# ibrohimmn1994/GPU-implementation-of-signle-and-block-Lanczos

Measured on AMD Instinct MI355X. Metric: block-Lanczos iters/sec + SpMM achieved HBM GB/s vs peak, n=10M nnz=1e8 b=16, higher is better.
Workload: dtype f64; 1 GPU; C3 block Lanczos b=16 fp64, banded-random symmetric CSR n=10000000 per GPU, nnz~10/row, halfwidth 4096; config=C3, n_total=10000000, n_per_gpu=10000000, nnz_per_gpu=100000182, b=16, parallelism=single

## Files before the change

### gpu-implementation-of-signle-and-block-lanczos_amd/__init__.py

```python
from __future__ import annotations

import ctypes
import os
from dataclasses import dataclass
from typing import NamedTuple, Optional

import numpy as np

PKG_DIR = os.path.dirname(os.path.abspath(__file__))
LIB_DIR = os.path.join(PKG_DIR, "lib")
HIP_LIB = os.environ.get("LZ_HIP_LIB") or os.path.join(LIB_DIR, "liblz_hip.so")
HOST_LIB = os.path.join(LIB_DIR, "liblz_host.so")

LZ_F64, LZ_F32 = 0, 1
LZ_ROW_MAJOR, LZ_COL_MAJOR = 0, 1
(LZ_K_SEG768, LZ_K_SEG1536, LZ_K_SEG1024, LZ_K_FNZ, LZ_K_BUF, LZ_K_LDS, LZ_K_ANY_B, LZ_K_CM_DIRECT,
 LZ_K_SPMV) = range(1, 10)
LZ_K_WIN, LZ_K_YCM, LZ_K_EPI, LZ_K_AX3, LZ_K_DOT = 0x100, 0x200, 0x400, 0x800, 0x1000
LZ_K_AX4 = 0x2000
LZ_K_GRAM16, LZ_K_GRAM32F, LZ_K_GRAM_GEN, LZ_K_TSMM16, LZ_K_TSMM32F, LZ_K_TSMM_GEN = range(1, 7)
LZ_K_PGRAM16, LZ_K_PGRAM_GEN, LZ_K_PAPPLY16, LZ_K_PAPPLY_GEN = range(7, 11)
PANEL_GROUP_16, PANEL_GROUP_GEN = 16, 4
PANEL_MAX_BLOCKS = 64
LZ_K_PCOMP16, LZ_K_PCOMP_GEN = 11, 12
PANEL_MAX_KEEP = 16
TRANSPOSE_SHORT, TRANSPOSE_LDS, TRANSPOSE_SCAN_BLOCK = 16, 4096, 2048
CG_THREADS, CG_ROWS_128, CG_GRID_CAP, CG_CHECK_EVERY = 256, 32, 2048, 8
CG_MET, CG_SPENT, CG_NOT_PD = 0, 1, 2
BCG_THREADS, BCG_ROWS_16, BCG_ROWS_32, BCG_ROWS_GEN, BCG_GRID_CAP, BCG_MAX_B = 256, 64, 128, 16, 1024, 32
LZ_K_BCG16, LZ_K_BCG32F, LZ_K_BCG_GEN = 13, 14, 15
BCG_NONE, BCG_CONVERGED, BCG_SPENT, BCG_RANK, BCG_NOT_PD = 0, 1, 2, 3, 4


def bcg_guard(b: int, eps: float) -> float:
    return max(1e-10, 64.0 * b * eps)


_c_i64, _c_i32, _c_int, _c_dbl, _c_vp = ctypes.c_int64, ctypes.c_int32, ctypes.c_int, ctypes.c_double, ctypes.c_void_p
_c_u32, _c_u64 = ctypes.c_uint32, ctypes.c_uint64


class LanczosError(RuntimeError):
    """Raised for a non-zero status from liblz_hip.so / liblz_host.so."""


_hip = None
_host = None

HIP_SYMBOLS = [
    ("lz_init", _c_int, [_c_int, ctypes.POINTER(_c_vp)]),
    ("lz_finalize", _c_int, [_c_vp]),
    ("lz_set_stream", _c_int, [_c_vp, _c_vp]),
    ("lz_set_final_state", _c_int, [_c_vp, _c_int]),
    ("lz_last_error", ctypes.c_char_p, []),
    ("lz_version", ctypes.c_char_p, []),
    ("lz_device_ok", _c_int, [_c_int]),
    ("lz_device_error", _c_int, [_c_vp, ctypes.POINTER(_c_int)]),
    ("lz_debug_poison_lds", _c_int, [_c_vp, ctypes.c_uint32]),
    ("lz_debug_set_device_error", _c_int, [_c_vp, _c_int]),
    ("lz_debug_fail_next_setup", _c_int, [_c_vp, _c_int]),
    ("lz_prof_enable", _c_int, [_c_vp, _c_int]),
    ("lz_prof_enable_mask", _c_int, [_c_vp, ctypes.c_uint]),
    ("lz_prof_read", _c_int, [_c_vp, _c_int, ctypes.POINTER(_c_dbl), ctypes.POINTER(_c_int)]),
    ("lz_csr_spmm", _c_int, [_c_vp, _c_i64, _c_i64, _c_i64, _c_vp, _c_vp, _c_vp, _c_int, _c_int,
                             _c_vp, _c_i64, _c_int, _c_vp, _c_i64]),
    ("lz_to_row_major", _c_int, [_c_vp, _c_i64, _c_int, _c_int, _c_vp, _c_i64, _c_vp]),
    ("lz_to_col_major", _c_int, [_c_vp, _c_i64, _c_int, _c_int, _c_vp, _c_vp, _c_i64]),
    ("lz_csr_spmv", _c_int, [_c_vp, _c_i64, _c_i64, _c_i64, _c_vp, _c_vp, _c_vp, _c_int, _c_vp, _c_vp]),
    ("lz_gram", _c_int, [_c_vp, _c_i64, _c_int, _c_int, _c_vp, _c_i64, _c_vp]),
    ("lz_sym_cross_gram", _c_int, [_c_vp, _c_i64, _c_int, _c_int, _c_vp, _c_vp, _c_i64, _c_vp]),
    ("lz_tsmm", _c_int, [_c_vp, _c_i64, _c_int, _c_int, _c_dbl, _c_dbl, _c_vp, _c_vp, _c_vp, _c_i64]),
    ("lz_sqrtm_pair", _c_int, [_c_vp, _c_int, _c_int, _c_vp, _c_vp, _c_vp, _c_vp]),
    ("lz_copy_row", _c_int, [_c_vp, _c_int, _c_int, _c_vp, _c_i64, _c_int, _c_i64, _c_vp, _c_i64]),
    ("lz_block_lanczos", _c_int, [_c_vp, _c_i64, _c_i64, _c_vp, _c_vp, _c_vp, _c_int, _c_int, _c_int,
                                  _c_i64, _c_vp, _c_vp, _c_vp, _c_vp, _c_vp, _c_vp, _c_vp]),
    ("lz_block_lanczos_unfused", _c_int, [_c_vp, _c_i64, _c_i64, _c_vp, _c_vp, _c_vp, _c_int, _c_int,
                                          _c_int, _c_i64, _c_vp, _c_vp, _c_vp, _c_vp, _c_vp, _c_vp, _c_vp]),
    ("lz_panel_gram", _c_int, [_c_vp, _c_i64, _c_int, _c_int, _c_int, _c_vp, _c_i64, _c_vp, _c_vp]),
    ("lz_panel_apply", _c_int, [_c_vp, _c_i64, _c_int, _c_int, _c_int, _c_dbl, _c_dbl, _c_vp, _c_i64, _c_vp, _c_vp]),
    ("lz_block_lanczos_reorth", _c_int, [_c_vp, _c_i64, _c_i64, _c_vp, _c_vp, _c_vp, _c_int, _c_int, _c_int,
                                         _c_i64, _c_vp, _c_vp, _c_vp, _c_vp, _c_vp, _c_i64, _c_vp, _c_int]),
    ("lz_panel_compress", _c_int, [_c_vp, _c_i64, _c_int, _c_int, _c_int, _c_int, _c_vp, _c_i64, _c_vp]),
    ("lz_block_lanczos_reorth_resume", _c_int, [_c_vp, _c_i64, _c_i64, _c_vp, _c_vp, _c_vp, _c_int, _c_int, _c_int,
                                                _c_int, _c_i64, _c_vp, _c_vp, _c_vp, _c_vp, _c_vp, _c_i64, _c_vp,
                                                _c_int]),
    ("lz_csr_spmm_axpby", _c_int, [_c_vp, _c_i64, _c_i64, _c_vp, _c_vp, _c_vp, _c_int, _c_int, _c_dbl, _c_vp,
                                   _c_dbl, _c_dbl, _c_vp, _c_vp]),
    ("lz_cheb_apply", _c_int, [_c_vp, _c_i64, _c_i64, _c_vp, _c_vp, _c_vp, _c_int, _c_int, _c_vp, _c_vp, _c_vp,
                               _c_vp]),
    ("lz_col_dots", _c_int, [_c_vp, _c_i64, _c_int, _c_int, _c_vp, _c_vp, _c_vp]),
    ("lz_csr_spmm_axpby_dots", _c_int, [_c_vp, _c_i64, _c_i64, _c_vp, _c_vp, _c_vp, _c_int, _c_int, _c_dbl, _c_vp,
                                        _c_dbl, _c_dbl, _c_vp, _c_vp, _c_vp]),
    ("lz_cheb_moments", _c_int, [_c_vp, _c_i64, _c_i64, _c_vp, _c_vp, _c_vp, _c_int, _c_int, _c_dbl, _c_dbl, _c_int,
                                 _c_vp, _c_vp, _c_vp]),
    ("lz_cg_update", _c_int, [_c_vp, _c_i64, _c_int, _c_int, _c_vp, _c_vp, _c_vp, _c_vp, _c_vp, _c_vp, _c_vp]),
    ("lz_cg_solve", _c_int, [_c_vp, _c_i64, _c_i64, _c_vp, _c_vp, _c_vp, _c_int, _c_int, _c_dbl, _c_vp, _c_vp, _c_vp,
                             _c_vp, _c_vp, _c_vp, _c_vp, _c_vp, _c_vp]),
    ("lz_bcg_update", _c_int, [_c_vp, _c_i64, _c_int, _c_int, _c_vp, _c_vp, _c_vp, _c_vp, _c_vp, _c_vp, _c_vp]),
    ("lz_bcg_direction", _c_int, [_c_vp, _c_i64, _c_int, _c_int, _c_vp, _c_vp, _c_vp, _c_vp]),
    ("lz_bcg_solve", _c_int, [_c_vp, _c_i64, _c_i64, _c_vp, _c_vp, _c_vp, _c_int, _c_int, _c_dbl, _c_vp, _c_vp, _c_vp,
                              _c_vp, _c_vp, _c_vp, _c_vp, _c_vp, _c_vp]),
    ("lz_block_lanczos_reorth_cheb", _c_int, [_c_vp, _c_i64, _c_i64, _c_vp, _c_vp, _c_vp, _c_int, _c_int, _c_int,
                                              _c_i64, _c_vp, _c_vp, _c_vp, _c_vp, _c_vp, _c_i64, _c_vp, _c_int,
                                              _c_vp, _c_vp]),
    ("lz_block_lanczos_reorth_resume_cheb", _c_int, [_c_vp, _c_i64, _c_i64, _c_vp, _c_vp, _c_vp, _c_int, _c_int,
                                                     _c_int, _c_int, _c_i64, _c_vp, _c_vp, _c_vp, _c_vp, _c_vp,
                                                     _c_i64, _c_vp, _c_int, _c_vp, _c_vp]),
    ("lz_csr_spmm_axpby4", _c_int, [_c_vp, _c_i64, _c_i64, _c_vp, _c_vp, _c_vp, _c_int, _c_int, _c_dbl, _c_vp,
                                    _c_dbl, _c_dbl, _c_vp, _c_dbl, _c_vp, _c_vp]),
    ("lz_cheb_series_apply", _c_int, [_c_vp, _c_i64, _c_i64, _c_vp, _c_vp, _c_vp, _c_int, _c_int, _c_int, _c_dbl,
                                      _c_dbl, _c_vp, _c_vp, _c_vp, _c_vp]),
    ("lz_block_lanczos_reorth_series", _c_int, [_c_vp, _c_i64, _c_i64, _c_vp, _c_vp, _c_vp, _c_int, _c_int, _c_int,
                                                _c_i64, _c_vp, _c_vp, _c_vp, _c_vp, _c_vp, _c_i64, _c_vp, _c_int,
                                                _c_int, _c_dbl, _c_dbl, _c_vp, _c_vp]),
    ("lz_block_lanczos_reorth_resume_series", _c_int, [_c_vp, _c_i64, _c_i64, _c_vp, _c_vp, _c_vp, _c_int, _c_int,
                                                       _c_int, _c_int, _c_i64, _c_vp, _c_vp, _c_vp, _c_vp, _c_vp,
                                                       _c_i64, _c_vp, _c_int, _c_int, _c_dbl, _c_dbl, _c_vp, _c_vp]),
    ("lz_csr_transpose", _c_int, [_c_vp, _c_i64, _c_i64, _c_i64, _c_vp, _c_vp, _c_vp, _c_int, _c_vp, _c_vp, _c_vp]),
    ("lz_normal_apply", _c_int, [_c_vp, _c_i64, _c_i64, _c_i64, _c_vp, _c_vp, _c_vp, _c_vp, _c_vp, _c_vp, _c_int,
                                 _c_int, _c_vp, _c_vp, _c_vp]),
    ("lz_block_lanczos_reorth_normal", _c_int, [_c_vp, _c_i64, _c_i64, _c_i64, _c_vp, _c_vp, _c_vp, _c_vp, _c_vp,
                                                _c_vp, _c_int, _c_int, _c_int, _c_i64, _c_vp, _c_vp, _c_vp, _c_vp,
                                                _c_vp, _c_i64, _c_vp, _c_int, _c_vp]),
    ("lz_block_lanczos_reorth_resume_normal", _c_int, [_c_vp, _c_i64, _c_i64, _c_i64, _c_vp, _c_vp, _c_vp, _c_vp,
                                                       _c_vp, _c_vp, _c_int, _c_int, _c_int, _c_int, _c_i64, _c_vp,
                                                       _c_vp, _c_vp, _c_vp, _c_vp, _c_i64, _c_vp, _c_int, _c_vp]),
    ("lz_vector_lanczos", _c_int, [_c_vp, _c_i64, _c_i64, _c_vp, _c_vp, _c_vp, _c_int, _c_int, _c_i64,
                                   _c_vp, _c_vp, _c_vp, _c_vp, _c_vp, _c_vp, _c_vp]),
    ("lz_fdtd_block", _c_int, [_c_vp, _c_i64, _c_i64, _c_vp, _c_vp, _c_vp, _c_int, _c_int, _c_vp,
                               _c_i64, _c_dbl, _c_i64, _c_vp, _c_vp, _c_vp]),
    ("lz_comm_unique_id", _c_int, [_c_vp]),
    ("lz_comm_init", _c_int, [_c_vp, _c_int, _c_int, _c_vp]),
    ("lz_halo_init", _c_int, [_c_vp, _c_i64, _c_i64, _c_vp, _c_vp]),
    ("lz_halo_sizes", _c_int, [_c_vp, _c_vp, _c_vp]),
    ("lz_halo_exchange", _c_int, [_c_vp, _c_int, _c_int, _c_vp]),
    ("lz_block_lanczos_halo", _c_int, [_c_vp, _c_i64, _c_i64, _c_vp, _c_vp, _c_vp, _c_int, _c_int, _c_int,
                                       _c_i64, _c_int, _c_vp, _c_vp, _c_vp, _c_vp, _c_vp, _c_vp]),
    ("lz_comm_destroy", _c_int, [_c_vp]),
    ("lz_local_group_create", _c_int, [_c_int, _c_int, ctypes.POINTER(_c_vp)]),
    ("lz_local_group_destroy", _c_int, [_c_vp]),
    ("lz_local_group_abort", _c_int, [_c_vp]),
    ("lz_comm_init_local", _c_int, [_c_vp, _c_vp, _c_int]),
    ("lz_comm_abort", _c_int, [_c_vp]),
    ("lz_debug_last_split", _c_int, [_c_vp, _c_vp]),
    ("lz_debug_last_wf", _c_int, [_c_vp, ctypes.POINTER(_c_int)]),
    ("lz_debug_last_kernel", _c_int, [_c_vp, ctypes.POINTER(_c_int)]),
    ("lz_debug_wf_plan", _c_int, [_c_vp, _c_i64, _c_i64, _c_vp, _c_vp, _c_i64, _c_i64, _c_vp, _c_vp,
                                  ctypes.POINTER(_c_int)]),
    ("lz_block_lanczos_dist", _c_int, [_c_vp, _c_i64, _c_i64, _c_i64, _c_i64, _c_vp, _c_vp, _c_vp,
                                       _c_int, _c_int, _c_int, _c_i64, _c_int, _c_vp, _c_vp, _c_vp,
                                       _c_vp, _c_vp, _c_vp, _c_vp, _c_vp]),
]

HOST_SYMBOLS = [
    ("lzh_gen_banded_count", _c_i64, [_c_i64, _c_dbl, _c_i64, _c_u64, _c_vp]),
    ("lzh_gen_banded_fill", _c_int, [_c_i64, _c_dbl, _c_i64, _c_u64, _c_vp, _c_vp, _c_vp, _c_vp]),
    ("lzh_gen_banded_local_count", _c_i64, [_c_i64, _c_dbl, _c_i64, _c_u64, _c_i64, _c_i64, _c_vp]),
    ("lzh_gen_banded_local_fill", _c_int, [_c_i64, _c_dbl, _c_i64, _c_u64, _c_i64, _c_i64, _c_vp, _c_vp,
                                           _c_vp, _c_vp]),
    ("lzh_gen_powerlaw_count", _c_i64, [_c_i64, _c_dbl, _c_dbl, _c_i64, _c_u64, _c_vp]),
    ("lzh_gen_powerlaw_fill", _c_int, [_c_i64, _c_dbl, _c_dbl, _c_i64, _c_u64, _c_vp, _c_vp, _c_vp, _c_vp]),
    ("lzh_matrix_a_shape", _c_int, [_c_int, _c_vp, _c_vp]),
    ("lzh_matrix_a_ell", _c_int, [_c_int, _c_int, _c_vp, _c_vp]),
    ("lzh_ell_to_csr_count", _c_i64, [_c_i64, _c_i64, _c_vp, _c_vp, _c_int, _c_vp]),
    ("lzh_ell_to_csr_fill", _c_int, [_c_i64, _c_i64, _c_vp, _c_vp, _c_int, _c_vp, _c_vp, _c_vp]),
    ("lzh_rand_B", _c_int, [_c_i64, _c_int, _c_u32, _c_i64, _c_int, _c_vp]),
    ("lzh_rand_lc", _c_i64, [_c_u32]),
    ("lzh_uniform_B", _c_int, [_c_i64, _c_int, _c_u64, _c_vp, _c_vp]),
    ("lzh_uniform_B_rows", _c_int, [_c_i64, _c_i64, _c_int, _c_u64, _c_vp, _c_vp]),
    ("lzh_sym_eig", _c_int, [_c_int, _c_vp, _c_vp, _c_vp]),
    ("lzh_assemble_T", _c_int, [_c_int, _c_int, _c_vp, _c_vp, _c_vp]),
    ("lzh_ritz_values", _c_int, [_c_int, _c_int, _c_vp, _c_vp, _c_vp]),
    ("lzh_ritz_pairs", _c_int, [_c_int, _c_int, _c_vp, _c_vp, _c_int, _c_int, _c_vp, _c_vp, _c_vp]),
    ("lzh_ritz_pairs_dense", _c_int, [_c_int, _c_int, _c_vp, _c_vp, _c_int, _c_int, _c_vp, _c_vp, _c_vp]),
    ("lzh_restart_coeffs", _c_int, [_c_int, _c_int, _c_int, _c_vp, _c_vp, _c_int, _c_vp, _c_vp, _c_vp, _c_vp]),
    ("lzh_restart_fill", _c_int, [_c_int, _c_int, _c_int, _c_vp, _c_vp, _c_vp]),
    ("lzh_gershgorin", _c_int, [_c_i64, _c_vp, _c_vp, _c_vp, _c_vp]),
    ("lzh_cg_start", _c_int, [_c_int, _c_int, _c_int, _c_vp, _c_vp, _c_vp, _c_vp, _c_vp, _c_vp, _c_vp, _c_vp, _c_vp,
                              _c_vp]),
    ("lzh_cg_scalars", _c_int, [_c_int, _c_int, _c_int, _c_vp, _c_vp, _c_vp, _c_vp, _c_vp, _c_vp, _c_vp, _c_vp, _c_vp,
                                _c_vp, _c_vp]),
    ("lzh_bcg_start", _c_int, [_c_int, _c_int, _c_vp, _c_vp, _c_vp, _c_vp, _c_vp, _c_vp]),
    ("lzh_bcg_start_finish", _c_int, [_c_int, _c_dbl, _c_vp, _c_vp, _c_vp, _c_vp, _c_vp, _c_vp, _c_vp]),
    ("lzh_bcg_mid", _c_int, [_c_int, _c_vp, _c_vp, _c_vp, _c_vp, _c_vp, _c_vp]),
    ("lzh_bcg_end", _c_int, [_c_int, _c_int, _c_dbl, _c_vp, _c_vp, _c_vp, _c_vp, _c_vp, _c_vp, _c_vp]),
    ("lzh_bcg_guard", _c_dbl, [_c_int, _c_dbl]),
    ("lzh_kpm_moments", _c_int, [_c_int, _c_int, _c_vp, _c_vp]),
    ("lzh_jackson", _c_int, [_c_int, _c_vp]),
    ("lzh_kpm_count", _c_int, [_c_int, _c_vp, _c_vp, _c_dbl, _c_dbl, _c_dbl, _c_dbl, _c_vp]),
    ("lzh_cheb_window", _c_int, [_c_int, _c_dbl, _c_dbl, _c_dbl, _c_dbl, _c_vp, _c_vp]),
    ("lzh_kpm_density", _c_int, [_c_int, _c_vp, _c_vp, _c_dbl, _c_dbl, _c_int, _c_vp, _c_vp]),
    ("lzh_block_solution", _c_int, [_c_int, _c_int, _c_dbl, _c_vp, _c_vp, _c_vp, _c_vp]),
    ("lzh_partition_rows", _c_int, [_c_i64, _c_vp, _c_int, _c_vp]),
    ("lzh_remap_cols_padded", _c_int, [_c_i64, _c_vp, _c_int, _c_vp, _c_i64, _c_vp]),
    ("lzh_halo_plan", _c_i64, [_c_i64, _c_vp, _c_int, _c_vp, _c_int, _c_vp, _c_vp, _c_vp]),
    ("lzh_csr_write", _c_int, [ctypes.c_char_p, _c_i64, _c_i64, _c_i64, _c_vp, _c_vp, _c_vp, _c_int]),
    ("lzh_csr_read_header", _c_int, [ctypes.c_char_p, _c_vp, _c_vp, _c_vp, _c_vp]),
    ("lzh_csr_read", _c_int, [ctypes.c_char_p, _c_vp, _c_vp, _c_vp]),
    ("lzh_num_threads", _c_int, []),
]


def _bind(lib, symbols, strict=True):
    for name, res, args in symbols:
        if not strict and not hasattr(lib, name):
            continue
        fn = getattr(lib, name)
        fn.restype = res
        fn.argtypes = args
    return lib


def build(verbose: bool = False) -> None:
    import subprocess
    jobs = str(min(16, os.cpu_count() or 4))
    out = subprocess.run(["make", "-C", PKG_DIR, "-j", jobs], capture_output=not verbose, text=True)
    if out.returncode != 0:
        raise LanczosError("build failed:\n" + (out.stdout or "") + (out.stderr or ""))


def host_lib():
    global _host
    if _host is None:
        if not os.path.exists(HOST_LIB):
            raise LanczosError(f"{HOST_LIB} missing: run make in {PKG_DIR}")
        _host = _bind(ctypes.CDLL(HOST_LIB), HOST_SYMBOLS)
    return _host


def hip_lib():
    global _hip
    if _hip is None:
        if not os.path.exists(HIP_LIB):
            raise LanczosError(f"{HIP_LIB} missing: run make in {PKG_DIR}")
        try:
            import torch
        except ImportError:
            pass
        _hip = _bind(ctypes.CDLL(HIP_LIB), HIP_SYMBOLS, strict=not os.environ.get("LZ_HIP_LIB"))
    return _hip


def _check(rc: int, what: str) -> None:
    if rc != 0:
        msg = hip_lib().lz_last_error().decode(errors="replace") if _hip is not None else ""
        raise LanczosError(f"{what} failed with status {rc}: {msg}")


def _p(a: np.ndarray):
    return a.ctypes.data_as(_c_vp)


@dataclass
class CsrHost:
    n: int
    row_ptr: np.ndarray
    col: np.ndarray
    val: np.ndarray

    @property
    def nnz(self) -> int:
        return int(self.row_ptr[-1])


def gen_banded(n: int, nnz_per_row: float = 10.0, halfwidth: int = 4096, seed: int = 20261015,
               dtype=np.float64) -> CsrHost:
    L = host_lib()
    rp = np.empty(n + 1, np.int64)
    nnz = L.lzh_gen_banded_count(n, nnz_per_row, halfwidth, seed, _p(rp))
    if nnz < 0:
        raise LanczosError("lzh_gen_banded_count failed")
    col = np.empty(nnz, np.int32)
    val = np.empty(nnz, dtype)
    v64 = _p(val) if dtype == np.float64 else None
    v32 = _p(val) if dtype == np.float32 else None
    if L.lzh_gen_banded_fill(n, nnz_per_row, halfwidth, seed, _p(rp), _p(col), v64, v32):
        raise LanczosError("lzh_gen_banded_fill failed")
    return CsrHost(n, rp, col, val)


def gen_banded_local(n: int, r0: int, r1: int, nnz_per_row: float = 10.0, halfwidth: int = 4096,
                     seed: int = 20261015, dtype=np.float64) -> CsrHost:
    L = host_lib()
    nl = r1 - r0
    rp = np.empty(nl + 1, np.int64)
    nnz = L.lzh_gen_banded_local_count(n, nnz_per_row, halfwidth, seed, r0, r1, _p(rp))
    if nnz < 0:
        raise LanczosError("lzh_gen_banded_local_count failed")
    col = np.empty(nnz, np.int32)
    val = np.empty(nnz, dtype)
    v64 = _p(val) if dtype == np.float64 else None
    v32 = _p(val) if dtype == np.float32 else None
    if L.lzh_gen_banded_local_fill(n, nnz_per_row, halfwidth, seed, r0, r1, _p(rp), _p(col), v64, v32):
        raise LanczosError("lzh_gen_banded_local_fill failed")
    return CsrHost(nl, rp, col, val)


def gen_powerlaw(n: int, nnz_per_row: float = 10.0, a: float = 2.1, cap: int = 100000,
                 seed: int = 20261015, dtype=np.float32) -> CsrHost:
    L = host_lib()
    rp = np.empty(n + 1, np.int64)
# ... 1035 lines not shown
                    scale=scale, cols=sel, filter=filt, n_steps=d.steps)

    def eigsh_interval(self, A: CsrDevice, a: float, b: float, /, block: int = 16, m: Optional[int] = None,
                       keep: Optional[int] = None, degree: Optional[int] = None, bounds=None, pad: float = 0.01,
                       tol: float = 1e-10, max_cycles: int = 100, B=None, lc: int = 0, passes: int = 2):
        torch = _torch()
        a, b = float(a), float(b)
        if not a < b:
            raise LanczosError(f"eigsh_interval: the window [{a}, {b}] needs a < b")
        lo, hi = gershgorin(A) if bounds is None else (float(bounds[0]), float(bounds[1]))
        if not (np.isfinite(lo) and np.isfinite(hi) and lo < hi and pad >= 0):
            raise LanczosError(f"eigsh_interval: bounds ({lo}, {hi}) must be finite with lo < hi, pad >= 0")
        lo, hi = lo - pad * (hi - lo), hi + pad * (hi - lo)
        if not (lo <= a and b <= hi):
            raise LanczosError(f"eigsh_interval: the window [{a}, {b}] is not inside the enclosure [{lo}, {hi}]")
        if degree is None:
            degree = min(65536, max(16, int(np.ceil(np.pi * (hi - lo) / (b - a)))))
        if not 1 <= int(degree) <= 65536:
            raise LanczosError("eigsh_interval: 1 <= degree <= 65536")
        degree = int(degree)
        if keep is None:
            keep = 4 if m is None else max(1, min(4, m - 1))
        m, r = _restart_sizes("eigsh_interval", "(keep - 1) * block", max((keep - 1) * block, 1), block, m, keep)
        n, bs = A.n, block
        scale = max(abs(lo), abs(hi))
        gamma = cheb_window(degree, lo, hi, a, b)
        work = torch.empty(2 * n * bs, dtype=A.val.dtype, device=A.val.device)
        d = _Restart(self, A, n, bs, m, r, lc, passes, A.val, series=(degree, lo, hi, gamma), work=work)
        V, vstride, kw = d.V, d.vstride, d.kw
        U, X = work[:n * bs].view(n, bs), work[n * bs:].view(n, bs)
        C = torch.empty(r, bs, bs, **kw)
        G, Dm = torch.empty(bs, bs, **kw), torch.empty(bs, bs, **kw)
        rb = r * bs

        def check():
            H = np.empty((rb, rb))
            for i in range(r):
                self.spmm(A, V[i * vstride:i * vstride + n * bs].view(n, bs), U)
                self.panel_gram(V, vstride, r, U, C)
                H[:, i * bs:(i + 1) * bs] = _f64(C).reshape(rb, bs)
            lam, Cm = np.linalg.eigh(0.5 * (H + H.T))
            Sd = torch.from_numpy(_pack_chunks(Cm, r, bs)).to(**kw)
            res = np.empty(rb)
            for c in range(r):
                self.panel_apply(0.0, 1.0, V, vstride, r, Sd[c], X)
                self.spmm(A, X, U)
                Dm.copy_(torch.from_numpy(np.diag(lam[c * bs:(c + 1) * bs])).to(**kw))
                self.mm_ts(1.0, -1.0, X, Dm, U)
                self.mm_tt(U, G)
                res[c * bs:(c + 1) * bs] = np.sqrt(np.maximum(np.diag(_f64(G)), 0.0))
            return lam, res, Cm

        d.first(d.start_block(B))
        history = []
        while True:
            d.compress("largest")
            lam, res, Cm = check()
            meets = (lam + res >= a) & (lam - res <= b)
            inside = (lam >= a) & (lam <= b)
            full = bool(inside.sum() == rb)
            history.append(float(res[meets].max()) if meets.any() else 0.0)
            converged = bool(not full and (res[meets] <= tol * scale).all())
            if converged or full or d.cycles >= max_cycles:
                break
            d.resume()
        sel = np.flatnonzero(inside)
        if sel.size:
            Zx = _pack_chunks(Cm[:, sel], r, bs)
            self.panel_compress(V, vstride, r, len(Zx), d._dev(Zx), n=n)
        return dict(theta=lam[sel], resid=res[sel], count=int(sel.size), V=V, vstride=vstride, cycles=d.cycles,
                    n_steps=d.steps, n_spmm=degree * d.steps + 2 * r * d.cycles, converged=converged, full=full,
                    history=history, scale=scale, filter=(degree, lo, hi))

    def set_final_state(self, on: bool) -> None:
        _check(self.L.lz_set_final_state(self.ptr, 1 if on else 0), "lz_set_final_state")

    def vector_lanczos(self, A: CsrDevice, bvec, m: int, lc: int, q, alpha, beta, q0, q1, w):
        n = bvec.shape[0]
        for t in (bvec, q, alpha, beta, q0, q1, w):
            if t.element_size() != (8 if A.dtype == LZ_F64 else 4):
                raise ValueError("vector_lanczos: every vector must have A's element type")
        _check(self.L.lz_vector_lanczos(self.ptr, n, A.nnz, _ptr(A.row_ptr), _ptr(A.col), _ptr(A.val), A.dtype,
                                        m, lc, _ptr(bvec), _ptr(q), _ptr(alpha), _ptr(beta), _ptr(q0),
                                        _ptr(q1), _ptr(w)), "lz_vector_lanczos")

    def ftdt_block(self, A: CsrDevice, U0, steps: int, T_end: float, lc: int, U, D, out):
        n, b = U0.shape
        _check(self.L.lz_fdtd_block(self.ptr, n, A.nnz, _ptr(A.row_ptr), _ptr(A.col), _ptr(A.val), A.dtype, b,
                                    _ptr(U0), steps, T_end, lc, _ptr(U), _ptr(D), _ptr(out)), "lz_fdtd_block")
        return out

    PROF_SPMM_PASS, PROF_UPDATE_PASS, PROF_SMALL, PROF_GRAM, PROF_TSMM, PROF_SPMM = range(6)

    def device_error(self) -> int:
        c = _c_int()
        _check(self.L.lz_device_error(self._h, ctypes.byref(c)), "lz_device_error")
        return c.value

    def debug_set_device_error(self, code: int):
        _check(self.L.lz_debug_set_device_error(self.ptr, code), "lz_debug_set_device_error")

    def debug_fail_next_setup(self, code: int = 5):
        _check(self.L.lz_debug_fail_next_setup(self._h, code), "lz_debug_fail_next_setup")

    def debug_poison_lds(self, pattern: int = 0xFFFFFFFF):
        _check(self.L.lz_debug_poison_lds(self._h, pattern), "lz_debug_poison_lds")

    def prof_enable(self, on: bool = True, classes=None):
        if classes is None:
            _check(self.L.lz_prof_enable(self._h, int(on)), "lz_prof_enable")
        else:
            mask = 0
            for c in classes:
                mask |= 1 << int(c)
            _check(self.L.lz_prof_enable_mask(self._h, mask if on else 0), "lz_prof_enable_mask")

    def prof_read(self, cls: int):
        ms, cnt = _c_dbl(), _c_int()
        _check(self.L.lz_prof_read(self._h, cls, ctypes.byref(ms), ctypes.byref(cnt)), "lz_prof_read")
        return ms.value, cnt.value

    def comm_init(self, nranks: int, rank: int, uid: bytes):
        buf = ctypes.create_string_buffer(uid, 128)
        _check(self.L.lz_comm_init(self._h, nranks, rank, buf), "lz_comm_init")

    def comm_init_local(self, group: "LocalGroup", rank: int):
        _check(self.L.lz_comm_init_local(self.ptr, group.ptr, rank), "lz_comm_init_local")
        group._keep.append(self)

    def last_wf(self):
        v = (_c_int * 2)()
        _check(self.L.lz_debug_last_wf(self._h, v), "lz_debug_last_wf")
        return bool(v[0]), bool(v[1])

    def last_kernel(self):
        v = (_c_int * 2)()
        _check(self.L.lz_debug_last_kernel(self._h, v), "lz_debug_last_kernel")
        return int(v[0]), int(v[1])

    def wf_plan(self, A, nx=None, xoff=0):
        import torch
        T_max = A.n // 16 + 2
        deps = torch.zeros(T_max * 2, dtype=torch.int32, device=A.row_ptr.device)
        c16 = torch.zeros(max(A.nnz, 1), dtype=torch.int16, device=A.row_ptr.device)
        info = (_c_int * 8)()
        _check(self.L.lz_debug_wf_plan(self.ptr, A.n, A.nnz, A.row_ptr.data_ptr(), A.col.data_ptr(),
                                       A.n if nx is None else nx, xoff, deps.data_ptr(), c16.data_ptr(), info),
               "lz_debug_wf_plan")
        T = int(info[2])
        d = {"ok": bool(info[0]), "col16": bool(info[1]), "T": T, "tr": int(info[3]),
             "spans": [int(info[4 + i]) for i in range(4)]}
        return d, deps[: 2 * T].view(T, 2), c16[: A.nnz]

    def last_split(self):
        v = (_c_i64 * 2)()
        _check(self.L.lz_debug_last_split(self._h, v), "lz_debug_last_split")
        return None if v[0] < 0 else (int(v[0]), int(v[1]))

    def comm_abort(self):
        _check(self.L.lz_comm_abort(self._h), "lz_comm_abort")

    def comm_destroy(self):
        _check(self.L.lz_comm_destroy(self._h), "lz_comm_destroy")

    def block_lanczos_dist(self, A_local: CsrDevice, n_pad: int, n_global: int, B_local, m: int,
                           lc_local: int, lc_rank: int, q, alpha, beta, Q0, W, X_full):
        n_local, b = A_local.n, B_local.shape[1]
        _check(self.L.lz_block_lanczos_dist(self.ptr, n_local, n_pad, n_global, A_local.nnz,
                                            _ptr(A_local.row_ptr), _ptr(A_local.col), _ptr(A_local.val),
                                            A_local.dtype, b, m, lc_local, lc_rank, _ptr(B_local), _ptr(q),
                                            _ptr(alpha), _ptr(beta), _ptr(Q0), None, _ptr(W), _ptr(X_full)),
               "lz_block_lanczos_dist")


    def halo_init(self, row0: int, n_local: int, recv_counts: np.ndarray, halo_rows: np.ndarray):
        rc = np.ascontiguousarray(recv_counts, np.int64)
        hr = np.ascontiguousarray(halo_rows, np.int32)
        _check(self.L.lz_halo_init(self.ptr, row0, n_local, _p(rc), _p(hr) if hr.size else None),
               "lz_halo_init")

    def halo_sizes(self):
        nh, ns = _c_i64(), _c_i64()
        _check(self.L.lz_halo_sizes(self.ptr, ctypes.byref(nh), ctypes.byref(ns)), "lz_halo_sizes")
        return nh.value, ns.value

    def halo_exchange(self, X):
        _check(self.L.lz_halo_exchange(self.ptr, _dt(X), X.shape[1], _ptr(X)), "lz_halo_exchange")

    def block_lanczos_halo(self, A_local: CsrDevice, B_local, m: int, lc_local: int, lc_rank: int,
                           q, alpha, beta, X0, X1):
        n_local, b = A_local.n, B_local.shape[1]
        _check(self.L.lz_block_lanczos_halo(self.ptr, n_local, A_local.nnz, _ptr(A_local.row_ptr),
                                            _ptr(A_local.col), _ptr(A_local.val), A_local.dtype, b, m,
                                            lc_local, lc_rank, _ptr(B_local), _ptr(q), _ptr(alpha),
                                            _ptr(beta), _ptr(X0), _ptr(X1)),
               "lz_block_lanczos_halo")


class LocalGroup:

    def __init__(self, nranks: int, device: int = 0):
        L = hip_lib()
        g = _c_vp()
        _check(L.lz_local_group_create(device, nranks, ctypes.byref(g)), "lz_local_group_create")
        self.ptr, self.nranks, self.device, self.L = g, nranks, device, L
        self._keep = []

    def abort(self):
        if self.ptr:
            self.L.lz_local_group_abort(self.ptr)

    def close(self):
        if self.ptr:
            self.L.lz_local_group_destroy(self.ptr)
            self.ptr = None

    def __del__(self):
        try:
            self.close()
        except Exception:
            pass


def run_virtual_ranks(nranks: int, fn, device: int = 0, timeout: float = 600.0):
    import threading
    torch = _torch()
    torch.cuda.synchronize(device)
    group = LocalGroup(nranks, device)
    handles = [Handle(device) for _ in range(nranks)]
    streams = [torch.cuda.Stream(device) for _ in range(nranks)]
    out, errs = [None] * nranks, [None] * nranks

    def body(r):
        try:
            with torch.cuda.device(device), torch.cuda.stream(streams[r]):
                handles[r].comm_init_local(group, r)
                out[r] = fn(r, handles[r])
                torch.cuda.current_stream(device).synchronize()
        except BaseException as e:
            errs[r] = e
            group.abort()

    threads = [threading.Thread(target=body, args=(r,), daemon=True) for r in range(nranks)]
    try:
        for t in threads:
            t.start()
        for t in threads:
            t.join(timeout)
        if any(t.is_alive() for t in threads):
            group.abort()
            for t in threads:
                t.join(30)
        if any(t.is_alive() for t in threads):
            raise LanczosError("virtual ranks did not finish")
    finally:
        if not any(t.is_alive() for t in threads):
            torch.cuda.synchronize(device)
            for h in handles:
                h.close()
            group.close()
            group._keep.clear()
            del streams[:]
    for r, e in enumerate(errs):
        if e is not None:
            raise LanczosError(f"virtual rank {r}: {e}") from e
    return out


def comm_unique_id() -> bytes:
    buf = ctypes.create_string_buffer(128)
    _check(hip_lib().lz_comm_unique_id(buf), "lz_comm_unique_id")
    return buf.raw


def run_block_lanczos(h: Handle, A: CsrDevice, B, m: int, lc: int, fused: bool = True):
    torch = _torch()
    n, b = B.shape
    kw = dict(dtype=B.dtype, device=B.device)
    q = torch.zeros(m * b, **kw)
    alpha = torch.zeros(m, b, b, **kw)
    beta = torch.zeros(m + 1, b, b, **kw)
    Q0, Q1, W = (torch.empty(n, b, **kw) for _ in range(3))
    h.block_lanczos_blas(A, B, m, lc, q, alpha, beta, Q0, Q1, W, fused=fused)
    return q, alpha, beta
```

### gpu-implementation-of-signle-and-block-lanczos_amd/csrc/lz_api.hip

```cpp
#include <cmath>
#include <cstdarg>
#include <cstdlib>
#include <cstring>
#include <algorithm>
#include <utility>
#include <vector>

#include <type_traits>
#include "lz_comm.hpp"
#include "lz_common.hpp"
#include "lz_internal.hpp"
#include "lz_kernels.hpp"

namespace lz {

static thread_local char g_err[1024] = "";

int prof_begin(lz_handle *h, int cls)
{
    if (!h->prof || !((h->prof_mask >> cls) & 1u) || h->ev_used + 2 > h->ev_cap) return -1;
    const int idx = h->ev_used;
    if (hipEventRecord(h->ev_pool[idx], h->stream) != hipSuccess) return -1;
    h->ev_class[idx / 2] = cls;
    h->ev_used += 2;
// ... 340 lines not shown
        LZ_ARG_CHECK(std::isfinite(sr.lo) && std::isfinite(sr.hi) && sr.lo < sr.hi, "Chebyshev series: lo < hi, finite");
        LZ_ARG_CHECK(sr.gamma != nullptr, "Chebyshev series: gamma is NULL");
        break;
    case OpSpec::Normal:
        LZ_ARG_CHECK(op.p >= 1, "normal operator: p >= 1");
        LZ_ARG_CHECK(op.t_rp != nullptr, "normal operator: the transpose's row_ptr is NULL");
        LZ_ARG_CHECK(op.t_col != nullptr && op.t_val != nullptr, "normal operator: the transpose's col/val NULL");
        break;
    }
    LZ_ARG_CHECK(op.work != nullptr, "work is NULL");
    LZ_ARG_CHECK(!work16 || reinterpret_cast<uintptr_t>(op.work) % 16 == 0, "work must be on 16 bytes");
    LZ_ARG_CHECK(apart(span_of(op.work, op.work_elems(n, b), dtype), others), apart_msg);
    return LZ_OK;
}

template <typename T>
static int reorth_op(lz_handle *h, int64_t n, int b, const OpSpec &op, const T *Q, T *W)
{
    const T *val = (const T *)op.val;
    T *work = (T *)op.work;
    switch (op.form) {
    case OpSpec::Filter:
        return cheb_apply<T>(h, n, op.nnz, op.rp, op.col, val, b, op.f, Q, W, work);
    case OpSpec::Series:
        return cheb_series_apply<T>(h, n, op.nnz, op.rp, op.col, val, b, op.sr, Q, W, work);
    case OpSpec::Normal:
        LZ_TRY(spmm_rm<T>(h, op.p, op.nnz, op.rp, op.col, val, b, Q, b, n, work, b));
        return spmm_rm<T>(h, n, op.nnz, op.t_rp, op.t_col, (const T *)op.t_val, b, work, b, op.p, W, b);
    case OpSpec::Plain:
        break;
    }
    return spmm_rm<T>(h, n, op.nnz, op.rp, op.col, val, b, Q, b, n, W, b);
}

template <typename T>
static int reorth_steps(lz_handle *h, int64_t n, const OpSpec &op, int b, int j0, int m, int64_t lc, T *q,
                        T *alpha, T *beta, T *V, int64_t vstride, T *W, int passes)
{
    const int64_t bb = (int64_t)b * b;
    T *binv = ScratchT<T>(h, b).binv[0];
    int P = 0;
    for (int j = j0; j < m; ++j) {
        T *bj = beta + j * bb, *aj = alpha + j * bb;
        T *Qp = V + (int64_t)(j - 1) * vstride, *Qj = V + (int64_t)j * vstride;
        LZ_TRY(gram_partials<T>(h, n, b, W, W, b, &P));
        LZ_TRY(sqrtm_pair<T>(h, b, nullptr, P, bj, binv, nullptr));
        LZ_TRY(tsmm<T>(h, n, b, T(0), T(1), W, binv, Qj, b));
        LZ_TRY(reorth_op<T>(h, n, b, op, Qj, W));
        LZ_TRY(tsmm<T>(h, n, b, T(1), T(-1), Qp, bj, W, b));
        LZ_TRY(gram_partials<T>(h, n, b, W, Qj, b, &P));
        LZ_TRY(gram_finish<T>(h, b, P, 1, aj));
        LZ_TRY(tsmm<T>(h, n, b, T(1), T(-1), Qj, aj, W, b));
        LZ_TRY(reorth_rounds<T>(h, n, b, j + 1, V, vstride, W, passes));
        LZ_TRY(copy_row<T>(h, b, Qj, b, 0, lc, q + (int64_t)j * b));
    }
    LZ_TRY(gram_partials<T>(h, n, b, W, W, b, &P));
    LZ_TRY(sqrtm_pair<T>(h, b, nullptr, P, beta + m * bb, binv, nullptr));
    return LZ_OK;
}

template <typename T>
static int reorth_cycle(lz_handle *h, int64_t n, const OpSpec &op, int b, int r, int m, int64_t lc, const T *B,
                        const T *sigma, T *q, T *alpha, T *beta, T *V, int64_t vstride, T *W, int passes)
{
    const int64_t bb = (int64_t)b * b;
    const bool first = r == 0;
    T *binv = ScratchT<T>(h, b).binv[0];
    LZ_TRY(reorth_reserve<T>(h, n, b, m, passes));
    int P = 0;
    const T *R = first ? B : W;
    T *br = beta + r * bb, *ar = alpha + r * bb, *Qr = V + (int64_t)r * vstride;
    LZ_TRY(gram_partials<T>(h, n, b, R, R, b, &P));
    LZ_TRY(sqrtm_pair<T>(h, b, nullptr, P, br, binv, nullptr));
    LZ_TRY(tsmm<T>(h, n, b, T(0), T(1), R, binv, Qr, b));
    if (first) LZ_TRY(copy_row<T>(h, b, Qr, b, 0, lc, q));
    LZ_TRY(reorth_op<T>(h, n, b, op, Qr, W));
    if (!first) LZ_TRY(panel_apply<T>(h, n, b, r, 1.0, -1.0, V, vstride, sigma, W));
    LZ_TRY(gram_partials<T>(h, n, b, W, Qr, b, &P));
    LZ_TRY(gram_finish<T>(h, b, P, 1, ar));
    LZ_TRY(tsmm<T>(h, n, b, T(1), T(-1), Qr, ar, W, b));
    LZ_TRY(reorth_rounds<T>(h, n, b, r + 1, V, vstride, W, passes));
    if (!first) LZ_TRY(copy_row<T>(h, b, Qr, b, 0, lc, q + (int64_t)r * b));
    return reorth_steps<T>(h, n, op, b, r + 1, m, lc, q, alpha, beta, V, vstride, W, passes);
}

struct Pass1Plan {
    const uint64_t *pairs = nullptr;
    int win = 0;
    const int16_t *col16 = nullptr;
};
static int pass1_plan(lz_handle *h, int64_t n, int64_t nnz, const int64_t *rp, const int32_t *col, int64_t nx,
                      int64_t row_off, Pass1Plan *pl)
{
    LZ_TRY(strip_pairs(h, n, rp, &pl->pairs));
    if (nx >= (1 << 24)) {
        bool ok = false;
        LZ_TRY(gather_window_ok(h, n, rp, col, nx, row_off, &ok));
        pl->win = ok ? 1 : 0;
    }
    if (nx < (1 << 24) || pl->win) LZ_TRY(col16_plan(h, n, nnz, rp, col, row_off, &pl->col16));
    return LZ_OK;
}

template <typename T>
struct ResidualRing {
    const T *in, *prev = nullptr;
    T *r0, *r1;
    ResidualRing(const T *B, int m, T *W, T *Q1) : in(B), r0((m & 1) ? W : Q1), r1((m & 1) ? Q1 : W) {}
    T *out(int j) const { return j == 0 ? r0 : j == 1 ? r1 : const_cast<T *>(prev); }
    void advance(T *out) { prev = in, in = out; }
};

template <typename T>
static int store_beta_m(lz_handle *h, T *beta, int m, int64_t bb, T *const binv[2])
{
    LZ_HIP_TRY(hipMemcpyAsync(beta + m * bb, binv[(m - 1) & 1], sizeof(T) * bb, hipMemcpyDeviceToDevice, h->stream));
    return LZ_OK;
}

struct WfTail {
    lz_handle *h;
    double *slab;
    double *const *binv;
    double *P1, *P2, *alpha, *beta, *q;
    int64_t lc;
    Comm *cm = nullptr;
    int operator()(int j, const WfSlabs &sl, const double *V) const
    {
        constexpr int64_t bb = 256;
        LZ_TRY(wf_fold16(h, sl, slab));
        if (cm) LZ_TRY(cm->allreduce_sum(slab, 3 * bb, h->stream));
        const WfAlpha wa{slab, 1, alpha + j * bb, P2, V, lc, q + j * 16};
        return sqrtm_pair<double>(h, 16, nullptr, 1, beta + j * bb, binv[j & 1], nullptr, slab + 2 * bb,
                                  j ? binv[(j - 1) & 1] : nullptr, j ? P1 : nullptr, &wa);
    }
};

static WfSlabs wf_one_set(const double *part, int P)
{
    WfSlabs sl;
    sl.add(part, P);
    return sl;
}

static int gram_beside(lz_handle *h, int64_t n, const double *B, int *P)
{
    LZ_TRY(stream_fork(h, h->ev_fork, h->side));
    StreamScope on_side(h, h->side);
    LZ_TRY(gram_partials<double>(h, n, 16, B, B, 16, P));
    LZ_HIP_TRY(hipEventRecord(h->ev_join, h->side));
    return LZ_OK;
}

static int block_lanczos_wf16(lz_handle *h, int64_t n, int64_t nnz, const int64_t *rp, const int32_t *col,
                              const double *val, int m, int64_t lc, const double *B, double *q, double *alpha,
                              double *beta, double *Q0, double *Q1, double *W, const Pass1Plan &pl,
                              const WfPlan &wp, int Pg)
{
    constexpr int64_t bb = 256;
    (void)nnz;
    const Scratch16 sc(h);
    double *const *binv = sc.binv;
    double *P1 = sc.P1, *P2 = sc.P2, *slab = sc.slab;
    const int64_t lcl = (lc >= 0 && lc < n) ? lc : -1;
    int P = 0;
    const bool g0 = Pg < 0;
    if (!g0) LZ_TRY(sqrtm_pair<double>(h, 16, nullptr, Pg, beta, binv[0], nullptr));
    LZ_TRY(wf_reset16(h, n, wp));
    const WfSolve ws{n, rp, col, val, pl.pairs, wp, n};
    const WfTail tail{h, slab, binv, P1, P2, alpha, beta, q, lcl};
    double *part = h->partials2;
    LZ_TRY(wf_step16(h, ws, ws.first(B, Q0, g0), part, &P));
    if (g0) LZ_TRY(tail(0, wf_one_set(part, P), B));
    else LZ_TRY(alpha_wf16(h, part, P, binv[0], nullptr, alpha, P2, B, lc, n, q));
    const double *Vm1 = nullptr, *V0 = B;
    auto pass2 = [&](int j, double *Vn) { return WfPass2{Q0, Vm1, V0, Vn, binv[j & 1], j ? P1 : nullptr, P2}; };
    for (int j = 0; j + 1 < m; ++j) {
        double *Vn = j == 0 ? W : j == 1 ? Q1 : const_cast<double *>(Vm1);
        LZ_TRY(wf_step16(h, ws, ws.step(pass2(j, Vn), ws.all(), {Vn, Q0, ws.all()}, j + 1), part, &P));
        LZ_TRY(tail(j + 1, wf_one_set(part, P), Vn));
        Vm1 = V0;
        V0 = Vn;
    }
    LZ_TRY(store_beta_m<double>(h, beta, m, bb, binv));
    if (h->final_state) {
        const WfPass2 p2 = pass2(m - 1, W);
        if (wp.var == 111)
            LZ_TRY(wf_step16(h, ws, ws.post_call(p2, m, Q0, m >= 2 ? Q1 : nullptr), part, &P));
        else
            LZ_TRY(final_state<double>(h, n, 16, p2.Yj, p2.Vprev, p2.Vj, nullptr, p2.binv, p2.P1, p2.P2, W, Q0,
                                       m >= 2 ? Q1 : nullptr));
    }
    return LZ_OK;
}

static int block_lanczos_fused16(lz_handle *h, int64_t n, int64_t nnz, const int64_t *rp, const int32_t *col,
                                 const double *val, int m, int64_t lc, const double *B, double *q,
                                 double *alpha, double *beta, double *Q0, double *Q1, double *W)
{
    constexpr int64_t bb = 256;
    (void)Q0;
    const Scratch16 qb(h);
    double *const qP = qb.P1;
    int P = 0;
    Pass1Plan pl;
    const bool g0 = wf_first_gram(n, nnz);
    if (!g0) LZ_TRY(gram_beside(h, n, B, &P));
    JoinSide join_side{h};
    {
        WfPlan wp;
        LZ_TRY(wf_plan16(h, n, nnz, rp, col, &wp));
        if (wp.ok) {
            LZ_TRY(strip_pairs(h, n, rp, &pl.pairs));
            pl.col16 = wp.col16;
            if (!g0) LZ_HIP_TRY(hipStreamWaitEvent(h->stream, h->ev_join, 0));
            else if (wp.var != 111) LZ_TRY(gram_partials<double>(h, n, 16, B, B, 16, &P));
            const bool first = g0 && wp.var == 111;
            return block_lanczos_wf16(h, n, nnz, rp, col, val, m, lc, B, q, alpha, beta, Q0, Q1, W, pl, wp,
                                      first ? -1 : P);
        }
    }
    if (g0) LZ_TRY(gram_partials<double>(h, n, 16, B, B, 16, &P));
    LZ_TRY(pass1_plan(h, n, nnz, rp, col, n, 0, &pl));
    LZ_HIP_TRY(hipStreamWaitEvent(h->stream, h->ev_join, 0));
    LZ_TRY(sqrtm_pair<double>(h, 16, nullptr, P, beta, qb.binv[0], nullptr));
    ResidualRing<double> r(B, m, W, Q1);
    for (int j = 0; j < m; ++j) {
        double *out = r.out(j);
        const double *bi = qb.binv[j & 1];
        LZ_TRY(fused_spmm16(h, n, rp, col, val, r.in, n, r.in, r.prev, out, bi, j ? qP : nullptr, lc, q + j * 16, &P,
                            pl.pairs, nnz, 0, pl.win, 0, pl.col16));
        LZ_TRY(gram_finish<double>(h, 16, P, 1, alpha + j * bb, h->partials2, bi, qP));
        LZ_TRY(fused_update16(h, n, out, r.in, qP, &P));
        if (j + 1 < m)
            LZ_TRY(sqrtm_pair<double>(h, 16, nullptr, P, beta + (j + 1) * bb, qb.binv[(j + 1) & 1], nullptr,
                                      nullptr, bi, qP));
        r.advance(out);
    }
    LZ_TRY(store_beta_m<double>(h, beta, m, bb, qb.binv));
    if (h->final_state)
        LZ_TRY(final_state<double>(h, n, 16, nullptr, nullptr, r.prev, r.in, qb.binv[(m - 1) & 1], nullptr, nullptr,
                                   W, Q0, m >= 2 ? Q1 : nullptr));
    return LZ_OK;
}

static int block_lanczos_b2_32(lz_handle *h, int64_t n, int64_t nnz, const int64_t *rp, const int32_t *col,
                               const float *val, int m, int64_t lc, const float *B, float *q, float *alpha,
                               float *beta, float *Q0, float *Q1, float *W)
{
    constexpr int b = 32;
    const int64_t bb = (int64_t)b * b;
    const ScratchT<float> sc(h, b);
    float *const *binv = sc.binv;
    float *P2 = sc.P, *M = sc.P3;
    float *U = Q0;
    JoinSide join_side{h};
    int np = 0, cap = 768, lslot = -1;
    LZ_TRY(spmm_b2_stage(h, n, rp, &cap));
#ifndef LZ_B2_STEP0_QUEUES
    LZ_TRY(spmm_b2_plan(h, n, rp, cap, &lslot));
#endif
    LZ_TRY(gram_partials<float>(h, n, b, B, B, b, &np));
    LZ_TRY(sqrtm_pair<float>(h, b, nullptr, np, beta, binv[0], nullptr));
    ResidualRing<float> r(B, m, W, Q1);
    for (int j = 0; j < m; ++j) {
        float *out = r.out(j);
        const float *bi = binv[j & 1];
        const float *in = r.in, *prev = r.prev;
#ifndef LZ_B2_STEP0_QUEUES
        LZ_TRY(spmm_rm_b2(h, n, nnz, rp, col, val, in, n, U, prev, j ? M : nullptr, lslot, nullptr, cap));
#else
        LZ_TRY(spmm_rm_b2(h, n, nnz, rp, col, val, in, n, U, prev, j ? M : nullptr, j ? lslot : -1,
                          j ? nullptr : &lslot, cap));
#endif
        if (j > 0) LZ_HIP_TRY(hipStreamWaitEvent(h->stream, h->ev_join, 0));
        LZ_TRY(fused_el32(h, n, in, U, &np));
        const int nf = fold_slabs_g(h, h->partials, np, (int)bb, 32);
        LZ_TRY(alpha_b2(h, h->partials2, nf, bi, alpha + j * bb, P2, in, lc, n, q + (int64_t)j * b));
        const bool qlast = j + 1 == m && h->final_state;
        LZ_TRY(fused_ub32(h, n, U, in, bi, P2, out, &np, qlast ? Q0 : nullptr, qlast && m >= 2 ? Q1 : nullptr));
        if (j + 1 < m) {
            const int ng = fold_slabs_g(h, h->partials, np, (int)bb, 32);
            LZ_TRY(m_b2(h, h->partials2, ng, bi, M));
            LZ_TRY(stream_fork(h, h->ev_fork, h->side));
            StreamScope on_side(h, h->side);
            LZ_TRY(sqrtm_pair<float>(h, b, nullptr, ng, beta + (j + 1) * bb, binv[(j + 1) & 1], nullptr,
                                     h->partials2));
            LZ_HIP_TRY(hipEventRecord(h->ev_join, h->side));
        }
        r.advance(out);
    }
    LZ_TRY(store_beta_m<float>(h, beta, m, bb, binv));
    return LZ_OK;
}

template <typename T>
static int block_lanczos_sep(lz_handle *h, int64_t n, int64_t nnz, const int64_t *rp, const int32_t *col,
                             const T *val, int b, int m, int64_t lc, const T *B, T *q, T *alpha, T *beta, T *Q0,
                             T *Q1, T *W)
{
    if constexpr (std::is_same<T, float>::value) {
        const char *e = getenv("LZ_C5_B2");
        if (b == 32 && !(e && atoi(e) == 0) && spmm_b2_ok(n, nnz, n))
            return block_lanczos_b2_32(h, n, nnz, rp, col, val, m, lc, B, q, alpha, beta, Q0, Q1, W);
    }
    const int64_t bb = (int64_t)b * b;
    const ScratchT<T> sc(h, b);
    T *const *binv = sc.binv;
    T *P = sc.P;
    T *Y = Q0;
    int np = 0;
    LZ_TRY(gram_partials<T>(h, n, b, B, B, b, &np));
    LZ_TRY(sqrtm_pair<T>(h, b, nullptr, np, beta, binv[0], nullptr));
    ResidualRing<T> r(B, m, W, Q1);
    for (int j = 0; j < m; ++j) {
        T *out = r.out(j);
        const T *bi = binv[j & 1];
        const T *in = r.in, *prev = r.prev;
        LZ_TRY(spmm_rm<T>(h, n, nnz, rp, col, val, b, in, b, n, Y, b));
        if (j > 0) LZ_HIP_TRY(hipStreamWaitEvent(h->stream, h->ev_join, 0));
        LZ_TRY(fused_e_sep<T>(h, n, b, Y, in, prev, out, bi, j ? P : nullptr, lc, q + (int64_t)j * b, &np));
        LZ_TRY(gram_finish<T>(h, b, np, 1, alpha + j * bb, h->partials, bi, P));
        LZ_TRY(fused_u_sep<T>(h, n, b, out, in, P, &np));
        if (j + 1 < m) {
            LZ_TRY(stream_fork(h, h->ev_fork, h->side));
            StreamScope on_side(h, h->side);
            LZ_TRY(sqrtm_pair<T>(h, b, nullptr, np, beta + (j + 1) * bb, binv[(j + 1) & 1], nullptr, nullptr, bi, P));
            LZ_HIP_TRY(hipEventRecord(h->ev_join, h->side));
        }
        r.advance(out);
    }
    LZ_TRY(store_beta_m<T>(h, beta, m, bb, binv));
    if (h->final_state)
        LZ_TRY(final_state<T>(h, n, b, nullptr, nullptr, r.prev, r.in, binv[(m - 1) & 1], nullptr, nullptr, W, Q0,
                              m >= 2 ? Q1 : nullptr));
    return LZ_OK;
}

constexpr int64_t kFdtdGraph = 256;
constexpr int64_t kFdtdFusedRows = 1 << 18;

template <typename T>
static int fdtd_block(lz_handle *h, int64_t n, int64_t nnz, const int64_t *rp, const int32_t *col, const T *val,
                      int b, const T *U0, int64_t steps, double T_end, int64_t lc, T *U, T *D,
                      T *out)
{
    const T dt = (T)(T_end / (double)steps);
    LZ_HIP_TRY(hipMemcpyAsync(U, U0, sizeof(T) * n * b, hipMemcpyDeviceToDevice, h->stream));
    const bool fused = n <= kFdtdFusedRows;
    T *cur = U;
    auto step = [&]() -> int {
        if (fused) {
            T *nxt = cur == U ? D : U;
            const int64_t nb = n * b;
            hipLaunchKernelGGL((k_fdtd_step<T>), dim3((unsigned)ceil_div(nb, 256)), dim3(256), 0, h->stream,
                               nb, b, rp, col, val, dt, (const T *)cur, nxt);
            LZ_LAUNCH_CHECK();
            cur = nxt;
            return LZ_OK;
        }
        LZ_TRY(spmm_rm<T>(h, n, nnz, rp, col, val, b, U, b, n, D, b));
        return axpy<T>(h, n * b, dt, D, U);
    };
    const char *graph_env = getenv("LZ_FDTD_GRAPH");
    const bool use_graph = !(graph_env && graph_env[0] == '0');
    int64_t s = 0;
    LZ_TRY(step());
    ++s;
    if (use_graph && steps - s >= 2 * kFdtdGraph) {
        hipStream_t cap = nullptr;
        LZ_HIP_TRY(hipStreamCreateWithFlags(&cap, hipStreamNonBlocking));
        int rc = LZ_OK;
// ... 453 lines not shown
    LZ_TRY(wf_reset16(h, n, wp));
    const WfSolve ws{n, rp, col, val, pairs, wp, nx};
    const WfTail tail{h, slab, binv, P1, P2, alpha, beta, q, lcl, cx.reduce ? cm : nullptr};
    const double *Vm1 = nullptr, *V0 = ag ? slot : X0;
    int G = 0;
    LZ_TRY(wf_step16(h, ws, ws.first(X0, Y, g0), h->partials2, &G));
    if (g0) {
        LZ_TRY(tail(0, wf_one_set(h->partials2, G), V0));
    } else {
        LZ_TRY(wf_fold16(h, wf_one_set(h->partials2, G), slab));
        LZ_TRY(cx.allreduce(3 * bb));
        LZ_TRY(alpha_wf16(h, slab, 1, binv[0], nullptr, alpha, P2, V0, lcl, n, q));
    }
    const bool sw = ag && h->nranks > 1;
    for (int j = 0; j + 1 < m; ++j) {
        double *Vn = sw ? slot : ((j & 1) ? X0 : X1);
        double *Vg = sw ? X0 : Vn;
        const double *Vprev = sw ? (j ? X1 : nullptr) : Vm1;
        const WfPass2 p2{Y, Vprev, V0, Vn, binv[j & 1], j ? P1 : nullptr, P2, sw ? X1 : nullptr};
        WfSlabs sl;
        double *part = h->partials2;
        auto launch = [&](const WfLaunch &L) -> int {
            int g = 0;
            LZ_TRY(wf_step16(h, ws, L, part, &g));
            sl.add(part, g);
            part += 3 * (int64_t)g * 256;
            return LZ_OK;
        };
        if (pre) {
            LZ_TRY(launch(ws.pass2(p2, {0, sh}, {st, T}, j + 1)));
            LZ_TRY(stream_fork(h, h->ev_cx, h->xstream));
            LZ_TRY(cx.exchange(Vg, h->xstream));
            LZ_HIP_TRY(hipEventRecord(h->ev_xd, h->xstream));
        }
        LZ_TRY(launch(ws.step(p2, pre ? WfTiles{sh, st} : ws.all(), {Vg, Y, {t0, t1}}, j + 1)));
        if (exch) {
            if (pre) LZ_HIP_TRY(hipStreamWaitEvent(h->stream, h->ev_xd, 0));
            else LZ_TRY(cx.exchange(Vg, h->stream));
            const bool two = t0 > 0 && t1 < T;
            if (two) LZ_TRY(stream_fork(h, h->ev_cx, h->xstream));
            LZ_TRY(launch(ws.boundary(Vg, Y, {0, t0})));
            {
                StreamScope on_x(h, two ? h->xstream : h->stream);
                LZ_TRY(launch(ws.boundary(Vg, Y, {t1, T})));
            }
            if (two) LZ_TRY(stream_join(h, h->ev_bd, h->xstream));
        }
        LZ_TRY(tail(j + 1, sl, Vn));
        Vm1 = V0;
        V0 = Vn;
    }
    LZ_TRY(store_beta_m<double>(h, beta, m, bb, binv));
    if (cm) LZ_TRY(cm->fence(h->stream));
    return LZ_OK;
}

template <typename T>
static int dist_solve(lz_handle *h, int form, HaloPlan *hp, int64_t n, int64_t n_pad, int64_t nnz, const int64_t *rp,
                      const int32_t *col, const T *val, int b, int m, int64_t lc, const T *B, T *q, T *alpha, T *beta,
                      T *X0, T *X1)
{
    LZ_TRY(solve_begin(h));
    int rc = dist_solve_impl<T>(h, form, hp, n, n_pad, nnz, rp, col, val, b, m, lc, B, q, alpha, beta, X0, X1);
    if (rc == LZ_OK) rc = solve_status(h);
    return rc;
}

}

using namespace lz;

static int dist_fail(lz_handle *h, int rc, uint64_t issued0)
{
    if (rc != LZ_OK && rc != LZ_E_DEVICE && h && h->comm &&
        (h->comm->abort_wakes_peers() || h->comm->issued != issued0))
        h->comm->abort();
    return rc;
}

static uint64_t comm_issued(const lz_handle *h) { return h && h->comm ? h->comm->issued : 0; }

#define LZ_HANDLE_CHECK(h)                                                          \
    do {                                                                            \
        if (!(h)) {                                                                 \
            set_error("handle is NULL");                                           \
            return LZ_E_STATE;                                                      \
        }                                                                           \
        LZ_HIP_TRY(hipSetDevice((h)->device));                                      \
    } while (0)

static int shape_args(lz_dtype dtype, int64_t n, int64_t n_min, int b, int b_max, const char *msg = nullptr)
{
    char text[64];
    if (!msg) snprintf(text, sizeof(text), "n >= %lld, b in [1,%d]", (long long)n_min, b_max), msg = text;
    LZ_ARG_CHECK(dtype == LZ_F64 || dtype == LZ_F32, "dtype");
    LZ_ARG_CHECK(n >= n_min && b >= 1 && b <= b_max, msg);
    return LZ_OK;
}

template <typename Solve>
static int krylov_entry(lz_handle *h, int64_t n, int64_t nnz, const int64_t *rp, const int32_t *col, const void *val,
                        lz_dtype dtype, int b, int b_max, double shift, const void *B, void *X, void *work,
                        const lz_cg_opts *opts, int *iters, int *status, double *resid, double *est, int *info,
                        Solve solve)
{
    LZ_HANDLE_CHECK(h);
    LZ_TRY(check_csr(n, nnz, rp, col, val));
    LZ_TRY(shape_args(dtype, n, 1, b, b_max));
    LZ_ARG_CHECK(B && X && work && opts && iters && status && resid && est && info, "NULL argument");
    LZ_ARG_CHECK(opts->tol > 0.0 && std::isfinite(opts->tol) && std::isfinite(shift), "tol > 0, tol and shift finite");
    LZ_ARG_CHECK(opts->max_iter >= 0 && opts->max_restarts >= 0, "max_iter, max_restarts >= 0");
    const int64_t nb = n * b;
    LZ_ARG_CHECK(pairwise_apart({span_of(B, nb, dtype), span_of(X, nb, dtype), span_of(work, 4 * nb, dtype)}),
                 "B, X and work must be pairwise distinct");
    return by_dtype(dtype, [&](auto t) {
        using T = decltype(t);
        return solve(h, n, nnz, rp, col, (const T *)val, b, shift, (const T *)B, (T *)X, (T *)work, *opts, iters, status,
                     resid, est, info);
    });
}

extern "C" {

const char *lz_last_error(void) { return g_err; }
const char *lz_version(void) { return "lz_hip 0.1 gfx950"; }

int lz_device_ok(int device)
{
    int count = 0;
    if (hipGetDeviceCount(&count) != hipSuccess || device < 0 || device >= count) return 0;
    hipDeviceProp_t prop;
    if (hipGetDeviceProperties(&prop, device) != hipSuccess) return 0;
    return std::strncmp(prop.gcnArchName, "gfx950", 6) == 0 ? 1 : 0;
}

static int init_handle(lz_handle *h, int device)
{
    h->device = device;
    hipDeviceProp_t prop;
    LZ_HIP_TRY(hipGetDeviceProperties(&prop, device));
    if (std::strncmp(prop.gcnArchName, "gfx950", 6) != 0) {
        set_error("device %d is %s, liblz_hip.so is built for gfx950 only", device, prop.gcnArchName);
        return LZ_E_HIP;
    }
    h->n_cu = prop.multiProcessorCount;
    LZ_TRY(ensure_partials(h, (size_t)kMaxPartials * kMaxB * kMaxB));
    LZ_HIP_TRY(hipMalloc(&h->partials2, sizeof(double) * kPartials2Doubles));
    LZ_HIP_TRY(hipMalloc(&h->scratch, sizeof(double) * kScratchDoubles));
    LZ_HIP_TRY(hipMalloc(&h->err_flag, sizeof(int) * kFlagWords));
    LZ_HIP_TRY(hipMemsetAsync(h->err_flag, 0, sizeof(int) * kFlagWords, h->stream));
    LZ_HIP_TRY(hipStreamCreateWithFlags(&h->side, hipStreamNonBlocking));
    LZ_HIP_TRY(hipEventCreateWithFlags(&h->ev_fork, hipEventDisableTiming));
    LZ_HIP_TRY(hipEventCreateWithFlags(&h->ev_join, hipEventDisableTiming));
    if (const char *pz = getenv("LZ_POISON"); pz && pz[0] == '1') {
        LZ_HIP_TRY(hipMemsetAsync(h->partials, 0xFF, h->partials_cap, h->stream));
        LZ_HIP_TRY(hipMemsetAsync(h->partials2, 0xFF, sizeof(double) * kPartials2Doubles, h->stream));
        LZ_HIP_TRY(hipMemsetAsync(h->scratch, 0xFF, sizeof(double) * kScratchDoubles, h->stream));
    }
    LZ_HIP_TRY(hipStreamSynchronize(h->stream));
    return LZ_OK;
}

int lz_init(int device, lz_handle **out)
{
    LZ_ARG_CHECK(out != nullptr, "out handle pointer is NULL");
    *out = nullptr;
    int count = 0;
    LZ_HIP_TRY(hipGetDeviceCount(&count));
    LZ_ARG_CHECK(device >= 0 && device < count, "device index");
    LZ_HIP_TRY(hipSetDevice(device));
    lz_handle *h = new lz_handle();
    const int rc = init_handle(h, device);
    if (rc != LZ_OK) {
        lz_finalize(h);
        return rc;
    }
    *out = h;
    return LZ_OK;
}

int lz_finalize(lz_handle *h)
{
    if (!h) return LZ_OK;
    (void)hipSetDevice(h->device);
    detach_comm(h);
    (void)hipFree(h->pairs);
    (void)hipFree(h->longq);
    (void)hipFree(h->cm_buf);
    (void)hipFree(h->dots_ws);
    (void)hipFree(h->cg_ws);
    (void)hipFree(h->bcg_ws);
    (void)hipFree(h->ybuf);
    (void)hipFree(h->coef);
    (void)hipFree(h->tr_ws);
    (void)hipFree(h->c16buf);
    (void)hipFree(h->wf_deps);
    (void)hipFree(h->wf_flags);
    (void)hipFree(h->fnz_colf);
    (void)hipFree(h->fnz_trow);
    if (h->ev_pool) {
        for (int i = 0; i < h->ev_cap; ++i) (void)hipEventDestroy(h->ev_pool[i]);
        delete[] h->ev_pool;
    }
    (void)hipFree(h->partials);
    (void)hipFree(h->partials2);
    (void)hipFree(h->scratch);
    (void)hipFree(h->err_flag);
    if (h->ev_fork) (void)hipEventDestroy(h->ev_fork);
    if (h->ev_join) (void)hipEventDestroy(h->ev_join);
    if (h->ev_lfork) (void)hipEventDestroy(h->ev_lfork);
    if (h->ev_ljoin) (void)hipEventDestroy(h->ev_ljoin);
    if (h->lstream) (void)hipStreamDestroy(h->lstream);
    if (h->side) (void)hipStreamDestroy(h->side);
    for (hipStream_t s : {h->pf_sg, h->pf_sp})
        if (s) {
            (void)hipStreamSynchronize(s);
            (void)hipStreamDestroy(s);
        }
    for (hipEvent_t e : {h->ev_pff, h->ev_pfg, h->ev_pfp})
        if (e) (void)hipEventDestroy(e);
    (void)hipFree(h->pf_ctl);
    delete h;
    return LZ_OK;
}

int lz_device_error(lz_handle *h, int *code)
{
    LZ_ARG_CHECK(h && code, "null argument");
    int c = 0;
    LZ_HIP_TRY(hipMemcpyAsync(&c, h->err_flag, sizeof(int), hipMemcpyDeviceToHost, h->stream));
    LZ_HIP_TRY(hipMemsetAsync(h->err_flag, 0, sizeof(int), h->stream));
    LZ_HIP_TRY(hipStreamSynchronize(h->stream));
    *code = c;
    return LZ_OK;
}

int lz_debug_set_device_error(lz_handle *h, int code)
{
    LZ_HANDLE_CHECK(h);
    LZ_HIP_TRY(hipMemsetD32Async(reinterpret_cast<hipDeviceptr_t>(h->err_flag), code, 1, h->stream));
    return LZ_OK;
}

int lz_debug_fail_next_setup(lz_handle *h, int code)
{
    LZ_HANDLE_CHECK(h);
    h->dbg_setup_fail = code;
    return LZ_OK;
}

__global__ __launch_bounds__(1024) void k_poison_lds(uint32_t pattern)
{
    constexpr int kWords = 160 * 1024 / 4;
    __shared__ uint32_t lds[kWords];
    volatile uint32_t *v = lds;
    for (int i = threadIdx.x; i < kWords; i += blockDim.x) v[i] = pattern;
}

int lz_debug_poison_lds(lz_handle *h, uint32_t pattern)
{
    LZ_HANDLE_CHECK(h);
    hipLaunchKernelGGL(k_poison_lds, dim3(h->n_cu * 4), dim3(1024), 0, h->stream, pattern);
    LZ_LAUNCH_CHECK();
    const int byte = (int)(pattern & 0xFF);
    LZ_HIP_TRY(hipMemsetAsync(h->partials, byte, h->partials_cap, h->stream));
    LZ_HIP_TRY(hipMemsetAsync(h->partials2, byte, sizeof(double) * kPartials2Doubles, h->stream));
    LZ_HIP_TRY(hipMemsetAsync(h->scratch, byte, sizeof(double) * kScratchDoubles, h->stream));
    if (h->dots_ws) LZ_HIP_TRY(hipMemsetAsync(h->dots_ws, byte, h->dots_cap, h->stream));
    if (h->cg_ws) LZ_HIP_TRY(hipMemsetAsync(h->cg_ws, byte, h->cg_cap, h->stream));
    if (h->bcg_ws) LZ_HIP_TRY(hipMemsetAsync(h->bcg_ws, byte, h->bcg_cap, h->stream));
    return LZ_OK;
}

int lz_prof_enable_mask(lz_handle *h, unsigned class_mask)
{
    LZ_HANDLE_CHECK(h);
    if (class_mask && !h->ev_pool) {
        h->ev_cap = 8192;
        h->ev_pool = new hipEvent_t[h->ev_cap];
        for (int i = 0; i < h->ev_cap; ++i) LZ_HIP_TRY(hipEventCreate(&h->ev_pool[i]));
    }
    h->prof = class_mask != 0;
    h->prof_mask = class_mask;
    h->ev_used = 0;
    return LZ_OK;
}

int lz_prof_enable(lz_handle *h, int on) { return lz_prof_enable_mask(h, on ? ~0u : 0u); }

int lz_prof_read(lz_handle *h, int cls, double *ms_total, int *count)
{
    LZ_HANDLE_CHECK(h);
    LZ_ARG_CHECK(ms_total && count, "NULL outputs");
    *ms_total = 0.0;
    *count = 0;
    if (!h->ev_pool || h->ev_used == 0) return LZ_OK;
    LZ_HIP_TRY(hipEventSynchronize(h->ev_pool[h->ev_used - 1]));
    for (int i = 0; i < h->ev_used; i += 2) {
        if (h->ev_class[i / 2] != cls) continue;
        float ms = 0.f;
        LZ_HIP_TRY(hipEventElapsedTime(&ms, h->ev_pool[i], h->ev_pool[i + 1]));
        *ms_total += ms;
        *count += 1;
    }
    return LZ_OK;
}

int lz_set_final_state(lz_handle *h, int on)
{
    LZ_HANDLE_CHECK(h);
    h->final_state = on ? 1 : 0;
    return LZ_OK;
}

int lz_set_stream(lz_handle *h, void *stream)
{
    LZ_HANDLE_CHECK(h);
    h->stream = reinterpret_cast<hipStream_t>(stream);
    return LZ_OK;
}

int lz_csr_spmm(lz_handle *h, int64_t n_rows, int64_t n_cols, int64_t nnz, const int64_t *rp,
                const int32_t *col, const void *val, lz_dtype dtype, int b, const void *X,
                int64_t ldx, lz_layout layout, void *Y, int64_t ldy)
{
    LZ_HANDLE_CHECK(h);
    LZ_TRY(check_csr(n_rows, nnz, rp, col, val));
    LZ_ARG_CHECK(b >= 1 && b <= kMaxB, "b in [1,64]");
    LZ_ARG_CHECK(X && Y, "X/Y NULL");
    if (layout == LZ_ROW_MAJOR) {
        LZ_ARG_CHECK(ldx >= b && ldy >= b, "row-major ld >= b");
    } else {
        LZ_ARG_CHECK(ldx >= n_cols && ldy >= n_rows, "column-major ld >= rows");
    }
    return by_dtype(dtype, [&](auto t) {
        using T = decltype(t);
        const T *v = (const T *)val, *x = (const T *)X;
        if (layout == LZ_ROW_MAJOR) return spmm_rm<T>(h, n_rows, nnz, rp, col, v, b, x, ldx, n_cols, (T *)Y, ldy);
        return spmm_cm<T>(h, n_rows, nnz, rp, col, v, b, x, ldx, n_cols, (T *)Y, ldy);
    });
}

int lz_to_row_major(lz_handle *h, int64_t rows, int b, lz_dtype dtype, const void *X, int64_t ldx, void *Y)
{
    LZ_HANDLE_CHECK(h);
    LZ_ARG_CHECK(X && Y && X != Y, "to_row_major: X, Y distinct, not NULL");
    return by_dtype(dtype, [&](auto t) {
        using T = decltype(t);
        return to_row_major<T>(h, rows, b, (const T *)X, ldx, (T *)Y);
    });
}

int lz_to_col_major(lz_handle *h, int64_t rows, int b, lz_dtype dtype, const void *X, void *Y, int64_t ldy)
{
    LZ_HANDLE_CHECK(h);
    LZ_ARG_CHECK(X && Y && X != Y, "to_col_major: X, Y distinct, not NULL");
    return by_dtype(dtype, [&](auto t) {
        using T = decltype(t);
        return to_col_major<T>(h, rows, b, (const T *)X, ldy, (T *)Y);
    });
}

// ... 381 lines not shown
int lz_block_lanczos_reorth_normal(lz_handle *h, int64_t n, int64_t p, int64_t nnz, const int64_t *rp,
                                   const int32_t *col, const void *val, const int64_t *t_rp, const int32_t *t_col,
                                   const void *t_val, lz_dtype dtype, int b, int m, int64_t lc, const void *B, void *q,
                                   void *alpha, void *beta, void *V, int64_t vstride, void *W, int passes, void *work)
{
    return cycle_entry(h, n, OpSpec::normal(p, nnz, rp, col, val, t_rp, t_col, t_val, work), dtype, b, 0, m, lc, B,
                       nullptr, q, alpha, beta, V, vstride, W, passes);
}

int lz_panel_compress(lz_handle *h, int64_t n, int b, int k, int r, lz_dtype dtype, void *V, int64_t vstride,
                      const void *Z)
{
    LZ_HANDLE_CHECK(h);
    LZ_TRY(panel_args(n, b, k, dtype, V, vstride));
    LZ_ARG_CHECK(r >= 1 && r <= k, "panel_compress keeps 1 <= r <= k blocks");
    LZ_ARG_CHECK(r <= kPanelMaxKeep, "panel_compress keeps at most LZ_PANEL_MAX_KEEP = 16 blocks");
    LZ_ARG_CHECK(Z != nullptr, "Z is NULL");
    return by_dtype(dtype, [&](auto t) {
        using T = decltype(t);
        return panel_compress<T>(h, n, b, k, r, (T *)V, vstride, (const T *)Z);
    });
}

int lz_block_lanczos_reorth_resume(lz_handle *h, int64_t n, int64_t nnz, const int64_t *rp, const int32_t *col,
                                   const void *val, lz_dtype dtype, int b, int r, int m, int64_t lc,
                                   const void *sigma, void *q, void *alpha, void *beta, void *V, int64_t vstride,
                                   void *W, int passes)
{
    return lz_block_lanczos_reorth_resume_cheb(h, n, nnz, rp, col, val, dtype, b, r, m, lc, sigma, q, alpha, beta, V,
                                               vstride, W, passes, nullptr, nullptr);
}

int lz_block_lanczos_reorth_resume_cheb(lz_handle *h, int64_t n, int64_t nnz, const int64_t *rp, const int32_t *col,
                                        const void *val, lz_dtype dtype, int b, int r, int m, int64_t lc,
                                        const void *sigma, void *q, void *alpha, void *beta, void *V, int64_t vstride,
                                        void *W, int passes, const lz_cheb *f, void *work)
{
    return cycle_entry(h, n, OpSpec::filter(nnz, rp, col, val, f, work), dtype, b, r, m, lc, nullptr, sigma, q, alpha,
                       beta, V, vstride, W, passes);
}

int lz_block_lanczos_reorth_resume_normal(lz_handle *h, int64_t n, int64_t p, int64_t nnz, const int64_t *rp,
                                          const int32_t *col, const void *val, const int64_t *t_rp,
                                          const int32_t *t_col, const void *t_val, lz_dtype dtype, int b, int r, int m,
                                          int64_t lc, const void *sigma, void *q, void *alpha, void *beta, void *V,
                                          int64_t vstride, void *W, int passes, void *work)
{
    return cycle_entry(h, n, OpSpec::normal(p, nnz, rp, col, val, t_rp, t_col, t_val, work), dtype, b, r, m, lc, nullptr,
                       sigma, q, alpha, beta, V, vstride, W, passes);
}

int lz_csr_spmm_axpby4(lz_handle *h, int64_t n, int64_t nnz, const int64_t *rp, const int32_t *col, const void *val,
                       lz_dtype dtype, int b, double a, const void *X, double c, double d, const void *Z, double e,
                       const void *U, void *Y)
{
    return terms_entry(h, n, false, nnz, rp, col, val, dtype, b, a, X, c, d, Z, e, U, true, Y, nullptr);
}

int lz_cheb_series_apply(lz_handle *h, int64_t n, int64_t nnz, const int64_t *rp, const int32_t *col, const void *val,
                         lz_dtype dtype, int b, int degree, double lo, double hi, const double *gamma, const void *X,
                         void *Y, void *work)
{
    LZ_HANDLE_CHECK(h);
    LZ_TRY(check_csr(n, nnz, rp, col, val));
    LZ_TRY(shape_args(dtype, n, 1, b, kMaxB));
    LZ_ARG_CHECK(X && Y && work, "X/Y/work NULL");
    return apply_entry(h, n, OpSpec::series(nnz, rp, col, val, degree, lo, hi, gamma, work), dtype, b, X, Y);
}

int lz_block_lanczos_reorth_series(lz_handle *h, int64_t n, int64_t nnz, const int64_t *rp, const int32_t *col,
                                   const void *val, lz_dtype dtype, int b, int m, int64_t lc, const void *B, void *q,
                                   void *alpha, void *beta, void *V, int64_t vstride, void *W, int passes, int degree,
                                   double lo, double hi, const double *gamma, void *work)
{
    return cycle_entry(h, n, OpSpec::series(nnz, rp, col, val, degree, lo, hi, gamma, work), dtype, b, 0, m, lc, B,
                       nullptr, q, alpha, beta, V, vstride, W, passes);
}

int lz_block_lanczos_reorth_resume_series(lz_handle *h, int64_t n, int64_t nnz, const int64_t *rp, const int32_t *col,
                                          const void *val, lz_dtype dtype, int b, int r, int m, int64_t lc,
                                          const void *sigma, void *q, void *alpha, void *beta, void *V,
                                          int64_t vstride, void *W, int passes, int degree, double lo, double hi,
                                          const double *gamma, void *work)
{
    return cycle_entry(h, n, OpSpec::series(nnz, rp, col, val, degree, lo, hi, gamma, work), dtype, b, r, m, lc, nullptr,
                       sigma, q, alpha, beta, V, vstride, W, passes);
}

int lz_vector_lanczos(lz_handle *h, int64_t n, int64_t nnz, const int64_t *rp, const int32_t *col,
                      const void *val, lz_dtype dtype, int m, int64_t lc, const void *bvec,
                      void *q, void *alpha, void *beta, void *q0, void *q1, void *w)
{
    LZ_HANDLE_CHECK(h);
    LZ_TRY(check_csr(n, nnz, rp, col, val));
    LZ_ARG_CHECK(n >= 1 && m >= 1 && lc >= 0 && lc < n, "vector Lanczos sizes");
    LZ_ARG_CHECK(bvec && q && alpha && beta && q0 && q1 && w, "NULL buffer");
    LZ_ARG_CHECK(bvec != q0 && bvec != q1 && bvec != w && q0 != q1 && q0 != w && q1 != w,
                 "b, q0, q1, w must be distinct buffers");
    return by_dtype(dtype, [&](auto t) {
        using T = decltype(t);
        return vector_lanczos_dev<T>(h, n, nnz, rp, col, (const T *)val, m, lc, (const T *)bvec, (T *)q, (T *)alpha,
                                     (T *)beta, (T *)q0, (T *)q1, (T *)w);
    });
}

int lz_fdtd_block(lz_handle *h, int64_t n, int64_t nnz, const int64_t *rp, const int32_t *col,
                  const void *val, lz_dtype dtype, int b, const void *U0, int64_t steps,
                  double T_end, int64_t lc, void *U, void *D, void *out)
{
    LZ_HANDLE_CHECK(h);
    LZ_TRY(check_csr(n, nnz, rp, col, val));
    LZ_ARG_CHECK(steps >= 1 && lc >= 0 && lc < n && U0 && U && D && out, "fdtd args");
    return by_dtype(dtype, [&](auto t) {
        using T = decltype(t);
        return fdtd_block<T>(h, n, nnz, rp, col, (const T *)val, b, (const T *)U0, steps, T_end, lc, (T *)U, (T *)D,
                             (T *)out);
    });
}

int lz_comm_init(lz_handle *h, int nranks, int rank, const unsigned char id[128])
{
    LZ_HANDLE_CHECK(h);
    LZ_ARG_CHECK(nranks >= 1 && rank >= 0 && rank < nranks && id, "comm args");
    LZ_ARG_CHECK(h->comm == nullptr, "handle already has a communicator (lz_comm_destroy first)");
    Comm *c = nullptr;
    LZ_TRY(make_rccl_comm(nranks, rank, id, &c));
    return attach_comm(h, c);
}

int lz_debug_last_split(lz_handle *h, int64_t out[2])
{
    LZ_ARG_CHECK(h && out, "NULL argument");
    out[0] = h->last_split[0];
    out[1] = h->last_split[1];
    return LZ_OK;
}

int lz_debug_last_wf(lz_handle *h, int out[2])
{
    LZ_ARG_CHECK(h && out, "NULL argument");
    out[0] = h->last_wf;
    out[1] = h->last_wf_pre;
    return LZ_OK;
}

int lz_debug_last_kernel(lz_handle *h, int out[2])
{
    LZ_HANDLE_CHECK(h);
    out[0] = h->last_kernel[0];
    out[1] = h->last_kernel[1];
    return LZ_OK;
}

int lz_debug_wf_plan(lz_handle *h, int64_t n, int64_t nnz, const int64_t *row_ptr, const int32_t *col_idx,
                     int64_t nx, int64_t xoff, int32_t *deps_out, int16_t *col16_out, int32_t info[8])
{
    LZ_HANDLE_CHECK(h);
    LZ_ARG_CHECK(row_ptr && col_idx && deps_out && col16_out && info, "NULL argument");
    lz::WfPlan wp;
    LZ_TRY(lz::wf_plan16(h, n, nnz, row_ptr, col_idx, &wp, nx, xoff));
    const int64_t T = wp.tr > 0 ? lz::ceil_div(n, (int64_t)wp.tr) : 0;
    int sp[4] = {0, 0, 0, 0};
    if (wp.planned && T > 0) {
        LZ_HIP_TRY(hipMemcpyAsync(deps_out, h->wf_deps, sizeof(int32_t) * 2 * (size_t)T, hipMemcpyDeviceToDevice,
                                  h->stream));
        LZ_HIP_TRY(hipMemcpyAsync(sp, flag_word(h, kFlagPlanStats), sizeof(sp), hipMemcpyDeviceToHost, h->stream));
    } else if (T > 0) {
        LZ_HIP_TRY(hipMemsetAsync(deps_out, 0, sizeof(int32_t) * 2 * (size_t)T, h->stream));
    }
    if (nnz > 0) {
        if (wp.col16)
            LZ_HIP_TRY(hipMemcpyAsync(col16_out, wp.col16, sizeof(int16_t) * (size_t)nnz, hipMemcpyDeviceToDevice,
                                      h->stream));
        else
            LZ_HIP_TRY(hipMemsetAsync(col16_out, 0, sizeof(int16_t) * (size_t)nnz, h->stream));
    }
    LZ_HIP_TRY(hipStreamSynchronize(h->stream));
    info[0] = wp.ok ? 1 : 0;
    info[1] = wp.col16 ? 1 : 0;
    info[2] = (int32_t)T;
    info[3] = wp.tr;
    for (int i = 0; i < 4; ++i) info[4 + i] = sp[i];
    return LZ_OK;
}

int lz_comm_destroy(lz_handle *h)
{
    LZ_HANDLE_CHECK(h);
    detach_comm(h);
    return LZ_OK;
}

static int dist_args(lz_handle *h, lz_dtype dtype, int b, int m)
{
    LZ_ARG_CHECK(dtype == LZ_F64 || dtype == LZ_F32, "dtype");
    LZ_ARG_CHECK(b >= 1 && b <= 32, "distributed block Lanczos: 1 <= b <= 32");
    LZ_ARG_CHECK(m >= 1, "m >= 1");
    (void)h;
    return LZ_OK;
}

static int lz_block_lanczos_dist_impl(lz_handle *h, int64_t n_local, int64_t n_pad, int64_t n_global,
                          int64_t nnz_local, const int64_t *rp, const int32_t *col,
                          const void *val, lz_dtype dtype, int b, int m, int64_t lc_local,
                          int lc_rank, const void *B_local, void *q, void *alpha, void *beta,
                          void *Q0, void *Q1, void *W, void *X_full)
{
    LZ_HANDLE_CHECK(h);
    LZ_ARG_CHECK(h->comm != nullptr, "lz_comm_init first");
    LZ_TRY(check_csr(n_local, nnz_local, rp, col, val));
    LZ_TRY(dist_args(h, dtype, b, m));
    LZ_ARG_CHECK(n_local >= 1 && n_pad >= n_local && n_pad * h->nranks == n_global,
                 "dist sizes: n_pad >= n_local >= 1 and n_global == n_pad * nranks (padded numbering)");
    LZ_ARG_CHECK(B_local && q && alpha && beta && W && X_full, "NULL buffer");
    LZ_ARG_CHECK(W != X_full && B_local != X_full && B_local != W, "B_local, W, X_full must be distinct");
    (void)Q0;
    (void)Q1;
    const int64_t lc = (lc_rank == h->rank) ? lc_local : -1;
    return by_dtype(dtype, [&](auto t) {
        using T = decltype(t);
        return dist_solve<T>(h, kFormAllgather, nullptr, n_local, n_pad, nnz_local, rp, col, (const T *)val, b, m, lc,
                             (const T *)B_local, (T *)q, (T *)alpha, (T *)beta, (T *)X_full, (T *)W);
    });
}

int lz_block_lanczos_dist(lz_handle *h, int64_t n_local, int64_t n_pad, int64_t n_global,
                          int64_t nnz_local, const int64_t *rp, const int32_t *col,
                          const void *val, lz_dtype dtype, int b, int m, int64_t lc_local,
                          int lc_rank, const void *B_local, void *q, void *alpha, void *beta,
                          void *Q0, void *Q1, void *W, void *X_full)
{
    const uint64_t issued0 = comm_issued(h);
    const int rc = lz_block_lanczos_dist_impl(h, n_local, n_pad, n_global, nnz_local, rp, col, val, dtype, b, m,
                                              lc_local, lc_rank, B_local, q, alpha, beta, Q0, Q1, W, X_full);
    return dist_fail(h, rc, issued0);
}

static int halo_init_impl(lz_handle *h, int64_t row0, int64_t n_local, const int64_t *recv_counts,
                          const int32_t *halo_rows)
{
    LZ_ARG_CHECK(n_local >= 0 && row0 >= 0 && recv_counts, "halo args");
    const int nr = h->nranks;
    LZ_ARG_CHECK(nr == 1 || h->comm != nullptr, "lz_comm_init first");
    LZ_ARG_CHECK(recv_counts[h->rank] == 0, "recv_counts[rank] must be 0 (own rows are not halo)");
    halo_free(h);
    HaloPlan *hp = new HaloPlan();
    h->halo = hp;
    hp->n_local = n_local;
    hp->roff.assign(nr + 1, 0);
    hp->soff.assign(nr + 1, 0);
    for (int p = 0; p < nr; ++p) {
        LZ_ARG_CHECK(recv_counts[p] >= 0, "negative recv count");
        hp->roff[p + 1] = hp->roff[p] + recv_counts[p];
    }
    hp->n_halo = hp->roff[nr];
    LZ_ARG_CHECK(hp->n_halo == 0 || halo_rows, "halo_rows is NULL");
    LZ_ARG_CHECK(n_local + hp->n_halo < (1LL << 31), "n_local + n_halo must fit int32 columns");
    if (nr == 1) return LZ_OK;
    Comm *cm = h->comm;
    int64_t *dcnt = nullptr;
    LZ_HIP_TRY(hipMalloc(&dcnt, sizeof(int64_t) * 2 * nr));
    std::vector<int64_t> scnt(nr, 0);
    int rc = LZ_OK;
    do {
        if (hipMemcpyAsync(dcnt, recv_counts, sizeof(int64_t) * nr, hipMemcpyHostToDevice, h->stream) != hipSuccess ||
            hipMemsetAsync(dcnt + nr, 0, sizeof(int64_t) * nr, h->stream) != hipSuccess ||
            hipStreamSynchronize(h->stream) != hipSuccess) {
            set_error("lz_halo_init: staging counts failed");
            rc = LZ_E_HIP;
            break;
        }
        std::vector<P2POp> ops;
        for (int p = 0; p < nr; ++p)
            if (p != h->rank) ops.push_back(P2POp{p, dcnt + p, sizeof(int64_t), dcnt + nr + p, sizeof(int64_t)});
        rc = cm->exchange(ops.data(), (int)ops.size(), h->stream);
        if (rc != LZ_OK) break;
        if (hipStreamSynchronize(h->stream) != hipSuccess ||
            hipMemcpyAsync(scnt.data(), dcnt + nr, sizeof(int64_t) * nr, hipMemcpyDeviceToHost, h->stream) !=
                hipSuccess ||
            hipStreamSynchronize(h->stream) != hipSuccess) {
            set_error("lz_halo_init: reading counts failed");
            rc = LZ_E_HIP;
        }
    } while (0);
    if (rc == LZ_OK) rc = cm->fence(h->stream);
    (void)hipStreamSynchronize(h->stream);
    (void)hipFree(dcnt);
    if (rc != LZ_OK) return rc;
    for (int p = 0; p < nr; ++p) {
        LZ_ARG_CHECK(scnt[p] >= 0 && scnt[p] <= n_local, "peer requested more rows than this rank owns");
        hp->soff[p + 1] = hp->soff[p] + scnt[p];
    }
    hp->n_send = hp->soff[nr];
    int32_t *dreq = nullptr;
    LZ_HIP_TRY(hipMalloc(&dreq, sizeof(int32_t) * std::max<int64_t>(1, hp->n_halo)));
    LZ_HIP_TRY(hipMalloc(&hp->send_idx, sizeof(int32_t) * std::max<int64_t>(1, hp->n_send)));
    std::vector<int32_t> sidx(hp->n_send);
    do {
        if (hp->n_halo &&
            (hipMemcpyAsync(dreq, halo_rows, sizeof(int32_t) * hp->n_halo, hipMemcpyHostToDevice, h->stream) !=
                 hipSuccess ||
             hipStreamSynchronize(h->stream) != hipSuccess)) {
            set_error("lz_halo_init: staging requests failed");
            rc = LZ_E_HIP;
            break;
        }
        std::vector<P2POp> ops;
        for (int p = 0; p < nr; ++p) {
            if (p == h->rank) continue;
            const int64_t sc = hp->soff[p + 1] - hp->soff[p], rcv = hp->roff[p + 1] - hp->roff[p];
            if (sc || rcv)
                ops.push_back(P2POp{p, dreq + hp->roff[p], sizeof(int32_t) * (size_t)rcv, hp->send_idx + hp->soff[p],
                                    sizeof(int32_t) * (size_t)sc});
        }
        rc = cm->exchange(ops.data(), (int)ops.size(), h->stream);
        if (rc != LZ_OK) break;
        if (hipStreamSynchronize(h->stream) != hipSuccess ||
            (hp->n_send && (hipMemcpyAsync(sidx.data(), hp->send_idx, sizeof(int32_t) * hp->n_send,
                                           hipMemcpyDeviceToHost, h->stream) != hipSuccess ||
                            hipStreamSynchronize(h->stream) != hipSuccess))) {
            set_error("lz_halo_init: reading requests failed");
            rc = LZ_E_HIP;
        }
    } while (0);
    if (rc == LZ_OK) rc = cm->fence(h->stream);
    (void)hipStreamSynchronize(h->stream);
    (void)hipFree(dreq);
    if (rc != LZ_OK) return rc;
    hp->send_head = 0;
    hp->send_tail = n_local;
    for (int64_t i = 0; i < hp->n_send; ++i) {
        const int64_t g = (int64_t)sidx[i] - row0;
        LZ_ARG_CHECK(g >= 0 && g < n_local, "a peer requested a row this rank does not own");
        sidx[i] = (int32_t)g;
        if (2 * g < n_local) hp->send_head = std::max(hp->send_head, g + 1);
        else hp->send_tail = std::min(hp->send_tail, g);
// ... 74 lines not shown
```

### gpu-implementation-of-signle-and-block-lanczos_amd/csrc/lz_common.hpp

```cpp
#pragma once
#include <hip/hip_runtime.h>

#include <cstdint>
#include <cstdio>
#include <string>

#include "lz_hip.h"

namespace lz {

class Comm;

void set_error(const char *fmt, ...);

#define LZ_HIP_TRY(expr)                                                          \
    do {                                                                          \
        hipError_t e_ = (expr);                                                   \
        if (e_ != hipSuccess) {                                                   \
            ::lz::set_error("%s:%d %s -> %s", __FILE__, __LINE__, #expr,          \
                            hipGetErrorString(e_));                               \
            return LZ_E_HIP;                                                      \
        }                                                                         \
    } while (0)

#define LZ_ARG_CHECK(cond, msg)                                                   \
    do {                                                                          \
        if (!(cond)) {                                                            \
            ::lz::set_error("argument error: %s (%s)", msg, #cond);             \
            return LZ_E_ARG;                                                      \
        }                                                                         \
    } while (0)

#define LZ_LAUNCH_CHECK()                                                         \
    do {                                                                          \
        hipError_t e_ = hipGetLastError();                                        \
        if (e_ != hipSuccess) {                                                   \
            ::lz::set_error("%s:%d kernel launch -> %s", __FILE__, __LINE__,      \
                            hipGetErrorString(e_));                               \
            return LZ_E_HIP;                                                      \
        }                                                                         \
    } while (0)

#define LZ_TRY(expr)                                                              \
    do {                                                                          \
        int rc_ = (expr);                                                         \
        if (rc_ != LZ_OK) return rc_;                                             \
    } while (0)

constexpr int kWave = 64;
constexpr int kMaxPartials = 2048;
constexpr int kMaxB = 64;
constexpr int kMaxSolveB = 32;
constexpr size_t kScratchDoubles = 8 * kMaxB * kMaxB;
constexpr size_t kPartials2Doubles = 256 * kMaxB * kMaxB + 4096 * 256;

__host__ __device__ inline int64_t ceil_div(int64_t a, int64_t b) { return (a + b - 1) / b; }

}

struct lz_handle {
    int device = 0;
    hipStream_t stream = nullptr;
    hipStream_t side = nullptr;
    hipEvent_t ev_fork = nullptr, ev_join = nullptr;
    int n_cu = 256;
    int grid_cap = 0;
    double *partials = nullptr;
    size_t partials_cap = 0;
    double *partials2 = nullptr;
    double *scratch = nullptr;
    int *err_flag = nullptr;
    lz::Comm *comm = nullptr;
    int nranks = 1, rank = 0;
    hipStream_t xstream = nullptr;
    hipEvent_t ev_cx = nullptr, ev_xd = nullptr;
    hipEvent_t ev_bd = nullptr;
    int64_t last_split[2] = {-1, -1};
    int last_wf = 0, last_wf_pre = 0;
    int last_kernel[2] = {0, 0};
    int final_state = 1;
    int dbg_setup_fail = 0;
    void *c16buf = nullptr;
    size_t c16_cap = 0;
    int32_t *fnz_colf = nullptr, *fnz_trow = nullptr;
    int64_t fnz_key[4] = {0, 0, 0, 0};
    bool fnz_ok = false;
    void *wf_deps = nullptr;
    int *wf_flags = nullptr;
    size_t wf_deps_cap = 0, wf_flags_cap = 0;
    void *ybuf = nullptr;
    size_t ybuf_cap = 0;
    void *coef = nullptr;
    size_t coef_cap = 0;
    void *tr_ws = nullptr;
    size_t tr_cap = 0;
    void *halo = nullptr;
    uint64_t *pairs = nullptr;
    int *longq = nullptr;
    size_t longq_cap = 0;
    int longq_parity = 0;
    hipStream_t lstream = nullptr;
    hipEvent_t ev_lfork = nullptr, ev_ljoin = nullptr;
    hipStream_t pf_sg = nullptr, pf_sp = nullptr;
    hipEvent_t ev_pff = nullptr, ev_pfg = nullptr, ev_pfp = nullptr;
    int *pf_ctl = nullptr;
    int pf_key = -1;
    int pf_band = 0;
    int64_t pf_band_key[3] = {0, 0, -1};
    size_t pairs_cap = 0;
    void *cm_buf = nullptr;
    size_t cm_cap = 0;
    double *dots_ws = nullptr;
    size_t dots_cap = 0;
    void *cg_ws = nullptr;
    size_t cg_cap = 0;
    void *bcg_ws = nullptr;
    size_t bcg_cap = 0;
    bool prof = false;
    unsigned prof_mask = ~0u;
    hipEvent_t *ev_pool = nullptr;
    int ev_cap = 0, ev_used = 0;
    int ev_class[4096];
};

namespace lz {
enum ProfClass { PROF_SPMM_PASS = 0, PROF_UPDATE_PASS = 1, PROF_SMALL = 2, PROF_GRAM = 3,
                 PROF_TSMM = 4, PROF_SPMM = 5, PROF_NCLASS = 6 };
int prof_begin(lz_handle *h, int cls);
void prof_end(lz_handle *h, int idx);

int grow_ws(lz_handle *h, void **buf, size_t *cap_bytes, size_t bytes);
template <typename P>
inline int grow_ws(lz_handle *h, P **buf, size_t *cap_bytes, size_t bytes)
{
    return grow_ws(h, reinterpret_cast<void **>(buf), cap_bytes, bytes);
}
int grow_ws_poisoned(lz_handle *h, void **buf, size_t *cap_bytes, size_t bytes);
template <typename P>
inline int grow_ws_poisoned(lz_handle *h, P **buf, size_t *cap_bytes, size_t bytes)
{
    return grow_ws_poisoned(h, reinterpret_cast<void **>(buf), cap_bytes, bytes);
}
int ensure_partials(lz_handle *h, size_t doubles);
inline int c16_reserve(lz_handle *h, int64_t nnz)
{
    return grow_ws(h, &h->c16buf, &h->c16_cap, (size_t)nnz * 2 + 16);
}

enum FlagWord {
    kFlagErr = 0,
    kFlagLongTiles = 4,
    kFlagWindow = 8,
    kFlagCol16 = 9,
    kFlagTrCol = 10,
    kFlagPlanStats = 12,
    kFlagWords = 16
};
inline int *flag_word(lz_handle *h, FlagWord w) { return h->err_flag + w; }

struct Scratch16 {
    static constexpr size_t kBegin = 4 * 256, kEnd = kBegin + 4 * 256 + 3 * 256;
    double *binv[2], *P1, *P2, *slab;
    explicit Scratch16(lz_handle *h)
    {
        double *sc = h->scratch + kBegin;
        binv[0] = sc;
        binv[1] = sc + 256;
        P1 = sc + 2 * 256;
        P2 = sc + 3 * 256;
        slab = sc + 4 * 256;
    }
};
template <typename T>
struct ScratchT {
    static constexpr size_t kSlabEnd = kMaxSolveB * kMaxSolveB;
    static constexpr size_t kBegin = 4 * kMaxB * kMaxB, kEnd = kBegin + 4 * kMaxSolveB * kMaxSolveB;
    double *slab;
    T *binv[2], *P, *P3;
    ScratchT(lz_handle *h, int b) : slab(h->scratch)
    {
        T *sc = reinterpret_cast<T *>(h->scratch + kBegin);
        const int64_t bb = (int64_t)b * b;
        binv[0] = sc;
        binv[1] = sc + bb;
        P = sc + 2 * bb;
        P3 = sc + 3 * bb;
    }
};
struct ScratchSplit {
    static constexpr size_t kBegin = 7 * kMaxB * kMaxB, kEnd = kBegin + 2;
    unsigned long long *words;
    explicit ScratchSplit(lz_handle *h) : words(reinterpret_cast<unsigned long long *>(h->scratch + kBegin)) {}
};
static_assert(sizeof(unsigned long long) == sizeof(double), "split words are scratch doubles");
static_assert(Scratch16::kEnd <= kScratchDoubles && ScratchT<double>::kEnd <= kScratchDoubles &&
                  ScratchSplit::kEnd <= kScratchDoubles,
              "every view fits h->scratch");
static_assert(3 * 256 <= ScratchT<double>::kSlabEnd && ScratchT<double>::kSlabEnd <= Scratch16::kBegin &&
                  Scratch16::kEnd <= ScratchT<double>::kBegin && ScratchT<double>::kEnd <= ScratchSplit::kBegin,
              "scratch views do not overlap");
}
```

### gpu-implementation-of-signle-and-block-lanczos_amd/csrc/lz_internal.hpp

```cpp
#pragma once
#include "lz_common.hpp"

namespace lz {

template <typename T>
int spmm_rm(lz_handle *h, int64_t n, int64_t nnz, const int64_t *rp, const int32_t *col, const T *val, int b,
            const T *X, int64_t ldx, int64_t nx, T *Y, int64_t ldy,
            bool ycm = false);
template <typename T>
struct SpmmTerms {
    T a;
    const T *X;
    T c, d;
    const T *Z;
    T e = T(0);
    const T *U = nullptr;
    bool four = false;
};
template <typename T>
int spmm_terms(lz_handle *h, int64_t n, int64_t nnz, const int64_t *rp, const int32_t *col, const T *val, int b,
               SpmmTerms<T> t, T *Y, double *dots = nullptr, bool fused = true, bool fused_dot = true);
template <typename T>
int spmm_cm(lz_handle *h, int64_t n, int64_t nnz, const int64_t *rp, const int32_t *col, const T *val, int b,
            const T *X, int64_t ldx, int64_t nx, T *Y, int64_t ldy);

int dots_reserve(lz_handle *h, int64_t n, int b, int64_t min_slabs = 0);
template <typename T>
int col_dots(lz_handle *h, int64_t n, int b, const T *Y, const T *X, double *dots, bool zero_cross = false);
int dots_fold(lz_handle *h, int64_t P, int b, double *dots, bool zero_cross = false);
int slabs_fold(lz_handle *h, int64_t P, int bb, double *out, int zero_from = -1);

constexpr int kCgThreads = 256, kCgRows128 = 32, kCgGridCap = 2048, kCgCheckEvery = 8;
template <typename T>
int cg_update(lz_handle *h, int64_t n, int b, const double *coef, T *R, const T *W, T *P, T *S, T *X, double *rr);
template <typename T>
int cg_solve(lz_handle *h, int64_t n, int64_t nnz, const int64_t *rp, const int32_t *col, const T *val, int b,
             double shift, const T *B, T *X, T *work, const lz_cg_opts &o, int *iters, int *status, double *resid,
             double *est, int *info);
constexpr int kBcgThreads = 256, kBcgRows16 = 64, kBcgRows32 = 128, kBcgRowsGen = 16, kBcgGridCap = 1024, kBcgRuleThreads = 256;
template <typename T>
int bcg_update(lz_handle *h, int64_t n, int b, const double *xi, const double *E, const T *S, const T *W, T *Q, T *X,
               double *G);
template <typename T>
int bcg_direction(lz_handle *h, int64_t n, int b, const double *z, const double *zinv, T *Q, T *S);
template <typename T>
int bcg_solve(lz_handle *h, int64_t n, int64_t nnz, const int64_t *rp, const int32_t *col, const T *val, int b,
              double shift, const T *B, T *X, T *work, const lz_cg_opts &o, int *iters, int *status, double *resid,
              double *est, int *info);
template <typename T>
int cheb_moments(lz_handle *h, int64_t n, int64_t nnz, const int64_t *rp, const int32_t *col, const T *val, int b,
                 double lo, double hi, int K, const T *X0, T *work, double *dots, bool fused, bool fused_dot);
template <typename T>
int to_row_major(lz_handle *h, int64_t rows, int b, const T *src, int64_t ld, T *dst);
template <typename T>
int spmv(lz_handle *h, int64_t n, const int64_t *rp, const int32_t *col, const T *val, const T *x,
         T *y, int64_t nnz_hint);

constexpr int kTrShort = 16;
constexpr int kTrLds = 4096;
constexpr int kTrScanThreads = 256, kTrScanPer = 8, kTrScanBlock = kTrScanThreads * kTrScanPer;
constexpr int kTrSortThreads = 1024;
static_assert((kTrLds & (kTrLds - 1)) == 0 && (kTrScanThreads & (kTrScanThreads - 1)) == 0, "powers of two");
template <typename T>
int csr_transpose(lz_handle *h, int64_t n_rows, int64_t n_cols, int64_t nnz, const int64_t *rp, const int32_t *col,
                  const T *val, int64_t *t_rp, int32_t *t_col, T *t_val);

template <typename T>
int gram_partials(lz_handle *h, int64_t n, int b, const T *X, const T *Y, int64_t ld, int *nparts);
template <typename T>
int gram_finish(lz_handle *h, int b, int nparts, int mode, T *R, const double *slabs = nullptr,
                const T *L = nullptr, T *LR = nullptr);
struct WfAlpha {
    const double *part = nullptr;
    int P = 0;
    double *alpha = nullptr, *P2 = nullptr;
    const double *V = nullptr;
    int64_t lc = -1;
    double *qrow = nullptr;
};
template <typename T>
int sqrtm_pair(lz_handle *h, int b, const T *G, int nparts, T *beta, T *beta_inv, T *eig,
               const double *slabs = nullptr, const T *L = nullptr, T *LB = nullptr,
               const WfAlpha *wa = nullptr);
template <typename T>
int tsmm(lz_handle *h, int64_t n, int b, T sw, T sq, const T *Q, const T *S, T *W, int64_t ld);
template <typename T>
int copy_row(lz_handle *h, int b, const T *Q, int64_t ld, int col_major, int64_t lc, T *q);
template <typename T>
int final_state(lz_handle *h, int64_t n, int b, const T *Y, const T *Vp, const T *Vq, const T *Wm, const T *binv,
                const T *P1, const T *P2, T *Wout, T *Q0, T *Q1);
template <typename T>
int to_col_major(lz_handle *h, int64_t rows, int b, const T *src, int64_t ld, T *dst);

constexpr int kPanelMaxK = 64;
constexpr int kPanelG16 = 16;
constexpr int kPanelGGen = 4;
template <typename T>
int panel_gram(lz_handle *h, int64_t n, int b, int k, const T *V, int64_t vstride, const T *W, T *C);
int panel_gram_reserve(lz_handle *h, int64_t n, int b, int kmax, bool f64);
template <typename T>
int panel_apply(lz_handle *h, int64_t n, int b, int k, double sw, double sq, const T *V, int64_t vstride, const T *S,
                T *W);
constexpr int kPanelMaxKeep = 16;
template <typename T>
int panel_compress(lz_handle *h, int64_t n, int b, int k, int r, T *V, int64_t vstride, const T *Z);

int fused_spmm16(lz_handle *h, int64_t n, const int64_t *rp, const int32_t *col,
                 const double *val, const double *Wg, int64_t nx, const double *Wown, const double *Wprev,
                 double *Wn, const double *binv, const double *P1, int64_t lc, double *qrow, int *nparts,
                 const uint64_t *pairs, int64_t nnz, int64_t row_off, int win, int slab_off = 0,
                 const int16_t *col16 = nullptr);
int col16_plan(lz_handle *h, int64_t n, int64_t nnz, const int64_t *rp, const int32_t *col, int64_t row_off,
               const int16_t **out);
bool fused16_direct(int64_t nx, int win);
int gather_window_ok(lz_handle *h, int64_t n, const int64_t *rp, const int32_t *col, int64_t nx, int64_t row_off,
                     bool *ok);
int strip_pairs(lz_handle *h, int64_t n, const int64_t *rp, const uint64_t **out);
int fused_update16(lz_handle *h, int64_t n, double *Wn, const double *Wcur, const double *P2,
                   int *nparts);
int fused_update16_swap(lz_handle *h, int64_t n, double *Wn, double *Xown, const double *alpha, int *nparts);
int mm16(lz_handle *h, const double *A, const double *B, double *C);

struct WfPlan {
    bool ok = false;
    int hback = 0, hfwd = 0;
    int nc = 12, tr = 192;
    int var = 0;
    const int16_t *col16 = nullptr;
    int64_t xoff = 0;
    bool planned = false;
};
bool wf_first_gram(int64_t n, int64_t nnz);
int wf_plan16(lz_handle *h, int64_t n, int64_t nnz, const int64_t *rp, const int32_t *col, WfPlan *pl,
              int64_t nx = -1, int64_t xoff = 0);
int wf_reset16(lz_handle *h, int64_t n, const WfPlan &pl);
struct WfTiles {
    int64_t a, b;
};
struct WfPass2 {
    const double *Yj, *Vprev, *Vj;
    double *Vout;
    const double *binv, *P1, *P2;
    double *Vsave = nullptr;
};
struct WfPass1 {
    const double *Vg;
    double *Yo;
    WfTiles t;
    bool gram = false;
};
struct WfLaunch {
    enum Role { kFirst, kBoundary, kStep, kPass2, kPostCall } role;
    WfPass1 p1;
    WfPass2 p2;
    WfTiles q, q2;
    int epoch = 0;
    double *Q0 = nullptr, *Q1 = nullptr;
};
struct WfSolve {
    int64_t n;
    const int64_t *rp;
    const int32_t *col;
    const double *val;
    const uint64_t *pairs;
    const WfPlan &pl;
    int64_t nx;
    int64_t T() const { return (n + pl.tr - 1) / pl.tr; }
    WfTiles all() const { return {0, T()}; }
    WfTiles none() const { return {T(), T()}; }
    WfLaunch first(const double *Vg, double *Yo, bool gram) const
    {
        return {WfLaunch::kFirst, {Vg, Yo, all(), gram}, {}, all(), none()};
    }
    WfLaunch boundary(const double *Vg, double *Yo, WfTiles t) const
    {
        return {WfLaunch::kBoundary, {Vg, Yo, t}, {}, all(), none()};
    }
    WfLaunch step(const WfPass2 &p2, WfTiles q, const WfPass1 &p1, int epoch) const
    {
        return {WfLaunch::kStep, p1, p2, q, none(), epoch};
    }
    WfLaunch pass2(const WfPass2 &p2, WfTiles qa, WfTiles qb, int epoch) const
    {
        return {WfLaunch::kPass2, {p2.Vout - 16 * pl.xoff, const_cast<double *>(p2.Yj), {0, 0}}, p2, qa, qb, epoch};
    }
    WfLaunch post_call(const WfPass2 &p2, int epoch, double *Q0, double *Q1) const
    {
        return {WfLaunch::kPostCall, {p2.Vout, nullptr, {0, 0}}, p2, all(), none(), epoch, Q0, Q1};
    }
};
int wf_step16(lz_handle *h, const WfSolve &ws, const WfLaunch &L, double *part, int *nparts);
struct WfSlabs {
    static constexpr int kMax = 6;
    const double *p[kMax] = {};
    int g[kMax] = {};
    int k = 0;
    void add(const double *ptr, int nslab)
    {
        p[k] = ptr;
        g[k] = nslab;
        ++k;
    }
};
int wf_fold16(lz_handle *h, const WfSlabs &sl, double *out);
int alpha_wf16(lz_handle *h, const double *part, int P, const double *binv, const double *P1, double *alpha,
               double *P2, const double *V, int64_t lc, int64_t n, double *qrow);

int fused_e32(lz_handle *h, int64_t n, const float *Y, const float *Wj, const float *Wprev, float *Wn,
              const float *binv, const float *P1, int64_t lc, float *qrow, int *nparts);
int fused_u32(lz_handle *h, int64_t n, float *Wn, const float *Wj, const float *P2, int *nparts);
int fused_el32(lz_handle *h, int64_t n, const float *Wj, const float *U, int *nparts);
int fused_ub32(lz_handle *h, int64_t n, const float *U, const float *Wj, const float *binv, const float *P2,
               float *Wn, int *nparts, float *Qa = nullptr,
               float *Qb = nullptr);
int alpha_b2(lz_handle *h, const double *part, int P, const float *binv, float *alpha, float *P2, const float *Wj,
             int64_t lc, int64_t n, float *qrow);
int m_b2(lz_handle *h, const double *part, int P, const float *binv, float *M);
bool spmm_b2_ok(int64_t n, int64_t nnz, int64_t nx);
int fold_slabs_g(lz_handle *h, const double *part, int64_t P, int bb, int G);
int spmm_rm_b2(lz_handle *h, int64_t n, int64_t nnz, const int64_t *rp, const int32_t *col, const float *val,
               const float *X, int64_t nx, float *Y, const float *Wp, const float *Mm, int plan_slot = -1,
               int *slot_out = nullptr, int cap = 768);
int spmm_b2_stage(lz_handle *h, int64_t n, const int64_t *rp, int *cap);
int spmm_b2_plan(lz_handle *h, int64_t n, const int64_t *rp, int cap, int *slot);
template <typename T>
int fused_e_sep(lz_handle *h, int64_t n, int b, const T *Y, const T *Wj, const T *Wprev, T *Wn, const T *binv,
                const T *P1, int64_t lc, T *qrow, int *nparts);
template <typename T>
int fused_u_sep(lz_handle *h, int64_t n, int b, T *Wn, const T *Wj, const T *P2, int *nparts);
template <typename T>
int fused_u_swap_sep(lz_handle *h, int64_t n, int b, T *Wn, T *Xown, const T *P2, int *nparts);

template <typename T>
int vector_lanczos_dev(lz_handle *h, int64_t n, int64_t nnz, const int64_t *rp, const int32_t *col,
                       const T *val, int m, int64_t lc, const T *b, T *q, T *alpha, T *beta, T *q0,
                       T *q1, T *w);

}
```

### gpu-implementation-of-signle-and-block-lanczos_amd/csrc/lz_wf.hip

```cpp
#include <climits>
#include <mutex>
#include <unordered_map>

#include "lz_internal.hpp"
#include "lz_kernels.hpp"

namespace lz {

constexpr int kWfK = 3, kWfNL = 2;
constexpr int kWfCapPerRow = 11;
constexpr int kWfWideCap = 4400;
constexpr double kWfWideRow = 27.0;
constexpr int kWfMaxSpan = 1024;
constexpr int kWfAux = 16;
constexpr long kWfSpin = 1L << 21;

__global__ __launch_bounds__(256) void k_wf_deps(int64_t n, int TR, const int64_t *__restrict__ rp,
                                                 const int32_t *__restrict__ col, int2 *__restrict__ deps,
                                                 int16_t *__restrict__ col16, int *__restrict__ spans, int64_t xoff,
                                                 int win)
{
    __shared__ int smin[4], smax[4];
    const int64_t T = ceil_div(n, (int64_t)TR);
    const int lane = threadIdx.x & 63, w = threadIdx.x >> 6;
    const int ns = TR / 16;
    int sb = 0, sf = 0, sw = 0, bad = 0, far = 0;
    for (int64_t t = blockIdx.x; t < T; t += gridDim.x) {
        int mn = INT_MAX, mx = -1;
        for (int s = w; s < ns; s += 4) {
            const int64_t s0 = t * TR + 16 * s;
            if (s0 >= n) break;
            const int64_t s1 = s0 + 16 < n ? s0 + 16 : n;
            for (int64_t k = rp[s0] + lane, e = rp[s1]; k < e; k += 64) {
                const int64_t c = (int64_t)col[k] - xoff;
                if (c >= 0 && c < n) {
                    mn = c < mn ? (int)c : mn;
                    mx = c > mx ? (int)c : mx;
                }
                const int64_t d = c - s0;
                if (win) far |= (d < -(kWinRows / 2) + 32) | (d > kWinRows / 2 - 32);
                if (col16) {
                    bad |= (d < -32768) | (d > 32767);
                    col16[k] = (int16_t)d;
                }
            }
        }
#pragma unroll
        for (int o = 32; o > 0; o >>= 1) {
            const int a = __shfl_xor(mn, o, 64), b = __shfl_xor(mx, o, 64);
            mn = a < mn ? a : mn;
            mx = b > mx ? b : mx;
        }
        if (lane == 0) {
            smin[w] = mn;
            smax[w] = mx;
        }
        __syncthreads();
        if (threadIdx.x == 0) {
            for (int i = 1; i < 4; ++i) {
                mn = smin[i] < mn ? smin[i] : mn;
                mx = smax[i] > mx ? smax[i] : mx;
            }
            int lo = (int)t, hi = (int)t;
            if (mx >= 0) {
                const int a = (int)(mn / TR), b = (int)(mx / TR);
                lo = a < lo ? a : lo;
                hi = b > hi ? b : hi;
            }
            deps[t] = make_int2(lo, hi);
            sb = (int)t - lo > sb ? (int)t - lo : sb;
            sf = hi - (int)t > sf ? hi - (int)t : sf;
            sw = hi - lo + 1 > sw ? hi - lo + 1 : sw;
        }
        __syncthreads();
    }
    if (__ballot(bad) != 0 && lane == 0) atomicOr(&spans[3], 1);
    if (__ballot(far) != 0 && lane == 0) atomicOr(&spans[3], 2);
    if (threadIdx.x == 0) {
        atomicMax(&spans[0], sb);
        atomicMax(&spans[1], sf);
        atomicMax(&spans[2], sw);
    }
}

typedef unsigned v4u32_t __attribute__((ext_vector_type(4)));
typedef double d2_t __attribute__((ext_vector_type(2)));

__device__ __forceinline__ double dpp_swap1(double x)
{
    int2 v;
    __builtin_memcpy(&v, &x, 8);
    v.x = __builtin_amdgcn_mov_dpp(v.x, 0xB1, 0xF, 0xF, false);
    v.y = __builtin_amdgcn_mov_dpp(v.y, 0xB1, 0xF, 0xF, false);
    double r;
    __builtin_memcpy(&r, &v, 8);
    return r;
}

template <int NC, int CAP, int K, int NL, int NU, int DU, bool C16, bool SW = false, bool GEN = true, int XO = 0>
__global__ __launch_bounds__(64 * (NC + NL + NU)) void k_wf16(
    int64_t n, const int64_t *__restrict__ rp, const int32_t *__restrict__ col, const int16_t *__restrict__ col16,
    const double *__restrict__ val, const uint64_t *__restrict__ pairs, const double *Yj, const double *Vprev,
    const double *Vj, double *Vout, const double *__restrict__ binv, const double *__restrict__ P1,
    const double *__restrict__ P2, const double *Vg, double *Yo, const int2 *__restrict__ deps, int *flags, int epoch,
    int64_t hback, int lead, double *__restrict__ part, int *__restrict__ err, int dbg, int64_t nx, int64_t p1a,
    int64_t p1b, int64_t Th, int cpol, int64_t xoff, int64_t q0, int64_t q1, int64_t q2, int64_t q3, double *Vsave)
{
    using CT = typename std::conditional<C16, int16_t, int32_t>::type;
    using C = FwCfg<NC, CAP, true, true, CT>;
    constexpr int TR = C::TR;
    constexpr int GA = kWfAux, SA = kWfAux;
    static_assert(NC > 3 && NC <= kPairPad, "strips per tile");
    __shared__ typename C::Stage st[K];
    __shared__ double scr[NC][256];
    __shared__ double ust[NU][DU + 1][3][256];
    __shared__ int ready[K], done[K], cons_in, upd_in;
    __shared__ int p1pub;
    const int lane = threadIdx.x & 63, w = __builtin_amdgcn_readfirstlane(threadIdx.x >> 6);
    const bool has_p2 = P2 != nullptr, has_prev = P1 != nullptr;
    constexpr bool kG0 = XO == 1 && DU >= 1 && NU * DU * 3 >= NC;
    constexpr bool QO = XO == 2;
    const bool g0 = kG0 && !has_p2 && Vj != nullptr;
    if (threadIdx.x < K) {
        ready[threadIdx.x] = -1;
        done[threadIdx.x] = 0;
    }
    if (threadIdx.x == 0) {
        cons_in = 0;
        p1pub = 0;
        upd_in = 0;
    }
    __syncthreads();
    const int64_t T = ceil_div(n, (int64_t)TR);
    static_assert(GEN || !SW, "SW stores are a distributed form");
    static_assert(!(SW && XO == 2), "Vsave carries either V_j (SW) or Q (XO 2)");
    if constexpr (!GEN) {
        xoff = 0;
        q0 = 0;
        q1 = q2 = q3 = T;
        nx = n;
    }
    if (T != Th || blockDim.x != 64 * (NC + NL + NU) || (kG0 != (!has_p2 && Vj != nullptr))) {
        if (threadIdx.x == 0) *err = 7;
        return;
    }
    const int64_t G = gridDim.x, bid = blockIdx.x;
    int64_t begin, end, kb, KB, pbeg, pend;
    const int64_t NP1 = p1b - p1a, nq1 = q1 - q0, NQ = nq1 + (q3 - q2);
    auto ptile = [&](int64_t v) {
        if constexpr (!GEN) return v;
        return v < nq1 ? q0 + v : q2 + (v - nq1);
    };
    auto clampq = [&](int64_t v) { return v < 0 ? (int64_t)0 : (v > NQ ? NQ : v); };
    if (G < 8) {
        begin = p1a; end = p1b; kb = bid; KB = G; pbeg = 0; pend = NQ;
    } else {
        const int64_t x = bid & 7;
        begin = p1a + NP1 * x / 8;
        end = p1a + NP1 * (x + 1) / 8;
        kb = bid >> 3;
        KB = (G - x + 7) >> 3;
        if (NP1 > 0) {
            pbeg = x == 0 ? 0 : clampq(begin - hback - q0);
            pend = x == 7 ? NQ : clampq(end - hback - q0);
        } else {
            pbeg = NQ * x / 8;
            pend = NQ * (x + 1) / 8;
        }
    }
    int64_t nt = (end - begin - kb + KB - 1) / KB > 0 ? (end - begin - kb + KB - 1) / KB : 0;
    if (dbg & 4) nt = 0;
    auto tile_of = [&](int64_t i) { return begin + kb + i * KB; };
    if (w < NL) {
        __builtin_amdgcn_s_setprio(3);
        const int64_t nnz = rp[n];
        for (int64_t i = w; i < nt; i += NL) {
            const int s = (int)(i % K);
            const int64_t t = tile_of(i);
            const int64_t r0 = t * TR, r1 = (r0 + TR < n) ? r0 + TR : n;
            const int64_t kA = rp[r0];
            if (i >= K) {
                long spin = 0;
                const uint32_t da = ws_lds_addr(&done[s]);
                while (ws_lds_read(da) < NC * (int)(i / K) && ++spin < kWsSpin) __builtin_amdgcn_s_sleep(1);
                if (spin >= kWsSpin) { *err = 3; break; }
            }
            const int64_t ca = kA & ~(int64_t)(C::CPP - 1), va = kA & ~(int64_t)1;
            const int64_t cb = ((nnz - ca) * (int64_t)sizeof(CT) + 3) & ~(int64_t)3, vb = (nnz - va) * 8;
            const auto rr = __builtin_amdgcn_make_buffer_rsrc(const_cast<int64_t *>(rp + r0), (short)0,
                                                              (int)((r1 - r0 + 1) * 8), 0x00020000);
            const CT *cbase = C16 ? reinterpret_cast<const CT *>(col16) : reinterpret_cast<const CT *>(col);
            const auto cr = __builtin_amdgcn_make_buffer_rsrc(const_cast<CT *>(cbase + ca), (short)0,
                                                              (int)(cb < 0x7fffffff ? cb : 0x7fffffff), 0x00020000);
            const auto vr = __builtin_amdgcn_make_buffer_rsrc(const_cast<double *>(val + va), (short)0,
                                                              (int)(vb < 0x7fffffff ? vb : 0x7fffffff), 0x00020000);
            const int64_t s0i = r0 / 16, ns = (n + 15) / 16 + kPairPad;
            const auto pr = __builtin_amdgcn_make_buffer_rsrc(const_cast<uint64_t *>(pairs + s0i), (short)0,
                                                              (int)((ns - s0i) * 8), 0x00020000);
            if (cpol & 2) {
                ws_dma<2>(rr, st[s].rp, C::RP_PIECES, lane);
                ws_dma<2>(cr, st[s].col, C::COL_PIECES, lane);
                ws_dma<2>(vr, st[s].val, C::VAL_PIECES, lane);
                ws_dma<2>(pr, st[s].pr, C::PR_PIECES, lane);
            } else {
                ws_dma(rr, st[s].rp, C::RP_PIECES, lane);
                ws_dma(cr, st[s].col, C::COL_PIECES, lane);
                ws_dma(vr, st[s].val, C::VAL_PIECES, lane);
                ws_dma(pr, st[s].pr, C::PR_PIECES, lane);
            }
            asm volatile("s_waitcnt vmcnt(0)" ::: "memory");
            if (has_p2 && !(dbg & 1)) {
                const int2 d = deps[t];
                long spin = 0;
                for (int lo = d.x; lo <= d.y && spin < kWfSpin; lo += 64) {
                    const int idx = lo + lane;
                    for (;;) {
                        const int f = idx <= d.y
                                          ? __hip_atomic_load(flags + idx, __ATOMIC_RELAXED, __HIP_MEMORY_SCOPE_AGENT)
                                          : epoch;
                        if (__ballot(f != epoch) == 0) break;
                        if (++spin >= kWfSpin) break;
                        __builtin_amdgcn_s_sleep(2);
                    }
                }
                if (spin >= kWfSpin) { *err = 5; break; }
            }
            if (lane == 0) {
                ws_lds_write(ws_lds_addr(&ready[s]), (int)i);
                asm volatile("ds_add_u32 %0, %1" ::"v"(ws_lds_addr(&p1pub)), "v"(1) : "memory");
            }
        }
        return;
    }
    if (w < NL + NU) {
        const int uw = w - NL;
        d4_t gacc = {0.0, 0.0, 0.0, 0.0}, sacc = {0.0, 0.0, 0.0, 0.0};
        if (has_p2 && !(dbg & 2)) {
            if (dbg & 8) __builtin_amdgcn_s_setprio(0);
            else if (dbg & 64) __builtin_amdgcn_s_setprio(3);
            else __builtin_amdgcn_s_setprio(2);
            const int c = lane & 15, g = lane >> 4;
            double bq[3][4];
#pragma unroll
            for (int kc = 0; kc < 4; ++kc) {
                const int idx = (4 * g + kc) * 16 + c;
                bq[0][kc] = binv[idx];
                bq[1][kc] = has_prev ? -P1[idx] : 0.0;
                bq[2][kc] = -P2[idx];
            }
            const int64_t ut0 = pbeg + kb + uw * KB, ustep = (int64_t)NU * KB;
            const int64_t ntl = ut0 < pend ? (pend - ut0 + ustep - 1) / ustep : 0;
            const int64_t ns = ntl * NC;
            const int bytes = (int)(n * 128);
            const __amdgpu_buffer_rsrc_t rs[3] = {
                __builtin_amdgcn_make_buffer_rsrc(const_cast<double *>(Yj), (short)0, bytes, 0x00020000),
                __builtin_amdgcn_make_buffer_rsrc(const_cast<double *>(has_prev ? Vprev : Vj), (short)0,
                                                  has_prev ? bytes : 0, 0x00020000),
                __builtin_amdgcn_make_buffer_rsrc(const_cast<double *>(Vj), (short)0, bytes, 0x00020000)};
            const auto Or = __builtin_amdgcn_make_buffer_rsrc(Vout, (short)0, bytes, 0x00020000);
            const auto Sr = __builtin_amdgcn_make_buffer_rsrc(SW || QO ? Vsave : Vout, (short)0, SW || QO ? bytes : 0,
                                                              0x00020000);
            const auto Qr = __builtin_amdgcn_make_buffer_rsrc(QO && Yo ? Yo : Vout, (short)0, QO && Yo ? bytes : 0,
                                                              0x00020000);
            auto strip_r0 = [&](int64_t s) { return ptile(ut0 + (s / NC) * ustep) * TR + 16 * (s % NC); };
            uint32_t goff[2];
#pragma unroll
            for (int k = 0; k < 2; ++k) {
                const int q = 64 * k + lane, row = q >> 3;
                goff[k] = (uint32_t)(row * 128 + 16 * ((q & 7) ^ ((row >> 1) & 7)));
            }
            const int64_t gap = begin - (NQ > 0 ? ptile(pbeg < NQ ? pbeg : NQ - 1) : 0) - hback;
            const int64_t poff = gap > 0 ? (gap + KB - 1) / KB : 0;
            int64_t paced = -1;
            auto pace = [&](int64_t s) {
                const int64_t m = uw + (s / NC) * NU - poff;
                if (s >= ns || s / NC <= paced) return;
                paced = s / NC;
                const uint32_t pa = ws_lds_addr(&p1pub);
                const int target = (int)(m - lead < nt ? m - lead : nt);
                long spin = 0;
                while (ws_lds_read(pa) < target && ++spin < kWsSpin) __builtin_amdgcn_s_sleep(2);
                if (spin >= kWsSpin) *err = 6;
            };
            auto dma = [&](int64_t s) {
                const int slot = (int)(s % (DU + 1));
                const bool live = s < ns;
                if (!(dbg & 32)) pace(s);
                const uint32_t rb = live ? (uint32_t)(strip_r0(s) * 128) : 0u;
#pragma unroll
                for (int m = 0; m < 3; ++m)
#pragma unroll
                    for (int k = 0; k < 2; ++k) {
                        ws_lds_t *dst = (ws_lds_t *)((char *)&ust[uw][slot][m][0] + 1024 * k);
                        const uint32_t off = live ? rb + goff[k] : 0x80000000u;
                        if (cpol & 1) __builtin_amdgcn_raw_ptr_buffer_load_lds(rs[m], dst, 16, off, 0, 0, 2);
                        else __builtin_amdgcn_raw_ptr_buffer_load_lds(rs[m], dst, 16, off, 0, 0, 0);
                    }
            };
            const int ra = c;
            const uint32_t oa0 = (uint32_t)(ra * 128 + 16 * ((2 * g) ^ ((ra >> 1) & 7)));
            const uint32_t oa1 = (uint32_t)(ra * 128 + 16 * ((2 * g + 1) ^ ((ra >> 1) & 7)));
            uint32_t oc[4];
#pragma unroll
            for (int r = 0; r < 4; ++r) {
                const int row = 4 * r + g;
                oc[r] = (uint32_t)(2 * 2048 + row * 128 + 16 * ((c >> 1) ^ ((row >> 1) & 7)) + 8 * (c & 1));
            }
            const bool ev = (c & 1) == 0;
#pragma unroll
            for (int s = 0; s < DU; ++s) dma(s);
            for (int64_t s = 0; s < ns; ++s) {
                dma(s + DU);
                constexpr int ST = SW ? 4 : QO ? 6 : 2;
                if (s < DU) asm volatile("s_waitcnt vmcnt(%0)" ::"n"(6 * DU) : "memory");
                else asm volatile("s_waitcnt vmcnt(%0)" ::"n"((6 + ST) * DU) : "memory");
                if (s % NC == DU && s >= NC && lane == 0)
                    __hip_atomic_store(flags + ptile(ut0 + (s / NC - 1) * ustep), epoch, __ATOMIC_RELAXED,
                                       __HIP_MEMORY_SCOPE_AGENT);
                const uint32_t sb = ws_lds_addr(reinterpret_cast<int *>(&ust[uw][(int)(s % (DU + 1))][0][0]));
                d2_t y0, y1, p0, p1, j0, j1;
                double vc0, vc1, vc2, vc3;
                asm volatile(
                    "ds_read_b128 %0, %10\n\t"
                    "ds_read_b128 %1, %11\n\t"
                    "ds_read_b128 %2, %10 offset:2048\n\t"
                    "ds_read_b128 %3, %11 offset:2048\n\t"
                    "ds_read_b128 %4, %10 offset:4096\n\t"
                    "ds_read_b128 %5, %11 offset:4096\n\t"
                    "ds_read_b64 %6, %12\n\t"
                    "ds_read_b64 %7, %13\n\t"
                    "ds_read_b64 %8, %14\n\t"
                    "ds_read_b64 %9, %15\n\t"
                    "s_waitcnt lgkmcnt(0)"
                    : "=&v"(y0), "=&v"(y1), "=&v"(p0), "=&v"(p1), "=&v"(j0), "=&v"(j1), "=&v"(vc0), "=&v"(vc1),
                      "=&v"(vc2), "=&v"(vc3)
                    : "v"(sb + oa0), "v"(sb + oa1), "v"(sb + oc[0]), "v"(sb + oc[1]), "v"(sb + oc[2]),
                      "v"(sb + oc[3])
                    : "memory");
                const double ya[4] = {y0.x, y0.y, y1.x, y1.y}, pa[4] = {p0.x, p0.y, p1.x, p1.y},
                             ja[4] = {j0.x, j0.y, j1.x, j1.y}, vjc[4] = {vc0, vc1, vc2, vc3};
                d4_t acc = {0.0, 0.0, 0.0, 0.0};
                if (dbg & 16) {
                    acc = d4_t{pa[0] + ya[0], pa[1] + ya[1], ja[2] + vjc[2], ja[3] + vjc[3]};
                } else {
#pragma unroll
                for (int kc = 0; kc < 4; ++kc) acc = mfma16(pa[kc], bq[1][kc], acc);
#pragma unroll
                for (int kc = 0; kc < 4; ++kc) acc = mfma16(ya[kc], bq[0][kc], acc);
#pragma unroll
                for (int kc = 0; kc < 4; ++kc) acc = mfma16(ja[kc], bq[2][kc], acc);
#pragma unroll
                for (int r = 0; r < 4; ++r) gacc = mfma16(acc[r], acc[r], gacc);
#pragma unroll
                for (int r = 0; r < 4; ++r) sacc = mfma16(acc[r], vjc[r], sacc);
                }
                const uint32_t r0b = (uint32_t)(strip_r0(s) * 128);
#pragma unroll
                for (int h2 = 0; h2 < 2; ++h2) {
                    const double a0 = acc[2 * h2], a1 = acc[2 * h2 + 1];
                    const double y = dpp_swap1(ev ? a1 : a0);
                    const double2 v = ev ? make_double2(a0, y) : make_double2(y, a1);
                    const int row = 4 * (2 * h2 + (ev ? 0 : 1)) + g;
                    const uint32_t off = r0b + (uint32_t)(row * 128 + (ev ? c : c - 1) * 8);
                    if (cpol & 8) __builtin_amdgcn_raw_buffer_store_b128(*reinterpret_cast<const v4u32_t *>(&v), Or, off, 0, SA | 2);
                    else if (dbg & 128)
                        __builtin_amdgcn_raw_buffer_store_b128(*reinterpret_cast<const v4u32_t *>(&v), Or, off, 0, 0);
                    else __builtin_amdgcn_raw_buffer_store_b128(*reinterpret_cast<const v4u32_t *>(&v), Or, off, 0, SA);
                }
                if constexpr (QO) {
                    d4_t qa = {0.0, 0.0, 0.0, 0.0};
#pragma unroll
                    for (int kc = 0; kc < 4; ++kc) qa = mfma16(ja[kc], bq[0][kc], qa);
#pragma unroll
                    for (int h2 = 0; h2 < 2; ++h2) {
                        const double a0 = qa[2 * h2], a1 = qa[2 * h2 + 1];
                        const double y = dpp_swap1(ev ? a1 : a0);
                        const double2 v = ev ? make_double2(a0, y) : make_double2(y, a1);
                        const int row = 4 * (2 * h2 + (ev ? 0 : 1)) + g;
                        const uint32_t off = r0b + (uint32_t)(row * 128 + (ev ? c : c - 1) * 8);
                        __builtin_amdgcn_raw_buffer_store_b128(*reinterpret_cast<const v4u32_t *>(&v), Sr, off, 0, 0);
                        __builtin_amdgcn_raw_buffer_store_b128(*reinterpret_cast<const v4u32_t *>(&v), Qr, off, 0, 0);
                    }
                }
                if constexpr (SW) {
                    v4u32_t vp0, vp1;
                    asm volatile(
                        "ds_read_b128 %0, %2 offset:4096\n\t"
                        "ds_read_b128 %1, %2 offset:5120\n\t"
                        "s_waitcnt lgkmcnt(0)"
                        : "=&v"(vp0), "=&v"(vp1)
                        : "v"(sb + 16u * (uint32_t)lane)
                        : "memory");
                    __builtin_amdgcn_raw_buffer_store_b128(vp0, Sr, r0b + goff[0], 0, 2);
                    __builtin_amdgcn_raw_buffer_store_b128(vp1, Sr, r0b + goff[1], 0, 2);
                }
            }
            asm volatile("s_waitcnt vmcnt(0)" ::: "memory");
            if (ntl > 0 && lane == 0)
                __hip_atomic_store(flags + ptile(ut0 + (ntl - 1) * ustep), epoch, __ATOMIC_RELAXED,
                                   __HIP_MEMORY_SCOPE_AGENT);
        }
        double *U = &ust[uw][0][0][0];
#pragma unroll
        for (int r = 0; r < 4; ++r) {
            U[((lane >> 4) + 4 * r) * 16 + (lane & 15)] = gacc[r];
            U[256 + ((lane >> 4) + 4 * r) * 16 + (lane & 15)] = sacc[r];
        }
        int arrived = 0;
        if (lane == 0) arrived = __hip_atomic_fetch_add(&upd_in, 1, __ATOMIC_ACQ_REL, __HIP_MEMORY_SCOPE_WORKGROUP);
        arrived = __shfl(arrived, 0, 64);
        if (arrived == NU - 1) {
            __builtin_amdgcn_fence(__ATOMIC_ACQUIRE, "workgroup");
            for (int e = lane; e < 512; e += 64) {
                double a = 0.0;
                for (int u = 0; u < NU; ++u) a += ust[u][0][0][e];
                if (!(g0 && e < 256)) part[(e < 256 ? 2 * G : G) * 256 + bid * 256 + (e & 255)] = a;
            }
        }
        return;
    }
    const int cw = w - NL - NU;
    {
        const int pr = (cw * 3) / NC;
        if (pr == 1) __builtin_amdgcn_s_setprio(1);
        else if (pr == 2) __builtin_amdgcn_s_setprio(2);
    }
    const int bytes = (int)(n * 128);
    const bool win = GEN && nx >= kWinRows;
    auto xwin = [&](int64_t s0, int64_t &wb) {
        const int64_t c = xoff + s0 - kWinRows / 2;
        wb = win ? (c > 0 ? c : 0) : 0;
        const int64_t rows = win ? (nx - wb < kWinRows ? nx - wb : kWinRows) : nx;
        return __builtin_amdgcn_make_buffer_rsrc(const_cast<double *>(Vg + wb * 16), (short)0, (int)(rows * 128),
                                                 0x00020000);
    };
    int64_t wb0 = 0;
    auto xr = xwin(0, wb0);
    const auto yr = __builtin_amdgcn_make_buffer_rsrc(Yo, (short)0, bytes, 0x00020000);
    double *S0 = scr[cw];
    d4_t macc = {0.0, 0.0, 0.0, 0.0}, gcc = {0.0, 0.0, 0.0, 0.0};
    double v1[4] = {0.0, 0.0, 0.0, 0.0};
    int64_t s0p = -1;
    auto epilogue = [&]() {
        double ya[4], va[4];
        const bool ev = (lane & 1) == 0;
#pragma unroll
        for (int h2 = 0; h2 < 2; ++h2) {
            const double x = v1[2 * h2], y = v1[2 * h2 + 1];
            const double got = dpp_swap1(ev ? y : x);
            va[2 * h2] = ev ? x : got;
            va[2 * h2 + 1] = ev ? got : y;
        }
#pragma unroll
        for (int r = 0; r < 4; ++r) ya[r] = S0[fw_sw(4 * r + (lane >> 4), lane & 15)];
#pragma unroll
        for (int r = 0; r < 4; ++r) macc = mfma16(va[r], ya[r], macc);
        if (g0) {
#pragma unroll
            for (int r = 0; r < 4; ++r) gcc = mfma16(va[r], va[r], gcc);
        }
    };
    for (int64_t i = 0; i < nt; ++i) {
        const int s = (int)(i % K);
        const int64_t r0 = tile_of(i) * TR;
        const int64_t s0 = r0 + 16 * cw;
        const int g = lane >> 3, p = lane & 7;
        const uint32_t lane_off = 16u * p;
        int64_t wb = 0;
        if (win) xr = xwin(s0, wb);
        long spin = 0;
        while (__hip_atomic_load(&ready[s], __ATOMIC_RELAXED, __HIP_MEMORY_SCOPE_WORKGROUP) != (int)i &&
               ++spin < kWsSpin)
            __builtin_amdgcn_s_sleep(1);
        if (spin >= kWsSpin) { *err = 4; break; }
        asm volatile("" ::: "memory");
        typename C::Stage &S = st[s];
        const int64_t kA = S.rp[0];
        const int co = (int)(kA & (C::CPP - 1)), vo = (int)(kA & 1);
        const int nrow = (int)(n - r0 < TR ? n - r0 : TR);
        const int runlen = (int)(S.rp[nrow] - kA);
        const uint64_t pw = S.pr[cw];
        const int ra = (int)(pw >> (4 * g)) & 15, rb = (int)(pw >> (4 * (15 - g))) & 15;
        const int lra = 16 * cw + ra, lrb = 16 * cw + rb;
        const int o0 = lra < nrow ? (int)(S.rp[lra] - kA) : 0;
        const int len0 = lra < nrow ? (int)(S.rp[lra + 1] - kA) - o0 : 0;
        const int o1 = lrb < nrow ? (int)(S.rp[lrb] - kA) : 0;
        const int len1 = lrb < nrow ? (int)(S.rp[lrb + 1] - kA) - o1 : 0;
        const int cnt = len0 + len1;
        double y[4] = {0.0, 0.0, 0.0, 0.0};
        if (runlen <= CAP) {
            const CT *cp = S.col + co;
            const uint32_t cb16 = C16 ? (uint32_t)(xoff + s0 - wb) : (uint32_t)(-wb);
            const double *vp = S.val + vo;
            auto slot = [&](int ff) {
                const int o = ff < len0 ? o0 + ff : o1 + (ff - len0);
                return ff < cnt ? o : o0;
            };
            auto issue = [&](int f, double2 *xs) {
                int32_t cc[8];
#pragma unroll
                for (int tt = 0; tt < 8; ++tt) cc[tt] = cp[slot(f + tt)];
#pragma unroll
                for (int tt = 0; tt < 8; ++tt) {
                    const uint32_t off = f + tt < cnt ? __umul24((unsigned)cc[tt] + cb16, 128u) + lane_off
                                                      : 0x80000000u;
                    const auto u4 = __builtin_amdgcn_raw_buffer_load_b128(xr, off, 0, GA);
                    __builtin_memcpy(&xs[tt], &u4, 16);
                }
            };
            auto fmas = [&](int f, const double2 *xs) {
#pragma unroll
                for (int tt = 0; tt < 8; ++tt) {
                    const double v = vp[slot(f + tt)];
                    if (f + tt < len0) {
                        y[0] = fma(v, xs[tt].x, y[0]);
                        y[1] = fma(v, xs[tt].y, y[1]);
                    } else {
                        y[2] = fma(v, xs[tt].x, y[2]);
                        y[3] = fma(v, xs[tt].y, y[3]);
                    }
                }
            };
            double2 xs[8];
            issue(0, xs);
            if (s0p >= 0) epilogue();
            fmas(0, xs);
            for (int f = 8; f < cnt; f += 8) {
                issue(f, xs);
                fmas(f, xs);
            }
        } else {
            if (s0p >= 0) epilogue();
            ws_gather<const int32_t *, const double *, GA>(col + kA, val + kA, o0, len0, o1, cnt, xr, lane_off,
                                                               y, (uint32_t)wb);
        }
        asm volatile("s_waitcnt lgkmcnt(0)" ::: "memory");
        if (lane == 0) atomicAdd(&done[s], 1);
        {
            const auto st0 = make_double2(y[0], y[1]), st1 = make_double2(y[2], y[3]);
            const uint32_t oa = (uint32_t)((s0 + ra) * 128) + lane_off, ob = (uint32_t)((s0 + rb) * 128) + lane_off;
            const uint32_t fa = s0 + ra < n ? oa : 0x80000000u, fb = s0 + rb < n ? ob : 0x80000000u;
            if (cpol & 4) {
                __builtin_amdgcn_raw_buffer_store_b128(*reinterpret_cast<const v4u32_t *>(&st0), yr, fa, 0, 2);
                __builtin_amdgcn_raw_buffer_store_b128(*reinterpret_cast<const v4u32_t *>(&st1), yr, fb, 0, 2);
            } else {
                __builtin_amdgcn_raw_buffer_store_b128(*reinterpret_cast<const v4u32_t *>(&st0), yr, fa, 0, 0);
                __builtin_amdgcn_raw_buffer_store_b128(*reinterpret_cast<const v4u32_t *>(&st1), yr, fb, 0, 0);
            }
        }
        S0[fw_sw(ra, 2 * p)] = y[0];
        S0[fw_sw(ra, 2 * p + 1)] = y[1];
        S0[fw_sw(rb, 2 * p)] = y[2];
        S0[fw_sw(rb, 2 * p + 1)] = y[3];
#pragma unroll
        for (int h2 = 0; h2 < 2; ++h2) {
            const int c = lane & 15;
            const int64_t row = s0 + 8 * h2 + 4 * (c & 1) + (lane >> 4);
            const uint32_t off = row < n ? (uint32_t)((xoff + row - wb) * 128 + (c & ~1) * 8) : 0x80000000u;
            const auto u = __builtin_amdgcn_raw_buffer_load_b128(xr, off, 0, GA);
            __builtin_memcpy(&v1[2 * h2], &u, 16);
        }
        s0p = s0;
        wave_lds_sync();
    }
    if (s0p >= 0) epilogue();
    auto gslab = [&](int c) { return &ust[(c / 3) % NU][1 + c / (3 * NU)][c % 3][0]; };
#pragma unroll
    for (int r = 0; r < 4; ++r) S0[((lane >> 4) + 4 * r) * 16 + (lane & 15)] = macc[r];
    if (g0) {
        double *Gs = gslab(cw);
#pragma unroll
        for (int r = 0; r < 4; ++r) Gs[((lane >> 4) + 4 * r) * 16 + (lane & 15)] = gcc[r];
    }
    int arrived = 0;
    if (lane == 0) arrived = __hip_atomic_fetch_add(&cons_in, 1, __ATOMIC_ACQ_REL, __HIP_MEMORY_SCOPE_WORKGROUP);
    arrived = __shfl(arrived, 0, 64);
    if (arrived == NC - 1) {
        __builtin_amdgcn_fence(__ATOMIC_ACQUIRE, "workgroup");
        double *slab = part + bid * 256;
        for (int e = lane; e < 256; e += 64) {
            double a[4] = {0.0, 0.0, 0.0, 0.0};
            int sl = 0;
            for (; sl + 3 < NC; sl += 4) {
#pragma unroll
                for (int q = 0; q < 4; ++q) a[q] += scr[sl + q][e];
            }
            for (; sl < NC; ++sl) a[0] += scr[sl][e];
            slab[e] = (a[0] + a[1]) + (a[2] + a[3]);
        }
        if (g0) {
            double *gout = part + (2 * G + bid) * 256;
            for (int e = lane; e < 256; e += 64) {
                double a = 0.0;
                for (int c = 0; c < NC; ++c) a += gslab(c)[e];
                gout[e] = a;
            }
        }
    }
}

static int wf_shape(int64_t n, int64_t nnz, int *nc, bool *allowed)
{
    const char *e = getenv("LZ_PASS_WF");
    const char *sh = getenv("LZ_WF_SHAPE");
    const int want = sh ? atoi(sh) : 111;
    const bool wide = (double)nnz > 10.2 * (double)n;
    const int var = wide ? 200 : (want == 10 || want == 11 || want == 12) ? 0 : 111;
    *nc = var == 200 ? 10 : var ? 11 : want;
    *allowed = !(e && e[0] == '0') && n < (1 << 24);
    return var;
}

bool wf_first_gram(int64_t n, int64_t nnz)
{
    int nc = 0;
    bool allowed = false;
    return wf_shape(n, nnz, &nc, &allowed) == 111 && allowed;
}

int wf_plan16(lz_handle *h, int64_t n, int64_t nnz, const int64_t *rp, const int32_t *col, WfPlan *pl, int64_t nx,
              int64_t xoff)
{
    if (nx < 0) nx = n;
    pl->ok = false;
    pl->planned = false;
    pl->col16 = nullptr;
    bool allowed = false;
    pl->var = wf_shape(n, nnz, &pl->nc, &allowed);
    pl->tr = 16 * pl->nc;
    if (!allowed || n < pl->tr || xoff < 0 || xoff + n > nx ||
        (double)nnz > kWfWideRow * (double)n)
        return LZ_OK;
    const int64_t T = ceil_div(n, (int64_t)pl->tr);
    LZ_TRY(grow_ws(h, &h->wf_deps, &h->wf_deps_cap, sizeof(int2) * (size_t)(T + 64)));
    LZ_TRY(grow_ws(h, &h->wf_flags, &h->wf_flags_cap, sizeof(int) * (size_t)(T + 64)));
    const char *c = getenv("LZ_PASS1_C16");
    int16_t *c16 = nullptr;
    if (!(c && c[0] == '0') && nnz > 0) {
        LZ_TRY(c16_reserve(h, nnz));
        c16 = static_cast<int16_t *>(h->c16buf);
    }
    int *spans = flag_word(h, kFlagPlanStats);
    LZ_HIP_TRY(hipMemsetAsync(spans, 0, 4 * sizeof(int), h->stream));
    const int grid = (int)std::max<int64_t>(1, std::min<int64_t>(T, (int64_t)h->n_cu * 8));
    hipLaunchKernelGGL(k_wf_deps, dim3(grid), dim3(256), 0, h->stream, n, pl->tr, rp, col,
                       static_cast<int2 *>(h->wf_deps), c16, spans, xoff, nx >= kWinRows ? 1 : 0);
    LZ_LAUNCH_CHECK();
    int sp[4] = {0, 0, 0, 1};
    LZ_HIP_TRY(hipMemcpyAsync(sp, spans, sizeof(sp), hipMemcpyDeviceToHost, h->stream));
    LZ_HIP_TRY(hipStreamSynchronize(h->stream));
    pl->planned = true;
    pl->hback = sp[0];
    pl->hfwd = sp[1];
    pl->ok = sp[2] <= kWfMaxSpan && !(sp[3] & 2);
    pl->xoff = xoff;
    if (c16 && !(sp[3] & 1)) pl->col16 = c16;
    return LZ_OK;
}

int wf_step16(lz_handle *h, const WfSolve &ws, const WfLaunch &L, double *part, int *nparts)
{
    const WfPlan &pl = ws.pl;
    const WfPass1 &p1 = L.p1;
    const WfPass2 &p2 = L.p2;
    const int64_t n = ws.n, nx = ws.nx, T = ws.T(), xoff = pl.xoff;
    const int64_t p1a = p1.t.a, p1b = p1.t.b, q0 = L.q.a, q1 = L.q.b, q2 = L.q2.a, q3 = L.q2.b;
    const bool has_p2 = L.role >= WfLaunch::kStep, qo = L.role == WfLaunch::kPostCall;
    const bool g0 = L.role == WfLaunch::kFirst && p1.gram;
    const bool sw = has_p2 && p2.Vsave != nullptr;
    const int16_t *col16 = pl.col16;
    LZ_ARG_CHECK(xoff >= 0 && xoff + n <= nx && 0 <= p1a && p1a <= p1b && p1b <= T, "wavefront step ranges");
    LZ_ARG_CHECK(0 <= q0 && q0 <= q1 && q1 <= q2 && q2 <= q3 && q3 <= T, "wavefront step pass-2 ranges");
    LZ_ARG_CHECK(pl.ok && n < (1 << 24), "wavefront step: wf_plan16 first");
    LZ_ARG_CHECK(ws.pairs != nullptr, "strip row orders (strip_pairs) missing");
    LZ_ARG_CHECK(!has_p2 || (p2.Yj && p2.Vj && p2.Vout && p2.binv && p2.P2 && p2.Vout == p1.Vg + 16 * xoff),
                 "wavefront step buffers");
    LZ_ARG_CHECK(!sw || (pl.var != 0 && !qo), "wavefront step: SW stores (the 111 / wide shapes)");
    LZ_ARG_CHECK(!qo || (L.Q0 && pl.var == 111 && xoff == 0 && nx == n),
                 "wavefront post-call state: a one-GPU launch of the default shape");
    LZ_ARG_CHECK(!g0 || pl.var == 111, "wavefront first launch with beta_0's Gram: the default shape only (internal)");
    static_assert(12 <= kPairPad, "row orders must cover the last tile's strips");
    const int64_t nq = (q1 - q0) + (q3 - q2);
    const int64_t work = has_p2 ? std::max(nq, p1b - p1a) : p1b - p1a;
    if (work <= 0) {
        *nparts = 0;
        return LZ_OK;
    }
    const char *gc = getenv("LZ_GRID_CAP");
    const int cap = gc && atoi(gc) > 0 ? atoi(gc) : (h->grid_cap > 0 ? h->grid_cap : h->n_cu);
    const int grid = (int)std::max<int64_t>(1, std::min<int64_t>(work, std::min(cap, h->n_cu)));
#ifdef LZ_DIAG
    const char *dg = getenv("LZ_WF_DBG");
    const int dbg = dg ? atoi(dg) : 0;
#else
    constexpr int dbg = 0;
#endif
    const int KB = grid < 8 ? grid : grid / 8;
    const int lmin = (int)((pl.hback + pl.hfwd + KB - 1) / KB) + 2;
#ifndef LZ_WF_LEAD_ADD
#define LZ_WF_LEAD_ADD 3
#endif
    const int lead = lmin + (pl.var ? LZ_WF_LEAD_ADD : 4);
    constexpr int cpol = 7;
    int rc = LZ_OK;
    const int ev = qo ? -1 : prof_begin(h, PROF_SPMM_PASS);
    auto go = [&](auto kern, int waves) {
        int occ = -1;
        {
            static std::mutex mu;
            static std::unordered_map<const void *, int> occ_cache;
            std::lock_guard<std::mutex> lk(mu);
            const auto it = occ_cache.find(reinterpret_cast<const void *>(kern));
            if (it != occ_cache.end()) {
                occ = it->second;
            } else {
                if (hipOccupancyMaxActiveBlocksPerMultiprocessor(&occ, kern, 64 * waves, 0) != hipSuccess) occ = 0;
                occ_cache.emplace(reinterpret_cast<const void *>(kern), occ);
            }
        }
        if ((int64_t)grid > (int64_t)occ * h->n_cu) {
            set_error("wavefront step: %d blocks of %d threads cannot all be resident (%d per CU x %d CUs)", grid,
                      64 * waves, occ, h->n_cu);
            rc = LZ_E_HIP;
            return;
        }
        hipLaunchKernelGGL(kern, dim3(grid), dim3(64 * waves), 0, h->stream, n, ws.rp, ws.col, col16, ws.val, ws.pairs,
                           p2.Yj, p2.Vprev, g0 ? p1.Vg : p2.Vj, p2.Vout, p2.binv, p2.P1, p2.P2, p1.Vg,
                           qo ? L.Q1 : p1.Yo, static_cast<const int2 *>(h->wf_deps), h->wf_flags, L.epoch,
                           (int64_t)pl.hback, lead, part, h->err_flag, dbg, nx, p1a, p1b, T, cpol, xoff, q0, q1, q2, q3,
                           qo ? L.Q0 : p2.Vsave);
    };
    constexpr int cap12 = 12 * 16 * kWfCapPerRow, cap11 = 11 * 16 * kWfCapPerRow, cap10 = 10 * 16 * kWfCapPerRow;
    const bool one = !sw && xoff == 0 && nx == n && q0 == 0 && q1 == T && q2 == T && q3 == T;
#ifdef LZ_WF_GEN_ONLY
    const bool spec = false;
    (void)one;
#else
    const bool spec = one;
#endif
    if (qo && col16) go(k_wf16<11, cap11, kWfK, 1, 4, 1, true, false, false, 2>, 11 + 1 + 4);
    else if (qo) go(k_wf16<11, cap11, kWfK, 1, 4, 1, false, false, false, 2>, 11 + 1 + 4);
    else if (g0 && col16 && spec) go(k_wf16<11, cap11, kWfK, 1, 4, 1, true, false, false, 1>, 11 + 1 + 4);
    else if (g0 && col16) go(k_wf16<11, cap11, kWfK, 1, 4, 1, true, false, true, 1>, 11 + 1 + 4);
    else if (g0 && spec) go(k_wf16<11, cap11, kWfK, 1, 4, 1, false, false, false, 1>, 11 + 1 + 4);
    else if (g0) go(k_wf16<11, cap11, kWfK, 1, 4, 1, false, false, true, 1>, 11 + 1 + 4);
    else if (pl.var == 200 && col16 && sw) go(k_wf16<10, kWfWideCap, 2, 1, 3, 1, true, true>, 10 + 1 + 3);
    else if (pl.var == 200 && col16 && spec) go(k_wf16<10, kWfWideCap, 2, 1, 3, 1, true, false, false>, 10 + 1 + 3);
    else if (pl.var == 200 && col16) go(k_wf16<10, kWfWideCap, 2, 1, 3, 1, true>, 10 + 1 + 3);
    else if (pl.var == 200 && sw) go(k_wf16<10, kWfWideCap, 2, 1, 2, 1, false, true>, 10 + 1 + 2);
    else if (pl.var == 200 && spec) go(k_wf16<10, kWfWideCap, 2, 1, 2, 1, false, false, false>, 10 + 1 + 2);
    else if (pl.var == 200) go(k_wf16<10, kWfWideCap, 2, 1, 2, 1, false>, 10 + 1 + 2);
    else if (pl.var == 111 && col16 && sw) go(k_wf16<11, cap11, kWfK, 1, 4, 1, true, true>, 11 + 1 + 4);
    else if (pl.var == 111 && col16 && spec) go(k_wf16<11, cap11, kWfK, 1, 4, 1, true, false, false>, 11 + 1 + 4);
    else if (pl.var == 111 && col16) go(k_wf16<11, cap11, kWfK, 1, 4, 1, true>, 11 + 1 + 4);
    else if (pl.var == 111 && sw) go(k_wf16<11, cap11, kWfK, 1, 4, 1, false, true>, 11 + 1 + 4);
    else if (pl.var == 111 && spec) go(k_wf16<11, cap11, kWfK, 1, 4, 1, false, false, false>, 11 + 1 + 4);
    else if (pl.var == 111) go(k_wf16<11, cap11, kWfK, 1, 4, 1, false>, 11 + 1 + 4);
    else if (col16) {
        if (pl.nc == 12) go(k_wf16<12, cap12, kWfK, kWfNL, 2, 3, true>, 12 + kWfNL + 2);
        else if (pl.nc == 11) go(k_wf16<11, cap11, kWfK, kWfNL, 3, 2, true>, 11 + kWfNL + 3);
        else go(k_wf16<10, cap10, kWfK, kWfNL, 4, 2, true>, 10 + kWfNL + 4);
    } else {
        if (pl.nc == 12) go(k_wf16<12, cap12, kWfK, kWfNL, 2, 2, false>, 12 + kWfNL + 2);
        else if (pl.nc == 11) go(k_wf16<11, cap11, kWfK, kWfNL, 3, 2, false>, 11 + kWfNL + 3);
        else go(k_wf16<10, cap10, kWfK, kWfNL, 4, 1, false>, 10 + kWfNL + 4);
    }
    prof_end(h, ev);
    LZ_TRY(rc);
    LZ_LAUNCH_CHECK();
    *nparts = grid;
    return LZ_OK;
}

__global__ __launch_bounds__(1024) void k_wf_fold(WfSlabs sl, double *__restrict__ out)
{
    __shared__ double ps[16][64];
    const int m = blockIdx.x >> 2, q = threadIdx.x >> 6, i = (blockIdx.x & 3) * 64 + (threadIdx.x & 63);
    auto sum = [&](const double *p, int P) {
        double a0 = 0.0, a1 = 0.0, a2 = 0.0, a3 = 0.0;
        int g = q;
        for (; g + 48 < P; g += 64) {
            a0 += p[(int64_t)g * 256 + i];
            a1 += p[(int64_t)(g + 16) * 256 + i];
            a2 += p[(int64_t)(g + 32) * 256 + i];
            a3 += p[(int64_t)(g + 48) * 256 + i];
        }
        for (; g < P; g += 16) a0 += p[(int64_t)g * 256 + i];
        return (a0 + a1) + (a2 + a3);
    };
    double s = 0.0;
    for (int t = 0; t < sl.k; ++t)
        if (sl.g[t] > 0) s = t == 0 ? sum(sl.p[t] + (int64_t)m * sl.g[t] * 256, sl.g[t])
                                    : s + sum(sl.p[t] + (int64_t)m * sl.g[t] * 256, sl.g[t]);
    ps[q][threadIdx.x & 63] = s;
    __syncthreads();
    if (q == 0) {
        const int l = threadIdx.x & 63;
        double t[4];
#pragma unroll
        for (int k = 0; k < 4; ++k) t[k] = (ps[4 * k][l] + ps[4 * k + 1][l]) + (ps[4 * k + 2][l] + ps[4 * k + 3][l]);
        out[m * 256 + i] = (t[0] + t[1]) + (t[2] + t[3]);
    }
}

int wf_fold16(lz_handle *h, const WfSlabs &sl, double *out)
{
    LZ_ARG_CHECK(sl.k >= 1 && sl.k <= WfSlabs::kMax, "wavefront fold: 1..6 slab sets");
    const int ev = prof_begin(h, PROF_SMALL);
    hipLaunchKernelGGL(k_wf_fold, dim3(12), dim3(1024), 0, h->stream, sl, out);
    prof_end(h, ev);
    LZ_LAUNCH_CHECK();
    return LZ_OK;
}

int wf_reset16(lz_handle *h, int64_t n, const WfPlan &pl)
{
    const int64_t T = ceil_div(n, (int64_t)pl.tr);
    LZ_ARG_CHECK(sizeof(int) * (size_t)T <= h->wf_flags_cap, "wf_plan16 first");
    LZ_HIP_TRY(hipMemsetAsync(h->wf_flags, 0, sizeof(int) * (size_t)T, h->stream));
    return LZ_OK;
}

}
```

### include/lz_hip.h

```cpp
#ifndef LZ_HIP_H
#define LZ_HIP_H
#include <stddef.h>
#include <stdint.h>

#ifdef __cplusplus
extern "C" {
#endif

typedef enum { LZ_F64 = 0, LZ_F32 = 1 } lz_dtype;
typedef enum { LZ_ROW_MAJOR = 0, LZ_COL_MAJOR = 1 } lz_layout;

enum {
    LZ_OK = 0,
    LZ_E_ARG = -1,
    LZ_E_HIP = -2,
    LZ_E_COMM = -3,
    LZ_E_STATE = -4,
    LZ_E_DEVICE = -5
};

typedef struct lz_handle lz_handle;

int lz_init(int device, lz_handle **h);
int lz_finalize(lz_handle *h);
// ... 55 lines not shown
                   const void *V, int64_t vstride, const void *S, void *W);
#define LZ_PANEL_MAX_KEEP 16
int lz_panel_compress(lz_handle *h, int64_t n, int b, int k, int r, lz_dtype dtype, void *V, int64_t vstride,
                      const void *Z);

int lz_block_lanczos_reorth(lz_handle *h, int64_t n, int64_t nnz, const int64_t *row_ptr,
                            const int32_t *col, const void *val, lz_dtype dtype, int b, int m,
                            int64_t lc, const void *B, void *q, void *alpha, void *beta, void *V,
                            int64_t vstride, void *W, int passes);

int lz_block_lanczos_reorth_resume(lz_handle *h, int64_t n, int64_t nnz, const int64_t *row_ptr,
                                   const int32_t *col, const void *val, lz_dtype dtype, int b, int r, int m,
                                   int64_t lc, const void *sigma, void *q, void *alpha, void *beta, void *V,
                                   int64_t vstride, void *W, int passes);

int lz_csr_spmm_axpby(lz_handle *h, int64_t n, int64_t nnz, const int64_t *row_ptr, const int32_t *col,
                      const void *val, lz_dtype dtype, int b, double a, const void *X, double c, double d,
                      const void *Z, void *Y);

typedef struct {
    int degree;
    double lo, hi, ref;
} lz_cheb;
int lz_cheb_apply(lz_handle *h, int64_t n, int64_t nnz, const int64_t *row_ptr, const int32_t *col,
                  const void *val, lz_dtype dtype, int b, const lz_cheb *f, const void *X, void *Y, void *work);

int lz_col_dots(lz_handle *h, int64_t n, int b, lz_dtype dtype, const void *Y, const void *X, double *dots);
int lz_csr_spmm_axpby_dots(lz_handle *h, int64_t n, int64_t nnz, const int64_t *row_ptr, const int32_t *col,
                           const void *val, lz_dtype dtype, int b, double a, const void *X, double c, double d,
                           const void *Z, void *Y, double *dots);
int lz_cheb_moments(lz_handle *h, int64_t n, int64_t nnz, const int64_t *row_ptr, const int32_t *col,
                    const void *val, lz_dtype dtype, int b, double lo, double hi, int K, const void *X0, void *work,
                    double *dots);
int lz_block_lanczos_reorth_cheb(lz_handle *h, int64_t n, int64_t nnz, const int64_t *row_ptr,
                                 const int32_t *col, const void *val, lz_dtype dtype, int b, int m,
                                 int64_t lc, const void *B, void *q, void *alpha, void *beta, void *V,
                                 int64_t vstride, void *W, int passes, const lz_cheb *f, void *work);
int lz_block_lanczos_reorth_resume_cheb(lz_handle *h, int64_t n, int64_t nnz, const int64_t *row_ptr,
                                        const int32_t *col, const void *val, lz_dtype dtype, int b, int r, int m,
                                        int64_t lc, const void *sigma, void *q, void *alpha, void *beta, void *V,
                                        int64_t vstride, void *W, int passes, const lz_cheb *f, void *work);

int lz_csr_spmm_axpby4(lz_handle *h, int64_t n, int64_t nnz, const int64_t *row_ptr, const int32_t *col,
                       const void *val, lz_dtype dtype, int b, double a, const void *X, double c, double d,
                       const void *Z, double e, const void *U, void *Y);
int lz_cheb_series_apply(lz_handle *h, int64_t n, int64_t nnz, const int64_t *row_ptr, const int32_t *col,
                         const void *val, lz_dtype dtype, int b, int degree, double lo, double hi,
                         const double *gamma, const void *X, void *Y, void *work);
int lz_block_lanczos_reorth_series(lz_handle *h, int64_t n, int64_t nnz, const int64_t *row_ptr,
                                   const int32_t *col, const void *val, lz_dtype dtype, int b, int m,
                                   int64_t lc, const void *B, void *q, void *alpha, void *beta, void *V,
                                   int64_t vstride, void *W, int passes, int degree, double lo, double hi,
                                   const double *gamma, void *work);
int lz_block_lanczos_reorth_resume_series(lz_handle *h, int64_t n, int64_t nnz, const int64_t *row_ptr,
                                          const int32_t *col, const void *val, lz_dtype dtype, int b, int r, int m,
                                          int64_t lc, const void *sigma, void *q, void *alpha, void *beta, void *V,
                                          int64_t vstride, void *W, int passes, int degree, double lo, double hi,
                                          const double *gamma, void *work);

int lz_cg_update(lz_handle *h, int64_t n, int b, lz_dtype dtype, const double *coef, void *R, const void *W, void *P,
                 void *S, void *X, double *rr);
typedef struct {
    double tol;
    int max_iter, check_every, max_restarts;
} lz_cg_opts;
int lz_cg_solve(lz_handle *h, int64_t n, int64_t nnz, const int64_t *row_ptr, const int32_t *col, const void *val,
                lz_dtype dtype, int b, double shift, const void *B, void *X, void *work, const lz_cg_opts *opts,
                int *iters, int *status, double *resid, double *est, int *info);

int lz_bcg_update(lz_handle *h, int64_t n, int b, lz_dtype dtype, const double *xi, const double *E, const void *S,
                  const void *W, void *Q, void *X, double *G);
int lz_bcg_direction(lz_handle *h, int64_t n, int b, lz_dtype dtype, const double *z, const double *zinv, void *Q,
                     void *S);
int lz_bcg_solve(lz_handle *h, int64_t n, int64_t nnz, const int64_t *row_ptr, const int32_t *col, const void *val,
                 lz_dtype dtype, int b, double shift, const void *B, void *X, void *work, const lz_cg_opts *opts,
                 int *iters, int *status, double *resid, double *est, int *info);

int lz_csr_transpose(lz_handle *h, int64_t n_rows, int64_t n_cols, int64_t nnz,
                     const int64_t *row_ptr, const int32_t *col, const void *val, lz_dtype dtype,
                     int64_t *t_row_ptr, int32_t *t_col, void *t_val);

int lz_normal_apply(lz_handle *h, int64_t n, int64_t p, int64_t nnz, const int64_t *row_ptr, const int32_t *col,
                    const void *val, const int64_t *t_row_ptr, const int32_t *t_col, const void *t_val,
                    lz_dtype dtype, int b, const void *X, void *Y, void *work);
int lz_block_lanczos_reorth_normal(lz_handle *h, int64_t n, int64_t p, int64_t nnz, const int64_t *row_ptr,
                                   const int32_t *col, const void *val, const int64_t *t_row_ptr,
                                   const int32_t *t_col, const void *t_val, lz_dtype dtype, int b, int m, int64_t lc,
                                   const void *B, void *q, void *alpha, void *beta, void *V, int64_t vstride, void *W,
                                   int passes, void *work);
int lz_block_lanczos_reorth_resume_normal(lz_handle *h, int64_t n, int64_t p, int64_t nnz, const int64_t *row_ptr,
                                          const int32_t *col, const void *val, const int64_t *t_row_ptr,
                                          const int32_t *t_col, const void *t_val, lz_dtype dtype, int b, int r, int m,
                                          int64_t lc, const void *sigma, void *q, void *alpha, void *beta, void *V,
                                          int64_t vstride, void *W, int passes, void *work);

int lz_vector_lanczos(lz_handle *h, int64_t n, int64_t nnz, const int64_t *row_ptr,
                      const int32_t *col, const void *val, lz_dtype dtype, int m, int64_t lc,
                      const void *bvec, void *q, void *alpha, void *beta, void *q0, void *q1,
                      void *w);

int lz_fdtd_block(lz_handle *h, int64_t n, int64_t nnz, const int64_t *row_ptr,
                  const int32_t *col, const void *val, lz_dtype dtype, int b, const void *U0,
                  int64_t steps, double T_end, int64_t lc, void *U, void *D, void *out);

int lz_comm_unique_id(unsigned char out[128]);
int lz_comm_init(lz_handle *h, int nranks, int rank, const unsigned char id[128]);
int lz_comm_destroy(lz_handle *h);

typedef struct lz_local_group lz_local_group;
int lz_local_group_create(int device, int nranks, lz_local_group **g);
int lz_local_group_destroy(lz_local_group *g);
int lz_local_group_abort(lz_local_group *g);
int lz_comm_init_local(lz_handle *h, lz_local_group *g, int rank);
int lz_comm_abort(lz_handle *h);
int lz_debug_last_split(lz_handle *h, int64_t out[2]);
int lz_debug_last_wf(lz_handle *h, int out[2]);
enum {
    LZ_K_SEG768 = 1,
    LZ_K_SEG1536 = 2,
    LZ_K_SEG1024 = 3,
    LZ_K_FNZ = 4,
    LZ_K_BUF = 5,
    LZ_K_LDS = 6,
    LZ_K_ANY_B = 7,
    LZ_K_CM_DIRECT = 8,
    LZ_K_SPMV = 9,
    LZ_K_WIN = 0x100,
    LZ_K_YCM = 0x200,
    LZ_K_EPI = 0x400,
    LZ_K_AX3 = 0x800,
    LZ_K_DOT = 0x1000,
    LZ_K_AX4 = 0x2000,
    LZ_K_GRAM16 = 1,
    LZ_K_GRAM32F = 2,
    LZ_K_GRAM_GEN = 3,
    LZ_K_TSMM16 = 4,
    LZ_K_TSMM32F = 5,
    LZ_K_TSMM_GEN = 6,
    LZ_K_PGRAM16 = 7,
    LZ_K_PGRAM_GEN = 8,
    LZ_K_PAPPLY16 = 9,
    LZ_K_PAPPLY_GEN = 10,
    LZ_K_PCOMP16 = 11,
    LZ_K_PCOMP_GEN = 12,
    LZ_K_BCG16 = 13,
    LZ_K_BCG32F = 14,
    LZ_K_BCG_GEN = 15
};
int lz_debug_last_kernel(lz_handle *h, int out[2]);

int lz_debug_wf_plan(lz_handle *h, int64_t n, int64_t nnz, const int64_t *row_ptr, const int32_t *col_idx,
                     int64_t nx, int64_t xoff, int32_t *deps_out, int16_t *col16_out, int32_t info[8]);

int lz_block_lanczos_dist(lz_handle *h, int64_t n_local, int64_t n_pad, int64_t n_global,
                          int64_t nnz_local, const int64_t *row_ptr, const int32_t *col,
                          const void *val, lz_dtype dtype, int b, int m, int64_t lc_local,
                          int lc_rank, const void *B_local, void *q, void *alpha, void *beta,
                          void *Q0, void *Q1, void *W, void *X_full);

int lz_halo_init(lz_handle *h, int64_t row0, int64_t n_local, const int64_t *recv_counts,
                 const int32_t *halo_rows);
int lz_halo_sizes(lz_handle *h, int64_t *n_halo, int64_t *n_send);
int lz_halo_exchange(lz_handle *h, lz_dtype dtype, int b, void *X);
int lz_block_lanczos_halo(lz_handle *h, int64_t n_local, int64_t nnz_local, const int64_t *row_ptr,
                          const int32_t *col, const void *val, lz_dtype dtype, int b, int m,
                          int64_t lc_local, int lc_rank, const void *B_local, void *q, void *alpha,
                          void *beta, void *X0, void *X1);

#ifdef __cplusplus
}
#endif
#endif
```

Baseline: 561.0 iters/s.

## Fuse wavefront dependency planning into the first block-Lanczos SpMM launch

Adds a planning variant of the wavefront kernel (XO==3) that computes tile dependencies, 16-bit column compression and span statistics while it performs the first SpMM with the beta_0 Gram. The separate k_wf_deps pass and its blocking host sync are dropped, and plan stats are read back through pinned memory and an event. This removes one full read of row_ptr/col plus a launch-and-sync bubble before the solve. In exchange the first step always uses 32-bit columns, and if the plan turns out invalid the fused first step is thrown away and the fallback path runs.

```diff
diff --git a/gpu-implementation-of-signle-and-block-lanczos_amd/__init__.py b/gpu-implementation-of-signle-and-block-lanczos_amd/__init__.py
--- a/gpu-implementation-of-signle-and-block-lanczos_amd/__init__.py
+++ b/gpu-implementation-of-signle-and-block-lanczos_amd/__init__.py
@@ -147,6 +147,8 @@
     ("lz_debug_last_kernel", _c_int, [_c_vp, ctypes.POINTER(_c_int)]),
     ("lz_debug_wf_plan", _c_int, [_c_vp, _c_i64, _c_i64, _c_vp, _c_vp, _c_i64, _c_i64, _c_vp, _c_vp,
                                   ctypes.POINTER(_c_int)]),
+    ("lz_debug_wf_first_plan", _c_int, [_c_vp, _c_i64, _c_i64, _c_vp, _c_vp, _c_vp, _c_vp, _c_vp, _c_vp, _c_vp,
+                                        ctypes.POINTER(_c_int)]),
     ("lz_block_lanczos_dist", _c_int, [_c_vp, _c_i64, _c_i64, _c_i64, _c_i64, _c_vp, _c_vp, _c_vp,
                                        _c_int, _c_int, _c_int, _c_i64, _c_int, _c_vp, _c_vp, _c_vp,
                                        _c_vp, _c_vp, _c_vp, _c_vp, _c_vp]),
@@ -1488,6 +1490,24 @@
              "spans": [int(info[4 + i]) for i in range(4)]}
         return d, deps[: 2 * T].view(T, 2), c16[: A.nnz]
 
+    def wf_first_plan(self, A, B):
+        import torch
+        if A.val.dtype != torch.float64 or B.dtype != torch.float64 or tuple(B.shape) != (A.n, 16) \
+                or not B.is_contiguous():
+            raise ValueError("wf_first_plan: fp64 operator and a contiguous (n, 16) fp64 block")
+        T_max = A.n // 16 + 2
+        deps = torch.zeros(T_max * 2, dtype=torch.int32, device=A.row_ptr.device)
+        c16 = torch.zeros(max(A.nnz, 1), dtype=torch.int16, device=A.row_ptr.device)
+        Y = torch.empty_like(B)
+        info = (_c_int * 8)()
+        _check(self.L.lz_debug_wf_first_plan(self.ptr, A.n, A.nnz, A.row_ptr.data_ptr(), A.col.data_ptr(),
+                                             A.val.data_ptr(), B.data_ptr(), Y.data_ptr(), deps.data_ptr(),
+                                             c16.data_ptr(), info), "lz_debug_wf_first_plan")
+        T = int(info[2])
+        d = {"ok": bool(info[0]), "col16": bool(info[1]), "T": T, "tr": int(info[3]),
+             "spans": [int(info[4 + i]) for i in range(4)]}
+        return d, deps[: 2 * T].view(T, 2), c16[: A.nnz], Y
+
     def last_split(self):
         v = (_c_i64 * 2)()
         _check(self.L.lz_debug_last_split(self._h, v), "lz_debug_last_split")
diff --git a/gpu-implementation-of-signle-and-block-lanczos_amd/csrc/lz_api.hip b/gpu-implementation-of-signle-and-block-lanczos_amd/csrc/lz_api.hip
--- a/gpu-implementation-of-signle-and-block-lanczos_amd/csrc/lz_api.hip
+++ b/gpu-implementation-of-signle-and-block-lanczos_amd/csrc/lz_api.hip
@@ -516,28 +516,32 @@
     return LZ_OK;
 }
 
-static int block_lanczos_wf16(lz_handle *h, int64_t n, int64_t nnz, const int64_t *rp, const int32_t *col,
-                              const double *val, int m, int64_t lc, const double *B, double *q, double *alpha,
-                              double *beta, double *Q0, double *Q1, double *W, const Pass1Plan &pl,
-                              const WfPlan &wp, int Pg)
+struct Solve16 {
+    int64_t n, nnz;
+    const int64_t *rp;
+    const int32_t *col;
+    const double *val;
+    int m;
+    int64_t lc;
+    const double *B;
+    double *q, *alpha, *beta, *Q0, *Q1, *W;
+};
+
+static WfTail wf16_tail(lz_handle *h, const Solve16 &s, const Scratch16 &sc)
+{
+    const int64_t lcl = (s.lc >= 0 && s.lc < s.n) ? s.lc : -1;
+    return WfTail{h, sc.slab, sc.binv, sc.P1, sc.P2, s.alpha, s.beta, s.q, lcl};
+}
+
+static int wf16_steps(lz_handle *h, const Solve16 &s, const WfSolve &ws, const WfTail &tail, const Scratch16 &sc)
 {
     constexpr int64_t bb = 256;
-    (void)nnz;
-    const Scratch16 sc(h);
+    const int m = s.m;
     double *const *binv = sc.binv;
-    double *P1 = sc.P1, *P2 = sc.P2, *slab = sc.slab;
-    const int64_t lcl = (lc >= 0 && lc < n) ? lc : -1;
+    double *P1 = sc.P1, *P2 = sc.P2, *Q0 = s.Q0, *Q1 = s.Q1, *W = s.W;
+    double *part = h->partials2;
     int P = 0;
-    const bool g0 = Pg < 0;
-    if (!g0) LZ_TRY(sqrtm_pair<double>(h, 16, nullptr, Pg, beta, binv[0], nullptr));
-    LZ_TRY(wf_reset16(h, n, wp));
-    const WfSolve ws{n, rp, col, val, pl.pairs, wp, n};
-    const WfTail tail{h, slab, binv, P1, P2, alpha, beta, q, lcl};
-    double *part = h->partials2;
-    LZ_TRY(wf_step16(h, ws, ws.first(B, Q0, g0), part, &P));
-    if (g0) LZ_TRY(tail(0, wf_one_set(part, P), B));
-    else LZ_TRY(alpha_wf16(h, part, P, binv[0], nullptr, alpha, P2, B, lc, n, q));
-    const double *Vm1 = nullptr, *V0 = B;
+    const double *Vm1 = nullptr, *V0 = s.B;
     auto pass2 = [&](int j, double *Vn) { return WfPass2{Q0, Vm1, V0, Vn, binv[j & 1], j ? P1 : nullptr, P2}; };
     for (int j = 0; j + 1 < m; ++j) {
         double *Vn = j == 0 ? W : j == 1 ? Q1 : const_cast<double *>(Vm1);
@@ -546,16 +550,50 @@
         Vm1 = V0;
         V0 = Vn;
     }
-    LZ_TRY(store_beta_m<double>(h, beta, m, bb, binv));
+    LZ_TRY(store_beta_m<double>(h, s.beta, m, bb, binv));
     if (h->final_state) {
         const WfPass2 p2 = pass2(m - 1, W);
-        if (wp.var == 111)
+        if (ws.pl.var == 111)
             LZ_TRY(wf_step16(h, ws, ws.post_call(p2, m, Q0, m >= 2 ? Q1 : nullptr), part, &P));
         else
-            LZ_TRY(final_state<double>(h, n, 16, p2.Yj, p2.Vprev, p2.Vj, nullptr, p2.binv, p2.P1, p2.P2, W, Q0,
+            LZ_TRY(final_state<double>(h, s.n, 16, p2.Yj, p2.Vprev, p2.Vj, nullptr, p2.binv, p2.P1, p2.P2, W, Q0,
                                        m >= 2 ? Q1 : nullptr));
     }
     return LZ_OK;
+}
+
+static int block_lanczos_wf16(lz_handle *h, const Solve16 &s, const Pass1Plan &pl, const WfPlan &wp, int Pg)
+{
+    const Scratch16 sc(h);
+    int P = 0;
+    const bool g0 = Pg < 0;
+    if (!g0) LZ_TRY(sqrtm_pair<double>(h, 16, nullptr, Pg, s.beta, sc.binv[0], nullptr));
+    LZ_TRY(wf_reset16(h, s.n, wp));
+    const WfSolve ws{s.n, s.rp, s.col, s.val, pl.pairs, wp, s.n};
+    const WfTail tail = wf16_tail(h, s, sc);
+    double *part = h->partials2;
+    LZ_TRY(wf_step16(h, ws, ws.first(s.B, s.Q0, g0), part, &P));
+    if (g0) LZ_TRY(tail(0, wf_one_set(part, P), s.B));
+    else LZ_TRY(alpha_wf16(h, part, P, sc.binv[0], nullptr, s.alpha, sc.P2, s.B, s.lc, s.n, s.q));
+    return wf16_steps(h, s, ws, tail, sc);
+}
+
+static int block_lanczos_wf16_planning(lz_handle *h, const Solve16 &s, WfPlan &wp, bool *ran)
+{
+    const Scratch16 sc(h);
+    int P = 0;
+    Pass1Plan pl;
+    LZ_TRY(strip_pairs(h, s.n, s.rp, &pl.pairs));
+    LZ_TRY(wf_reset16(h, s.n, wp));
+    const WfSolve ws{s.n, s.rp, s.col, s.val, pl.pairs, wp, s.n};
+    const WfTail tail = wf16_tail(h, s, sc);
+    double *part = h->partials2;
+    LZ_TRY(wf_step16(h, ws, ws.first_plan(s.B, s.Q0), part, &P));
+    LZ_TRY(wf_first_plan_read(h));
+    LZ_TRY(tail(0, wf_one_set(part, P), s.B));
+    LZ_TRY(wf_first_plan_end(h, &wp));
+    *ran = wp.ok;
+    return wp.ok ? wf16_steps(h, s, ws, tail, sc) : LZ_OK;
 }
 
 static int block_lanczos_fused16(lz_handle *h, int64_t n, int64_t nnz, const int64_t *rp, const int32_t *col,
@@ -563,25 +601,35 @@
                                  double *alpha, double *beta, double *Q0, double *Q1, double *W)
 {
     constexpr int64_t bb = 256;
-    (void)Q0;
+    const Solve16 s{n, nnz, rp, col, val, m, lc, B, q, alpha, beta, Q0, Q1, W};
     const Scratch16 qb(h);
     double *const qP = qb.P1;
     int P = 0;
     Pass1Plan pl;
+    h->last_wf = h->last_wf_pre = 0;
     const bool g0 = wf_first_gram(n, nnz);
     if (!g0) LZ_TRY(gram_beside(h, n, B, &P));
     JoinSide join_side{h};
     {
         WfPlan wp;
-        LZ_TRY(wf_plan16(h, n, nnz, rp, col, &wp));
-        if (wp.ok) {
+        bool first_plans = false;
+        LZ_TRY(wf_first_plan_begin(h, n, nnz, &wp, &first_plans));
+        if (first_plans) {
+            bool ran = false;
+            LZ_TRY(block_lanczos_wf16_planning(h, s, wp, &ran));
+            h->last_wf = ran ? 1 : 0;
+            if (ran) return LZ_OK;
+        } else {
+            LZ_TRY(wf_plan16(h, n, nnz, rp, col, &wp));
+        }
+        if (!first_plans && wp.ok) {
             LZ_TRY(strip_pairs(h, n, rp, &pl.pairs));
             pl.col16 = wp.col16;
             if (!g0) LZ_HIP_TRY(hipStreamWaitEvent(h->stream, h->ev_join, 0));
             else if (wp.var != 111) LZ_TRY(gram_partials<double>(h, n, 16, B, B, 16, &P));
             const bool first = g0 && wp.var == 111;
-            return block_lanczos_wf16(h, n, nnz, rp, col, val, m, lc, B, q, alpha, beta, Q0, Q1, W, pl, wp,
-                                      first ? -1 : P);
+            h->last_wf = 1;
+            return block_lanczos_wf16(h, s, pl, wp, first ? -1 : P);
         }
     }
     if (g0) LZ_TRY(gram_partials<double>(h, n, 16, B, B, 16, &P));
@@ -1341,6 +1389,8 @@
     LZ_HIP_TRY(hipStreamCreateWithFlags(&h->side, hipStreamNonBlocking));
     LZ_HIP_TRY(hipEventCreateWithFlags(&h->ev_fork, hipEventDisableTiming));
     LZ_HIP_TRY(hipEventCreateWithFlags(&h->ev_join, hipEventDisableTiming));
+    LZ_HIP_TRY(hipEventCreateWithFlags(&h->ev_plan, hipEventDisableTiming));
+    LZ_HIP_TRY(hipHostMalloc(reinterpret_cast<void **>(&h->plan_host), 4 * sizeof(int), hipHostMallocDefault));
     if (const char *pz = getenv("LZ_POISON"); pz && pz[0] == '1') {
         LZ_HIP_TRY(hipMemsetAsync(h->partials, 0xFF, h->partials_cap, h->stream));
         LZ_HIP_TRY(hipMemsetAsync(h->partials2, 0xFF, sizeof(double) * kPartials2Doubles, h->stream));
@@ -1397,6 +1447,8 @@
     (void)hipFree(h->err_flag);
     if (h->ev_fork) (void)hipEventDestroy(h->ev_fork);
     if (h->ev_join) (void)hipEventDestroy(h->ev_join);
+    if (h->ev_plan) (void)hipEventDestroy(h->ev_plan);
+    if (h->plan_host) (void)hipHostFree(h->plan_host);
     if (h->ev_lfork) (void)hipEventDestroy(h->ev_lfork);
     if (h->ev_ljoin) (void)hipEventDestroy(h->ev_ljoin);
     if (h->lstream) (void)hipStreamDestroy(h->lstream);
@@ -2084,13 +2136,9 @@
     return LZ_OK;
 }
 
-int lz_debug_wf_plan(lz_handle *h, int64_t n, int64_t nnz, const int64_t *row_ptr, const int32_t *col_idx,
-                     int64_t nx, int64_t xoff, int32_t *deps_out, int16_t *col16_out, int32_t info[8])
-{
-    LZ_HANDLE_CHECK(h);
-    LZ_ARG_CHECK(row_ptr && col_idx && deps_out && col16_out && info, "NULL argument");
-    lz::WfPlan wp;
-    LZ_TRY(lz::wf_plan16(h, n, nnz, row_ptr, col_idx, &wp, nx, xoff));
+static int wf_plan_outputs(lz_handle *h, const lz::WfPlan &wp, int64_t n, int64_t nnz, int32_t *deps_out,
+                           int16_t *col16_out, int32_t info[8])
+{
     const int64_t T = wp.tr > 0 ? lz::ceil_div(n, (int64_t)wp.tr) : 0;
     int sp[4] = {0, 0, 0, 0};
     if (wp.planned && T > 0) {
@@ -2114,6 +2162,42 @@
     info[3] = wp.tr;
     for (int i = 0; i < 4; ++i) info[4 + i] = sp[i];
     return LZ_OK;
+}
+
+int lz_debug_wf_plan(lz_handle *h, int64_t n, int64_t nnz, const int64_t *row_ptr, const int32_t *col_idx,
+                     int64_t nx, int64_t xoff, int32_t *deps_out, int16_t *col16_out, int32_t info[8])
+{
+    LZ_HANDLE_CHECK(h);
+    LZ_ARG_CHECK(row_ptr && col_idx && deps_out && col16_out && info, "NULL argument");
+    lz::WfPlan wp;
+    LZ_TRY(lz::wf_plan16(h, n, nnz, row_ptr, col_idx, &wp, nx, xoff));
+    return wf_plan_outputs(h, wp, n, nnz, deps_out, col16_out, info);
+}
+
+int lz_debug_wf_first_plan(lz_handle *h, int64_t n, int64_t nnz, const int64_t *row_ptr, const int32_t *col_idx,
+                           const double *val, const double *B, double *Y_out, int32_t *deps_out, int16_t *col16_out,
+                           int32_t info[8])
+{
+    LZ_HANDLE_CHECK(h);
+    LZ_ARG_CHECK(row_ptr && col_idx && val && B && Y_out && deps_out && col16_out && info, "NULL argument");
+    LZ_ARG_CHECK(n >= 1 && nnz >= 0, "n >= 1, nnz >= 0");
+    lz::WfPlan wp;
+    bool go = false;
+    LZ_TRY(lz::wf_first_plan_begin(h, n, nnz, &wp, &go));
+    if (go) {
+        const uint64_t *pairs = nullptr;
+        int P = 0;
+        LZ_TRY(lz::strip_pairs(h, n, row_ptr, &pairs));
+        LZ_TRY(lz::wf_reset16(h, n, wp));
+        const lz::WfSolve ws{n, row_ptr, col_idx, val, pairs, wp, n};
+        LZ_TRY(lz::wf_step16(h, ws, ws.first_plan(B, Y_out), h->partials2, &P));
+        LZ_TRY(lz::wf_first_plan_read(h));
+        LZ_TRY(lz::wf_first_plan_end(h, &wp));
+    } else {
+        wp.tr = 0;
+        LZ_HIP_TRY(hipMemsetAsync(Y_out, 0, sizeof(double) * 16 * (size_t)n, h->stream));
+    }
+    return wf_plan_outputs(h, wp, n, nnz, deps_out, col16_out, info);
 }
 
 int lz_comm_destroy(lz_handle *h)
diff --git a/gpu-implementation-of-signle-and-block-lanczos_amd/csrc/lz_common.hpp b/gpu-implementation-of-signle-and-block-lanczos_amd/csrc/lz_common.hpp
--- a/gpu-implementation-of-signle-and-block-lanczos_amd/csrc/lz_common.hpp
+++ b/gpu-implementation-of-signle-and-block-lanczos_amd/csrc/lz_common.hpp
@@ -88,6 +88,8 @@
     void *wf_deps = nullptr;
     int *wf_flags = nullptr;
     size_t wf_deps_cap = 0, wf_flags_cap = 0;
+    int *plan_host = nullptr;
+    hipEvent_t ev_plan = nullptr;
     void *ybuf = nullptr;
     size_t ybuf_cap = 0;
     void *coef = nullptr;
diff --git a/gpu-implementation-of-signle-and-block-lanczos_amd/csrc/lz_internal.hpp b/gpu-implementation-of-signle-and-block-lanczos_amd/csrc/lz_internal.hpp
--- a/gpu-implementation-of-signle-and-block-lanczos_amd/csrc/lz_internal.hpp
+++ b/gpu-implementation-of-signle-and-block-lanczos_amd/csrc/lz_internal.hpp
@@ -129,10 +129,14 @@
     const int16_t *col16 = nullptr;
     int64_t xoff = 0;
     bool planned = false;
+    int16_t *c16_out = nullptr;
 };
 bool wf_first_gram(int64_t n, int64_t nnz);
 int wf_plan16(lz_handle *h, int64_t n, int64_t nnz, const int64_t *rp, const int32_t *col, WfPlan *pl,
               int64_t nx = -1, int64_t xoff = 0);
+int wf_first_plan_begin(lz_handle *h, int64_t n, int64_t nnz, WfPlan *pl, bool *go);
+int wf_first_plan_read(lz_handle *h);
+int wf_first_plan_end(lz_handle *h, WfPlan *pl);
 int wf_reset16(lz_handle *h, int64_t n, const WfPlan &pl);
 struct WfTiles {
     int64_t a, b;
@@ -150,7 +154,7 @@
     bool gram = false;
 };
 struct WfLaunch {
-    enum Role { kFirst, kBoundary, kStep, kPass2, kPostCall } role;
+    enum Role { kFirst, kFirstPlan, kBoundary, kStep, kPass2, kPostCall } role;
     WfPass1 p1;
     WfPass2 p2;
     WfTiles q, q2;
@@ -171,6 +175,10 @@
     WfLaunch first(const double *Vg, double *Yo, bool gram) const
     {
         return {WfLaunch::kFirst, {Vg, Yo, all(), gram}, {}, all(), none()};
+    }
+    WfLaunch first_plan(const double *Vg, double *Yo) const
+    {
+        return {WfLaunch::kFirstPlan, {Vg, Yo, all(), true}, {}, all(), none()};
     }
     WfLaunch boundary(const double *Vg, double *Yo, WfTiles t) const
     {
diff --git a/gpu-implementation-of-signle-and-block-lanczos_amd/csrc/lz_wf.hip b/gpu-implementation-of-signle-and-block-lanczos_amd/csrc/lz_wf.hip
--- a/gpu-implementation-of-signle-and-block-lanczos_amd/csrc/lz_wf.hip
+++ b/gpu-implementation-of-signle-and-block-lanczos_amd/csrc/lz_wf.hip
@@ -117,9 +117,12 @@
     __shared__ int ready[K], done[K], cons_in, upd_in;
     __shared__ int p1pub;
     const int lane = threadIdx.x & 63, w = __builtin_amdgcn_readfirstlane(threadIdx.x >> 6);
-    const bool has_p2 = P2 != nullptr, has_prev = P1 != nullptr;
-    constexpr bool kG0 = XO == 1 && DU >= 1 && NU * DU * 3 >= NC;
+    constexpr bool PLAN = XO == 3;
+    static_assert(!PLAN || (!C16 && !GEN && !SW), "the planning first launch: 32-bit columns, one GPU");
+    const bool has_p2 = !PLAN && P2 != nullptr, has_prev = P1 != nullptr;
+    constexpr bool kG0 = (XO == 1 || PLAN) && DU >= 1 && NU * DU * 3 >= NC;
     constexpr bool QO = XO == 2;
+    constexpr int kArrive = PLAN ? NC + 1 : NC;
     const bool g0 = kG0 && !has_p2 && Vj != nullptr;
     if (threadIdx.x < K) {
         ready[threadIdx.x] = -1;
@@ -140,7 +143,8 @@
         q1 = q2 = q3 = T;
         nx = n;
     }
-    if (T != Th || blockDim.x != 64 * (NC + NL + NU) || (kG0 != (!has_p2 && Vj != nullptr))) {
+    if (T != Th || blockDim.x != 64 * (NC + NL + NU) || (kG0 != (!has_p2 && Vj != nullptr)) ||
+        (PLAN && P2 != nullptr)) {
         if (threadIdx.x == 0) *err = 7;
         return;
     }
@@ -182,7 +186,7 @@
             if (i >= K) {
                 long spin = 0;
                 const uint32_t da = ws_lds_addr(&done[s]);
-                while (ws_lds_read(da) < NC * (int)(i / K) && ++spin < kWsSpin) __builtin_amdgcn_s_sleep(1);
+                while (ws_lds_read(da) < kArrive * (int)(i / K) && ++spin < kWsSpin) __builtin_amdgcn_s_sleep(1);
                 if (spin >= kWsSpin) { *err = 3; break; }
             }
             const int64_t ca = kA & ~(int64_t)(C::CPP - 1), va = kA & ~(int64_t)1;
@@ -400,6 +404,72 @@
                 __hip_atomic_store(flags + ptile(ut0 + (ntl - 1) * ustep), epoch, __ATOMIC_RELAXED,
                                    __HIP_MEMORY_SCOPE_AGENT);
         }
+        if constexpr (PLAN) {
+            int2 *dout = const_cast<int2 *>(deps);
+            int16_t *c16o = const_cast<int16_t *>(col16);
+            int sb = 0, sf = 0, sw = 0, bad = 0;
+            for (int64_t i = uw; i < nt; i += NU) {
+                const int s = (int)(i % K);
+                const int64_t t = tile_of(i), r0 = t * TR;
+                long spin = 0;
+                while (__hip_atomic_load(&ready[s], __ATOMIC_RELAXED, __HIP_MEMORY_SCOPE_WORKGROUP) != (int)i &&
+                       ++spin < kWsSpin)
+                    __builtin_amdgcn_s_sleep(1);
+                if (spin >= kWsSpin) { *err = 8; break; }
+                asm volatile("" ::: "memory");
+                const typename C::Stage &S = st[s];
+                const int64_t kA = S.rp[0];
+                const int nrow = (int)(n - r0 < TR ? n - r0 : TR);
+                const int32_t *cs = S.col + (int)(kA & (C::CPP - 1));
+                int mn = INT_MAX, mx = -1;
+                auto walk = [&](auto column) {
+                    for (int a = 0; a < nrow; a += 16) {
+                        const int b = a + 16 < nrow ? a + 16 : nrow;
+                        const int64_t s0 = r0 + a;
+                        for (int k = (int)(S.rp[a] - kA) + lane, e = (int)(S.rp[b] - kA); k < e; k += 64) {
+                            const int64_t c = column(k);
+                            if (c >= 0 && c < n) {
+                                mn = c < mn ? (int)c : mn;
+                                mx = c > mx ? (int)c : mx;
+                            }
+                            const int64_t d = c - s0;
+                            if (c16o) {
+                                bad |= (d < -32768) | (d > 32767);
+                                c16o[kA + k] = (int16_t)d;
+                            }
+                        }
+                    }
+                };
+                if (S.rp[nrow] - kA <= CAP) walk([&](int k) { return (int64_t)cs[k]; });
+                else walk([&](int k) { return (int64_t)col[kA + k]; });
+                asm volatile("s_waitcnt lgkmcnt(0)" ::: "memory");
+                if (lane == 0) atomicAdd(&done[s], 1);
+#pragma unroll
+                for (int o = 32; o > 0; o >>= 1) {
+                    const int a = __shfl_xor(mn, o, 64), b = __shfl_xor(mx, o, 64);
+                    mn = a < mn ? a : mn;
+                    mx = b > mx ? b : mx;
+                }
+                int lo = (int)t, hi = (int)t;
+                if (mx >= 0) {
+                    const int a = mn / TR, b = mx / TR;
+                    lo = a < lo ? a : lo;
+                    hi = b > hi ? b : hi;
+                }
+                if (lane == 0) dout[t] = make_int2(lo, hi);
+                sb = (int)t - lo > sb ? (int)t - lo : sb;
+                sf = hi - (int)t > sf ? hi - (int)t : sf;
+                sw = hi - lo + 1 > sw ? hi - lo + 1 : sw;
+            }
+            const int anybad = __ballot(bad) != 0 ? 1 : 0;
+            if (lane == 0) {
+                int *us = reinterpret_cast<int *>(&ust[uw][0][2][0]);
+                us[0] = sb;
+                us[1] = sf;
+                us[2] = sw;
+                us[3] = anybad;
+            }
+        }
         double *U = &ust[uw][0][0][0];
 #pragma unroll
         for (int r = 0; r < 4; ++r) {
@@ -415,6 +485,17 @@
                 double a = 0.0;
                 for (int u = 0; u < NU; ++u) a += ust[u][0][0][e];
                 if (!(g0 && e < 256)) part[(e < 256 ? 2 * G : G) * 256 + bid * 256 + (e & 255)] = a;
+            }
+            if constexpr (PLAN) {
+                if (lane < 4) {
+                    int v = 0;
+                    for (int u = 0; u < NU; ++u) {
+                        const int x = reinterpret_cast<const int *>(&ust[u][0][2][0])[lane];
+                        v = x > v ? x : v;
+                    }
+                    if (lane < 3) atomicMax(&flags[lane], v);
+                    else if (v) atomicOr(&flags[3], 1);
+                }
             }
         }
         return;
@@ -618,30 +699,50 @@
     return wf_shape(n, nnz, &nc, &allowed) == 111 && allowed;
 }
 
-int wf_plan16(lz_handle *h, int64_t n, int64_t nnz, const int64_t *rp, const int32_t *col, WfPlan *pl, int64_t nx,
-              int64_t xoff)
-{
-    if (nx < 0) nx = n;
+static int wf_plan_begin(lz_handle *h, int64_t n, int64_t nnz, int64_t nx, int64_t xoff, WfPlan *pl, int16_t **c16,
+                         bool *go)
+{
     pl->ok = false;
     pl->planned = false;
     pl->col16 = nullptr;
+    *c16 = nullptr;
     bool allowed = false;
     pl->var = wf_shape(n, nnz, &pl->nc, &allowed);
     pl->tr = 16 * pl->nc;
-    if (!allowed || n < pl->tr || xoff < 0 || xoff + n > nx ||
-        (double)nnz > kWfWideRow * (double)n)
-        return LZ_OK;
+    *go = allowed && n >= pl->tr && xoff >= 0 && xoff + n <= nx && (double)nnz <= kWfWideRow * (double)n;
+    if (!*go) return LZ_OK;
     const int64_t T = ceil_div(n, (int64_t)pl->tr);
     LZ_TRY(grow_ws(h, &h->wf_deps, &h->wf_deps_cap, sizeof(int2) * (size_t)(T + 64)));
     LZ_TRY(grow_ws(h, &h->wf_flags, &h->wf_flags_cap, sizeof(int) * (size_t)(T + 64)));
     const char *c = getenv("LZ_PASS1_C16");
-    int16_t *c16 = nullptr;
     if (!(c && c[0] == '0') && nnz > 0) {
         LZ_TRY(c16_reserve(h, nnz));
-        c16 = static_cast<int16_t *>(h->c16buf);
-    }
+        *c16 = static_cast<int16_t *>(h->c16buf);
+    }
+    LZ_HIP_TRY(hipMemsetAsync(flag_word(h, kFlagPlanStats), 0, 4 * sizeof(int), h->stream));
+    return LZ_OK;
+}
+
+static void wf_plan_fill(WfPlan *pl, const int sp[4], int16_t *c16, int64_t xoff)
+{
+    pl->planned = true;
+    pl->hback = sp[0];
+    pl->hfwd = sp[1];
+    pl->ok = sp[2] <= kWfMaxSpan && !(sp[3] & 2);
+    pl->xoff = xoff;
+    pl->col16 = c16 && !(sp[3] & 1) ? c16 : nullptr;
+}
+
+int wf_plan16(lz_handle *h, int64_t n, int64_t nnz, const int64_t *rp, const int32_t *col, WfPlan *pl, int64_t nx,
+              int64_t xoff)
+{
+    if (nx < 0) nx = n;
+    int16_t *c16 = nullptr;
+    bool go = false;
+    LZ_TRY(wf_plan_begin(h, n, nnz, nx, xoff, pl, &c16, &go));
+    if (!go) return LZ_OK;
+    const int64_t T = ceil_div(n, (int64_t)pl->tr);
     int *spans = flag_word(h, kFlagPlanStats);
-    LZ_HIP_TRY(hipMemsetAsync(spans, 0, 4 * sizeof(int), h->stream));
     const int grid = (int)std::max<int64_t>(1, std::min<int64_t>(T, (int64_t)h->n_cu * 8));
     hipLaunchKernelGGL(k_wf_deps, dim3(grid), dim3(256), 0, h->stream, n, pl->tr, rp, col,
                        static_cast<int2 *>(h->wf_deps), c16, spans, xoff, nx >= kWinRows ? 1 : 0);
@@ -649,12 +750,33 @@
     int sp[4] = {0, 0, 0, 1};
     LZ_HIP_TRY(hipMemcpyAsync(sp, spans, sizeof(sp), hipMemcpyDeviceToHost, h->stream));
     LZ_HIP_TRY(hipStreamSynchronize(h->stream));
-    pl->planned = true;
-    pl->hback = sp[0];
-    pl->hfwd = sp[1];
-    pl->ok = sp[2] <= kWfMaxSpan && !(sp[3] & 2);
-    pl->xoff = xoff;
-    if (c16 && !(sp[3] & 1)) pl->col16 = c16;
+    wf_plan_fill(pl, sp, c16, xoff);
+    return LZ_OK;
+}
+
+int wf_first_plan_begin(lz_handle *h, int64_t n, int64_t nnz, WfPlan *pl, bool *go)
+{
+    const char *e = getenv("LZ_WF_FUSED_PLAN");
+    *go = false;
+    if ((e && e[0] == '0') || !wf_first_gram(n, nnz) || n >= kWinRows) return LZ_OK;
+    LZ_TRY(wf_plan_begin(h, n, nnz, n, 0, pl, &pl->c16_out, go));
+    pl->ok = *go;
+    return LZ_OK;
+}
+
+int wf_first_plan_read(lz_handle *h)
+{
+    LZ_HIP_TRY(hipMemcpyAsync(h->plan_host, flag_word(h, kFlagPlanStats), 4 * sizeof(int), hipMemcpyDeviceToHost,
+                              h->stream));
+    LZ_HIP_TRY(hipEventRecord(h->ev_plan, h->stream));
+    return LZ_OK;
+}
+
+int wf_first_plan_end(lz_handle *h, WfPlan *pl)
+{
+    LZ_HIP_TRY(hipEventSynchronize(h->ev_plan));
+    wf_plan_fill(pl, h->plan_host, pl->c16_out, 0);
+    pl->c16_out = nullptr;
     return LZ_OK;
 }
 
@@ -666,9 +788,10 @@
     const int64_t n = ws.n, nx = ws.nx, T = ws.T(), xoff = pl.xoff;
     const int64_t p1a = p1.t.a, p1b = p1.t.b, q0 = L.q.a, q1 = L.q.b, q2 = L.q2.a, q3 = L.q2.b;
     const bool has_p2 = L.role >= WfLaunch::kStep, qo = L.role == WfLaunch::kPostCall;
-    const bool g0 = L.role == WfLaunch::kFirst && p1.gram;
+    const bool fp = L.role == WfLaunch::kFirstPlan;
+    const bool g0 = (L.role == WfLaunch::kFirst && p1.gram) || fp;
     const bool sw = has_p2 && p2.Vsave != nullptr;
-    const int16_t *col16 = pl.col16;
+    const int16_t *col16 = fp ? pl.c16_out : pl.col16;
     LZ_ARG_CHECK(xoff >= 0 && xoff + n <= nx && 0 <= p1a && p1a <= p1b && p1b <= T, "wavefront step ranges");
     LZ_ARG_CHECK(0 <= q0 && q0 <= q1 && q1 <= q2 && q2 <= q3 && q3 <= T, "wavefront step pass-2 ranges");
     LZ_ARG_CHECK(pl.ok && n < (1 << 24), "wavefront step: wf_plan16 first");
@@ -679,6 +802,9 @@
     LZ_ARG_CHECK(!qo || (L.Q0 && pl.var == 111 && xoff == 0 && nx == n),
                  "wavefront post-call state: a one-GPU launch of the default shape");
     LZ_ARG_CHECK(!g0 || pl.var == 111, "wavefront first launch with beta_0's Gram: the default shape only (internal)");
+    LZ_ARG_CHECK(!fp || (xoff == 0 && nx == n && n < kWinRows && !pl.col16 &&
+                         sizeof(int2) * (size_t)T <= h->wf_deps_cap),
+                 "wavefront planning first launch: one GPU, wf_first_plan_begin first");
     static_assert(12 <= kPairPad, "row orders must cover the last tile's strips");
     const int64_t nq = (q1 - q0) + (q3 - q2);
     const int64_t work = has_p2 ? std::max(nq, p1b - p1a) : p1b - p1a;
@@ -726,7 +852,8 @@
         }
         hipLaunchKernelGGL(kern, dim3(grid), dim3(64 * waves), 0, h->stream, n, ws.rp, ws.col, col16, ws.val, ws.pairs,
                            p2.Yj, p2.Vprev, g0 ? p1.Vg : p2.Vj, p2.Vout, p2.binv, p2.P1, p2.P2, p1.Vg,
-                           qo ? L.Q1 : p1.Yo, static_cast<const int2 *>(h->wf_deps), h->wf_flags, L.epoch,
+                           qo ? L.Q1 : p1.Yo, static_cast<const int2 *>(h->wf_deps),
+                           fp ? flag_word(h, kFlagPlanStats) : h->wf_flags, L.epoch,
                            (int64_t)pl.hback, lead, part, h->err_flag, dbg, nx, p1a, p1b, T, cpol, xoff, q0, q1, q2, q3,
                            qo ? L.Q0 : p2.Vsave);
     };
@@ -740,6 +867,7 @@
 #endif
     if (qo && col16) go(k_wf16<11, cap11, kWfK, 1, 4, 1, true, false, false, 2>, 11 + 1 + 4);
     else if (qo) go(k_wf16<11, cap11, kWfK, 1, 4, 1, false, false, false, 2>, 11 + 1 + 4);
+    else if (fp) go(k_wf16<11, cap11, kWfK, 1, 4, 1, false, false, false, 3>, 11 + 1 + 4);
     else if (g0 && col16 && spec) go(k_wf16<11, cap11, kWfK, 1, 4, 1, true, false, false, 1>, 11 + 1 + 4);
     else if (g0 && col16) go(k_wf16<11, cap11, kWfK, 1, 4, 1, true, false, true, 1>, 11 + 1 + 4);
     else if (g0 && spec) go(k_wf16<11, cap11, kWfK, 1, 4, 1, false, false, false, 1>, 11 + 1 + 4);
diff --git a/include/lz_hip.h b/include/lz_hip.h
--- a/include/lz_hip.h
+++ b/include/lz_hip.h
@@ -231,6 +231,10 @@
 int lz_debug_wf_plan(lz_handle *h, int64_t n, int64_t nnz, const int64_t *row_ptr, const int32_t *col_idx,
                      int64_t nx, int64_t xoff, int32_t *deps_out, int16_t *col16_out, int32_t info[8]);
 
+int lz_debug_wf_first_plan(lz_handle *h, int64_t n, int64_t nnz, const int64_t *row_ptr, const int32_t *col_idx,
+                           const double *val, const double *B, double *Y_out, int32_t *deps_out, int16_t *col16_out,
+                           int32_t info[8]);
+
 int lz_block_lanczos_dist(lz_handle *h, int64_t n_local, int64_t n_pad, int64_t n_global,
                           int64_t nnz_local, const int64_t *row_ptr, const int32_t *col,
                           const void *val, lz_dtype dtype, int b, int m, int64_t lc_local,
```

Result: no change. 561.0 iters/s (median of 3 runs) (-0.0%).
